# ukeSJTU/tiaozhanbei-unet

Measured on AMD Instinct MI355X. Metric: training images/sec, AnomalyUNet 256x256 bs=32 per GPU, higher is better.
Workload: dtype bf16; 1 GPU; AnomalyUNet 3x256x256, bs=32/GPU, MSE+focal loss, Adam (BASELINE.json configs[2], synthetic randn images, bernoulli masks); global_batch=32, parallelism=dp1, accumulate=fp32, master_params=fp32, dist_world=1, reserved_cus=0, cu_budget=256

## Files before the change

include/unet_hip.h:

```cpp
#ifndef UNET_HIP_H_
#define UNET_HIP_H_

#include <stddef.h>
#include <stdint.h>

#ifdef __cplusplus
extern "C" {
#endif

#define UNET_ABI_VERSION 1

enum unet_dtype { UNET_F32 = 0, UNET_BF16 = 1 };

enum unet_status {
  UNET_OK = 0,
  UNET_ERR_BAD_ARG = -1,
  UNET_ERR_UNSUPPORTED = -2,
  UNET_ERR_WORKSPACE = -3,
  UNET_ERR_LAUNCH = -4
};

typedef struct unet_view {
  void* ptr;
  int32_t c;
  int32_t h, w;
  int32_t off_y, off_x;
} unet_view;

int32_t unet_abi_version(void);
const char* unet_last_error(void);

int32_t unet_set_reserved_cus(int32_t n);
int32_t unet_get_cu_budget(void);
int32_t unet_debug_spin(int32_t blocks, int32_t lds_bytes, int32_t microseconds, void* stream);

enum unet_kclass {
  UNET_K_CONV_FWD = 0, UNET_K_CONV_DGRAD, UNET_K_CONV_WGRAD, UNET_K_CONVT_FWD, UNET_K_CONVT_DGRAD,
  UNET_K_CONVT_WGRAD, UNET_K_BN, UNET_K_POOL, UNET_K_HEAD, UNET_K_LOSS, UNET_K_PACK, UNET_K_OTHER,
  UNET_K_COUNT
};
int32_t unet_prof_enable(int32_t on);
int32_t unet_prof_collect(double* ms, int64_t* launches, double* flops);
int32_t unet_prof_kernel_stats(int32_t index, const char** name, double* ms, int64_t* launches, double* flops);
int32_t unet_prof_kernel_bytes(int32_t index, double* bytes);

int32_t unet_nchw_to_nhwc(const float* src, void* dst, int32_t n, int32_t c, int32_t h, int32_t w,
                          int32_t c_pad, int32_t dtype, void* stream);
int32_t unet_nhwc_to_nchw(const void* src, float* dst, int32_t n, int32_t c, int32_t h, int32_t w,
                          int32_t c_pad, int32_t dtype, void* stream);

enum unet_pack_mode {
  UNET_PACK_CONV_FWD = 0,
  UNET_PACK_CONV_DGRAD = 1,
  UNET_PACK_CONVT_FWD = 2,
  UNET_PACK_CONVT_DGRAD = 3
};
int32_t unet_pack_weight(const float* w, void* out, int32_t c_out, int32_t c_in, int32_t rows,
                         int32_t k, int32_t mode, int32_t dtype, void* stream);

typedef struct unet_pack_desc {
  const float* w;
  void* out;
  int32_t c_out, c_in, rows, k, mode, reserved;
} unet_pack_desc;
int32_t unet_pack_weights_batched(const unet_pack_desc* descs, int32_t n, int32_t dtype, void* stream);

int32_t unet_pack_weight_seg(const float* w, void* out, int32_t c_out, int32_t c_in, int32_t rows, int32_t k,
                             int32_t mode, int32_t split, int32_t dtype, void* stream);
int32_t unet_pack_conv_weight_folded_seg(const float* w, const float* scale, void* out, int32_t c_out, int32_t c_in,
                                         int32_t rows, int32_t k, int32_t split, int32_t dtype, void* stream);

enum unet_remap_op { UNET_REMAP_PAD = 0, UNET_REMAP_UNPAD = 1 };
#define UNET_REMAP_MAX 8
typedef struct unet_remap_desc {
  const float* src;
  float* dst;
  int32_t rows, cols, inner;
  int32_t prows, pcols;
  int32_t split, op, reserved;
} unet_remap_desc;
int32_t unet_remap_batched(const unet_remap_desc* descs, int32_t n, void* stream);

int32_t unet_widen_channels(const void* src, int32_t src_dtype, const int64_t* strides, int32_t n, int32_t c, int32_t h,
                            int32_t w, void* dst, int32_t c_pad, int32_t dtype, void* stream);

int32_t unet_conv3x3(int32_t dtype, int32_t n, int32_t h, int32_t w, const unet_view src[2],
                     const void* w_packed, int32_t c_out, const unet_view dst[2], int32_t dst_split,
                     int32_t accumulate, int32_t kclass, void* stream);

int32_t unet_pack_conv_weight_folded(const float* w, const float* scale, void* out, int32_t c_out, int32_t c_in,
                                     int32_t rows, int32_t k, int32_t dtype, void* stream);
int32_t unet_conv3x3_bias_relu(int32_t dtype, int32_t n, int32_t h, int32_t w, const unet_view src[2],
                               const void* w_packed, int32_t c_out, void* y, const float* bias, int32_t relu,
                               void* stream);

int32_t unet_conv3x3_first_supported(int32_t c_in, int32_t c_out, int32_t h, int32_t w);
int32_t unet_conv3x3_first_stats(int32_t n, int32_t h, int32_t w, const float* x_nchw, int32_t c_in,
                                 const float* weight_oihw, void* y, float* partial, int32_t* n_parts, void* stream);
size_t unet_conv3x3_first_wgrad_workspace(int32_t n, int32_t h, int32_t w);
int32_t unet_conv3x3_first_wgrad(int32_t n, int32_t h, int32_t w, const float* x_nchw, int32_t c_in, const void* dy,
                                 float* dw, void* workspace, size_t workspace_bytes, void* stream);
int32_t unet_conv3x3_first_wgrad_bn(int32_t n, int32_t h, int32_t w, const float* x_nchw, int32_t c_in, const void* dz,
                                    const void* y, const float* coefs, float* dw, void* workspace,
                                    size_t workspace_bytes, void* stream);

size_t unet_conv3x3_stats_max_parts(int32_t n, int32_t h, int32_t w);
int32_t unet_conv3x3_stats(int32_t dtype, int32_t n, int32_t h, int32_t w, const unet_view src[2],
                           const void* w_packed, int32_t c_out, void* y, float* partial, int32_t* n_parts,
                           void* stream);

int32_t unet_conv3x3_dgrad_bnrelu_supported(int32_t dtype, int32_t n, int32_t h, int32_t w, int32_t c_dy, int32_t c_dx);
int32_t unet_conv3x3_dgrad_bnrelu(int32_t dtype, int32_t n, int32_t h, int32_t w, const void* dy, int32_t c_dy,
                                  const void* w_packed, int32_t c_dx, const void* y_prev, const float* bn_scale,
                                  const float* bn_shift, const float* bn_mean, void* dz, float* partial,
                                  int32_t* n_parts, void* stream);

size_t unet_conv3x3_wgrad_workspace(int32_t n, int32_t h, int32_t w, int32_t c_in, int32_t c_out);
int32_t unet_conv3x3_wgrad(int32_t dtype, int32_t n, int32_t h, int32_t w, const unet_view src[2],
                           const void* dy, int32_t c_out, float* dw, int32_t c_in_param,
                           void* workspace, size_t workspace_bytes, void* stream);

int32_t unet_convt2x2_fwd(int32_t dtype, int32_t n, int32_t h, int32_t w, const void* x, int32_t c_in,
                          const void* w_packed, const float* bias, void* y, int32_t c_out, void* stream);
int32_t unet_convt2x2_dgrad(int32_t dtype, int32_t n, int32_t h, int32_t w, const void* dy,
                            int32_t c_out, const void* w_packed, void* dx, int32_t c_in, void* stream);

int32_t unet_convt2x2_dgrad_bnrelu_supported(int32_t dtype, int32_t n, int32_t h, int32_t w, int32_t c_in, int32_t c_out);
size_t unet_convt2x2_dgrad_bnrelu_max_parts(void);
int32_t unet_convt2x2_dgrad_bnrelu(int32_t dtype, int32_t n, int32_t h, int32_t w, const void* dy, int32_t c_out,
                                   const void* w_packed, const void* y_prev, const float* bn_scale, const float* bn_shift,
                                   const float* bn_mean, void* dz, int32_t c_in, float* partial, int32_t* n_parts,
                                   void* stream);
size_t unet_convt2x2_wgrad_workspace(int32_t n, int32_t h, int32_t w, int32_t c_in, int32_t c_out);
int32_t unet_convt2x2_wgrad(int32_t dtype, int32_t n, int32_t h, int32_t w, const void* x, int32_t c_in,
                            const void* dy, int32_t c_out, float* dw, float* db, void* workspace,
                            size_t workspace_bytes, void* stream);

size_t unet_bn_workspace(int64_t pixels, int32_t c);
int32_t unet_bn_train_stats(int32_t dtype, const void* y, int64_t pixels, int32_t c, const float* gamma,
                            const float* beta, float* running_mean, float* running_var, float momentum,
                            float eps, float* save_mean, float* save_istd, float* scale, float* shift,
                            void* workspace, size_t workspace_bytes, void* stream);
int32_t unet_bn_finalize_partials(const float* partial, int32_t n_parts, int64_t pixels, int32_t c,
                                  const float* gamma, const float* beta, float* running_mean,
                                  float* running_var, float momentum, float eps, float* save_mean,
                                  float* save_istd, float* scale, float* shift, void* stream);
int32_t unet_bn_eval_coeffs(int32_t c, const float* gamma, const float* beta, const float* running_mean,
                            const float* running_var, float eps, float* scale, float* shift, void* stream);
int32_t unet_bn_eval_coeffs4(int32_t c, const float* gamma, const float* beta, const float* running_mean,
                             const float* running_var, float eps, float* mean, float* istd, float* scale,
                             float* shift, void* stream);
int32_t unet_bn_relu_apply(int32_t dtype, const void* y, int64_t pixels, int32_t c, const float* scale,
                           const float* shift, void* a, void* stream);
int32_t unet_bn_relu_bwd(int32_t dtype, const void* da, const void* y, int64_t pixels, int32_t c,
                         const float* gamma, const float* save_mean, const float* save_istd,
                         const float* scale, const float* shift, float* dgamma, float* dbeta, void* dy,
                         void* workspace, size_t workspace_bytes, void* stream);

int32_t unet_bn_relu_bwd_frozen(int32_t dtype, const void* da, const void* y, int64_t pixels, int32_t c,
                                const float* gamma, const float* mean, const float* istd, const float* scale,
                                const float* shift, float* dgamma, float* dbeta, void* dy, void* workspace,
                                size_t workspace_bytes, void* stream);
int32_t unet_bn_bwd_premasked(int32_t dtype, const void* dz, const void* y, int64_t pixels, int32_t c,
                              const float* gamma, const float* save_mean, const float* save_istd,
                              const float* partial, int32_t n_parts, float* dgamma, float* dbeta, void* dy,
                              void* workspace, size_t workspace_bytes, void* stream);

int32_t unet_maxpool2_fwd(int32_t dtype, const void* x, int32_t n, int32_t h, int32_t w, int32_t c,
                          void* y, void* stream);
int32_t unet_maxpool2_bwd(int32_t dtype, const void* x, const void* dy, int32_t n, int32_t h, int32_t w,
                          int32_t c, void* dx, int32_t accumulate, void* stream);

int32_t unet_bn_relu_pool_supported(int32_t dtype, int32_t c);
int32_t unet_bn_relu_pool_fwd(int32_t dtype, const void* y, int32_t n, int32_t h, int32_t w, int32_t c,
                              const float* scale, const float* shift, void* a, void* pooled, void* stream);
size_t unet_bn_relu_pool_max_parts(void);
int32_t unet_bn_relu_pool_bwd(int32_t dtype, const void* y, const void* dpooled, const void* da_old, int32_t n, int32_t h,
                              int32_t w, int32_t c, const float* scale, const float* shift, const float* mean, void* dz,
                              float* partial, int32_t* n_parts, void* stream);

int32_t unet_upsample_bilinear2x_fwd(int32_t dtype, const void* x, int32_t n, int32_t h, int32_t w,
                                     int32_t c, void* y, void* stream);
int32_t unet_upsample_bilinear2x_bwd(int32_t dtype, const void* dy, int32_t n, int32_t h, int32_t w,
                                     int32_t c, void* dx, void* stream);

int32_t unet_head_fwd(int32_t dtype, const void* x, int32_t n, int32_t h, int32_t w, int32_t c_in,
                      const float* weight, const float* bias, int32_t c_out, int32_t sigmoid, float* out,
                      void* stream);
size_t unet_head_bwd_workspace(int32_t n, int32_t h, int32_t w, int32_t c_in, int32_t c_out);
int32_t unet_head_bwd(int32_t dtype, const void* x, const float* out, const float* dout, int32_t n,
                      int32_t h, int32_t w, int32_t c_in, const float* weight, int32_t c_out,
                      int32_t sigmoid, void* dx, float* dweight, float* dbias, void* workspace,
                      size_t workspace_bytes, void* stream);

int32_t unet_head_bnrelu_fwd(int32_t dtype, const void* y, int32_t n, int32_t h, int32_t w, int32_t c_in,
                             const float* bn_scale, const float* bn_shift, const float* weight, const float* bias,
                             int32_t c_out, int32_t sigmoid, float* out, void* stream);
size_t unet_head_bnrelu_max_parts(void);
int32_t unet_head_bnrelu_bwd(int32_t dtype, const void* y, const float* bn_scale, const float* bn_shift,
                             const float* bn_mean, const float* out, const float* dout, int32_t n, int32_t h, int32_t w,
                             int32_t c_in, const float* weight, int32_t c_out, int32_t sigmoid, void* dz,
                             float* dweight, float* dbias, float* bn_partial, int32_t* n_parts, void* workspace,
                             size_t workspace_bytes, void* stream);

size_t unet_loss_workspace(int64_t elems);
int32_t unet_loss_mse_focal(const float* recon, const float* image, int64_t n_recon, const float* amap,
                            const float* mask, int64_t n_amap, float alpha, float gamma, float* losses,
                            float* d_recon, float* d_amap, void* workspace, size_t workspace_bytes,
                            void* stream);
size_t unet_ssim_workspace(int32_t planes, int32_t h, int32_t w);
int32_t unet_ssim_loss(const float* img1, const float* img2, int32_t planes, int32_t h, int32_t w,
                       int32_t window, float* loss, float* d_img1, float* d_img2, void* workspace,
                       size_t workspace_bytes, void* stream);

int32_t unet_ssim_loss_per_image(const float* img1, const float* img2, int32_t n, int32_t c, int32_t h, int32_t w,
                                 int32_t window, float* loss, float* d_img1, float* d_img2, void* workspace,
                                 size_t workspace_bytes, void* stream);

size_t unet_seg_loss_workspace(int32_t n, int32_t c, int64_t hw);
int32_t unet_seg_loss(const float* logits, const int64_t* target, int32_t n, int32_t c, int64_t hw,
                      const float* class_weights, int64_t ignore_index, int32_t input_is_prob, float ce_weight,
                      float dice_weight, float focal_weight, float focal_alpha, float focal_gamma, float* loss,
                      float* dlogits, void* workspace, size_t workspace_bytes, void* stream);
int32_t unet_seg_confusion(const float* logits, const int64_t* target, int32_t n, int32_t c, int64_t hw,
                           int64_t ignore_index, int64_t* labels, int64_t* confusion, void* stream);
size_t unet_seg_image_stats_workspace(int32_t n, int32_t c, int64_t hw);
int32_t unet_seg_image_stats(const float* logits, const int64_t* target, int32_t n, int32_t c, int64_t hw,
                             int64_t ignore_index, uint8_t* labels, int64_t* confusion, double* conf, void* workspace,
                             size_t workspace_bytes, void* stream);

int32_t unet_threshold_confusion(const float* pred, const float* truth, const uint8_t* select, int64_t n_images,
                                 int64_t per_image, const float* thresholds, int32_t k, int64_t* counts, void* stream);

int32_t unet_rank_auc_append(const float* pred, const float* truth, const uint8_t* select, int64_t n_images,
                             int64_t per_image, uint32_t* keys, int64_t capacity, int64_t* counts, void* stream);
size_t unet_rank_auc_workspace(int64_t n_pos, int64_t n_neg);
int32_t unet_rank_auc(uint32_t* pos_keys, int64_t n_pos, uint32_t* neg_keys, int64_t n_neg, double* out,
                      void* workspace, size_t workspace_bytes, void* stream);

size_t unet_label_regions_workspace(int64_t n, int64_t h, int64_t w);
int32_t unet_label_regions(const float* truth, const uint8_t* select, int64_t n, int64_t h, int64_t w, int32_t* labels,
                           int32_t* sizes, int64_t* counts, void* workspace, size_t workspace_bytes, void* stream);

size_t unet_label_class_regions_workspace(int64_t n, int64_t h, int64_t w, int32_t num_classes);
int32_t unet_label_class_regions(const uint8_t* classes, int64_t n, int64_t h, int64_t w, int32_t num_classes,
                                 int32_t* region, int32_t* sizes, int64_t* counts, void* workspace,
                                 size_t workspace_bytes, void* stream);
size_t unet_match_class_regions_workspace(int64_t n, int64_t h, int64_t w, int32_t num_classes);
int32_t unet_match_class_regions(const uint8_t* truth, const int32_t* truth_region, const int32_t* truth_sizes,
                                 const uint8_t* pred, const int32_t* pred_region, const int32_t* pred_sizes, int64_t n,
                                 int64_t h, int64_t w, int32_t num_classes, int32_t min_pixels, int32_t image_base,
                                 int32_t* truth_records, int32_t* pred_records, int64_t capacity,
                                 int64_t* record_counts, void* workspace, size_t workspace_bytes, void* stream);

int32_t unet_region_auc_append(const float* pred, const int32_t* sizes, const uint8_t* select, int64_t n_images,
                               int64_t per_image, void* slots, int64_t capacity, int64_t* counts, void* stream);
size_t unet_region_auc_workspace(int64_t n_pos, int64_t n_neg);
int32_t unet_region_auc(uint64_t* pos_pairs, int64_t n_pos, uint32_t* neg_keys, int64_t n_neg, int64_t regions,
                        int64_t max_region, double fpr_limit, double* out, void* workspace, size_t workspace_bytes,
                        void* stream);

enum unet_panel_kind {
  UNET_PANEL_IMAGE = 0, UNET_PANEL_UNIT = 1, UNET_PANEL_GRAY = 2, UNET_PANEL_HOT = 3, UNET_PANEL_OVERLAY = 4
};
typedef struct unet_panel {
  int32_t kind;
  int32_t alpha8;
  const float* rgb;
  const float* map;
} unet_panel;
int32_t unet_render_range(const unet_panel* panels, int32_t k, int32_t n, int32_t h, int32_t w, uint32_t* keys,
                          void* stream);
int32_t unet_render_sheet(const unet_panel* panels, int32_t k, int32_t n, int32_t h, int32_t w, int32_t gutter,
                          const float* mean3, const float* std3, const uint32_t* keys, const uint8_t* luts,
                          uint8_t* sheet, void* stream);

int32_t unet_seg_confidence(const float* logits, int32_t n, int32_t c, int64_t hw, uint8_t* labels, float* conf,
                            void* stream);

enum unet_seg_panel_kind {
  UNET_SEG_PANEL_IMAGE = 0, UNET_SEG_PANEL_CLASSES = 1, UNET_SEG_PANEL_OVERLAY = 2, UNET_SEG_PANEL_LUT = 3
};
typedef struct unet_seg_panel {
  int32_t kind;
  int32_t alpha8;
  const uint8_t* labels;
  const float* map;
} unet_seg_panel;
int32_t unet_seg_render_sheet(const float* image, const unet_seg_panel* panels, int32_t k, int32_t n, int32_t h,
                              int32_t w, int32_t gutter, int32_t per_row, const float* mean3, const float* std3,
                              const uint8_t* palette, const uint8_t* lut, uint8_t* sheet, void* stream);

int32_t unet_channel_scale(int32_t dtype, const void* x, const float* scale, int32_t n, int64_t hw, int32_t c, void* y,
                           void* stream);
size_t unet_anomaly_score_workspace(int32_t n, int64_t hw);
int32_t unet_anomaly_score(const float* recon, const float* image, int32_t n, int32_t c, int64_t hw, int32_t l1,
                           float* score, float* image_score, void* workspace, size_t workspace_bytes, void* stream);

int32_t unet_preprocess_u8(const uint8_t* images_hwc, const uint8_t* flip, float* out_nchw, int32_t n, int32_t h,
                           int32_t w, const float* mean3, const float* std3, void* stream);

int32_t unet_resize_bilinear_ksize(int32_t in_size, int32_t out_size);
int32_t unet_resize_bilinear_coeffs(int32_t in_size, int32_t out_size, int32_t* bounds, int32_t* kk);
int32_t unet_resize_bilinear_u8(const uint8_t* src, int32_t n, int32_t h, int32_t w, int32_t c, int32_t out_h,
                                int32_t out_w, const int32_t* xbounds, const int32_t* xkk, int32_t xksize,
                                const int32_t* ybounds, const int32_t* ykk, int32_t yksize, uint8_t* tmp, uint8_t* dst,
                                void* stream);
int32_t unet_resize_nearest_index(int32_t in_size, int32_t out_size, int32_t* idx);
int32_t unet_resize_nearest_u8(const uint8_t* src, int32_t n, int32_t h, int32_t w, int32_t c, int32_t out_h,
                               int32_t out_w, const int32_t* yidx, const int32_t* xidx, uint8_t* dst, void* stream);
int32_t unet_polygon_mask_u8(const int32_t* verts, const int32_t* poly_offsets, const int32_t* poly_class,
                             const int32_t* poly_image, int32_t n_polys, int32_t max_poly_vertices, const int32_t* src_hw,
                             int32_t n, int32_t out_h, int32_t out_w, const int32_t* yidx, const int32_t* xidx,
                             uint8_t* dst, void* stream);
int32_t unet_polygon_class_histogram(const int32_t* verts, const int32_t* poly_offsets, const int32_t* poly_class,
                                     const int32_t* poly_image, int32_t n_polys, int32_t max_poly_vertices,
                                     const int32_t* src_hw, int32_t n, int32_t max_h, int32_t max_w, int64_t* hist,
                                     void* stream);
int32_t unet_flip_rotate_u8(const uint8_t* src, int32_t n, int32_t h, int32_t w, int32_t c, const uint8_t* flip,
                            const int32_t* matrices, uint8_t* dst, void* stream);
typedef struct unet_jitter_desc {
  int32_t order[4];
  float brightness, contrast, saturation;
  int32_t hue_shift;
} unet_jitter_desc;
size_t unet_color_jitter_workspace(int32_t n);
int32_t unet_color_jitter_normalize_u8(const uint8_t* images_hwc, int32_t n, int32_t h, int32_t w,
                                       const unet_jitter_desc* desc, const float* mean3, const float* std3,
                                       float* out_nchw, void* workspace, size_t workspace_bytes, void* stream);

int32_t unet_adam_step(float* param, const float* grad, float* exp_avg, float* exp_avg_sq, int64_t n,
                       float lr, double beta1, double beta2, float eps, float weight_decay,
                       float grad_scale, int32_t step, void* stream);

typedef struct unet_adam_desc {
  float* p;
  const float* g;
  float* m;
  float* v;
  int64_t n;
} unet_adam_desc;
typedef struct unet_adam_chunk {
  int32_t tensor;
  int32_t reserved;
  int64_t first;
} unet_adam_chunk;
int32_t unet_adam_chunk_elems(void);
int32_t unet_adam_multi(const unet_adam_desc* descs, const unet_adam_chunk* chunks, int32_t n_chunks, float lr, double beta1,
                        double beta2, float eps, float weight_decay, float grad_scale, int32_t step, int32_t decoupled,
                        void* stream);

#ifdef __cplusplus
}
#endif
#endif
```

tiaozhanbei_unet_amd/_lib.py:

```python
from __future__ import annotations

import ctypes as C
import os
import subprocess

_HERE = os.path.dirname(os.path.abspath(__file__))
LIB_PATH = os.environ.get("UNET_HIP_LIB") or os.path.join(_HERE, "libunet_hip.so")
CSRC = os.path.join(_HERE, "csrc")

UNET_F32, UNET_BF16 = 0, 1
PACK_CONV_FWD, PACK_CONV_DGRAD, PACK_CONVT_FWD, PACK_CONVT_DGRAD = 0, 1, 2, 3
(K_CONV_FWD, K_CONV_DGRAD, K_CONV_WGRAD, K_CONVT_FWD, K_CONVT_DGRAD, K_CONVT_WGRAD, K_BN, K_POOL,
 K_HEAD, K_LOSS, K_PACK, K_OTHER, K_COUNT) = range(13)
KCLASS_NAMES = ["conv3x3_fwd", "conv3x3_dgrad", "conv3x3_wgrad", "convt_fwd", "convt_dgrad",
                "convt_wgrad", "bn", "pool_upsample", "head", "loss", "pack_layout", "other"]


class View(C.Structure):
    _fields_ = [("ptr", C.c_void_p), ("c", C.c_int32), ("h", C.c_int32), ("w", C.c_int32),
                ("off_y", C.c_int32), ("off_x", C.c_int32)]


View2 = View * 2


class RemapDesc(C.Structure):
    _fields_ = [("src", C.c_void_p), ("dst", C.c_void_p), ("rows", C.c_int32), ("cols", C.c_int32),
                ("inner", C.c_int32), ("prows", C.c_int32), ("pcols", C.c_int32), ("split", C.c_int32),
                ("op", C.c_int32), ("reserved", C.c_int32)]


REMAP_PAD, REMAP_UNPAD = 0, 1


class Panel(C.Structure):
    _fields_ = [("kind", C.c_int32), ("alpha8", C.c_int32), ("rgb", C.c_void_p), ("map", C.c_void_p)]


PANEL_IMAGE, PANEL_UNIT, PANEL_GRAY, PANEL_HOT, PANEL_OVERLAY = range(5)


class SegPanel(C.Structure):
    _fields_ = [("kind", C.c_int32), ("alpha8", C.c_int32), ("labels", C.c_void_p), ("map", C.c_void_p)]


SEG_PANEL_IMAGE, SEG_PANEL_CLASSES, SEG_PANEL_OVERLAY, SEG_PANEL_LUT = range(4)
_i, _l, _f, _p, _z, _d = C.c_int32, C.c_int64, C.c_float, C.c_void_p, C.c_size_t, C.c_double

SIGNATURES = {
    "unet_abi_version": (_i, []),
    "unet_last_error": (C.c_char_p, []),
    "unet_set_reserved_cus": (_i, [_i]),
    "unet_get_cu_budget": (_i, []),
    "unet_debug_spin": (_i, [_i, _i, _i, _p]),
    "unet_prof_enable": (_i, [_i]),
    "unet_prof_collect": (_i, [_p, _p, _p]),
    "unet_prof_kernel_stats": (_i, [_i, _p, _p, _p, _p]),
    "unet_prof_kernel_bytes": (_i, [_i, _p]),
    "unet_nchw_to_nhwc": (_i, [_p, _p, _i, _i, _i, _i, _i, _i, _p]),
    "unet_nhwc_to_nchw": (_i, [_p, _p, _i, _i, _i, _i, _i, _i, _p]),
    "unet_pack_weight": (_i, [_p, _p, _i, _i, _i, _i, _i, _i, _p]),
    "unet_pack_weights_batched": (_i, [_p, _i, _i, _p]),
    "unet_pack_weight_seg": (_i, [_p, _p, _i, _i, _i, _i, _i, _i, _i, _p]),
    "unet_pack_conv_weight_folded_seg": (_i, [_p, _p, _p, _i, _i, _i, _i, _i, _i, _p]),
    "unet_remap_batched": (_i, [_p, _i, _p]),
    "unet_widen_channels": (_i, [_p, _i, _p, _i, _i, _i, _i, _p, _i, _i, _p]),
    "unet_conv3x3": (_i, [_i, _i, _i, _i, C.POINTER(View), _p, _i, C.POINTER(View), _i, _i, _i, _p]),
    "unet_pack_conv_weight_folded": (_i, [_p, _p, _p, _i, _i, _i, _i, _i, _p]),
    "unet_conv3x3_bias_relu": (_i, [_i, _i, _i, _i, C.POINTER(View), _p, _i, _p, _p, _i, _p]),
    "unet_conv3x3_stats_max_parts": (_z, [_i, _i, _i]),
    "unet_conv3x3_stats": (_i, [_i, _i, _i, _i, C.POINTER(View), _p, _i, _p, _p, _p, _p]),
    "unet_conv3x3_first_supported": (_i, [_i, _i, _i, _i]),
    "unet_conv3x3_first_stats": (_i, [_i, _i, _i, _p, _i, _p, _p, _p, _p, _p]),
    "unet_conv3x3_first_wgrad_workspace": (_z, [_i, _i, _i]),
    "unet_conv3x3_first_wgrad": (_i, [_i, _i, _i, _p, _i, _p, _p, _p, _z, _p]),
    "unet_conv3x3_first_wgrad_bn": (_i, [_i, _i, _i, _p, _i, _p, _p, _p, _p, _p, _z, _p]),
    "unet_bn_finalize_partials": (_i, [_p, _i, _l, _i, _p, _p, _p, _p, _f, _f, _p, _p, _p, _p, _p]),
    "unet_convt2x2_dgrad_bnrelu_supported": (_i, [_i, _i, _i, _i, _i, _i]),
    "unet_convt2x2_dgrad_bnrelu_max_parts": (_z, []),
    "unet_convt2x2_dgrad_bnrelu": (_i, [_i, _i, _i, _i, _p, _i, _p, _p, _p, _p, _p, _p, _i, _p, _p, _p]),
    "unet_conv3x3_dgrad_bnrelu_supported": (_i, [_i, _i, _i, _i, _i, _i]),
    "unet_conv3x3_dgrad_bnrelu": (_i, [_i, _i, _i, _i, _p, _i, _p, _i, _p, _p, _p, _p, _p, _p, _p, _p]),
    "unet_conv3x3_wgrad_workspace": (_z, [_i, _i, _i, _i, _i]),
    "unet_conv3x3_wgrad": (_i, [_i, _i, _i, _i, C.POINTER(View), _p, _i, _p, _i, _p, _z, _p]),
    "unet_convt2x2_fwd": (_i, [_i, _i, _i, _i, _p, _i, _p, _p, _p, _i, _p]),
    "unet_convt2x2_dgrad": (_i, [_i, _i, _i, _i, _p, _i, _p, _p, _i, _p]),
    "unet_convt2x2_wgrad_workspace": (_z, [_i, _i, _i, _i, _i]),
    "unet_convt2x2_wgrad": (_i, [_i, _i, _i, _i, _p, _i, _p, _i, _p, _p, _p, _z, _p]),
    "unet_bn_workspace": (_z, [_l, _i]),
    "unet_bn_train_stats": (_i, [_i, _p, _l, _i, _p, _p, _p, _p, _f, _f, _p, _p, _p, _p, _p, _z, _p]),
    "unet_bn_eval_coeffs": (_i, [_i, _p, _p, _p, _p, _f, _p, _p, _p]),
    "unet_bn_eval_coeffs4": (_i, [_i, _p, _p, _p, _p, _f, _p, _p, _p, _p, _p]),
    "unet_bn_relu_bwd_frozen": (_i, [_i, _p, _p, _l, _i, _p, _p, _p, _p, _p, _p, _p, _p, _p, _z, _p]),
    "unet_bn_relu_apply": (_i, [_i, _p, _l, _i, _p, _p, _p, _p]),
    "unet_bn_relu_bwd": (_i, [_i, _p, _p, _l, _i, _p, _p, _p, _p, _p, _p, _p, _p, _p, _z, _p]),
    "unet_bn_bwd_premasked": (_i, [_i, _p, _p, _l, _i, _p, _p, _p, _p, _i, _p, _p, _p, _p, _z, _p]),
    "unet_head_bnrelu_fwd": (_i, [_i, _p, _i, _i, _i, _i, _p, _p, _p, _p, _i, _i, _p, _p]),
    "unet_head_bnrelu_max_parts": (_z, []),
    "unet_head_bnrelu_bwd": (_i, [_i, _p, _p, _p, _p, _p, _p, _i, _i, _i, _i, _p, _i, _i, _p, _p, _p, _p, _p, _p, _z, _p]),
    "unet_maxpool2_fwd": (_i, [_i, _p, _i, _i, _i, _i, _p, _p]),
    "unet_maxpool2_bwd": (_i, [_i, _p, _p, _i, _i, _i, _i, _p, _i, _p]),
    "unet_bn_relu_pool_supported": (_i, [_i, _i]),
    "unet_bn_relu_pool_fwd": (_i, [_i, _p, _i, _i, _i, _i, _p, _p, _p, _p, _p]),
    "unet_bn_relu_pool_max_parts": (_z, []),
    "unet_bn_relu_pool_bwd": (_i, [_i, _p, _p, _p, _i, _i, _i, _i, _p, _p, _p, _p, _p, _p, _p]),
    "unet_upsample_bilinear2x_fwd": (_i, [_i, _p, _i, _i, _i, _i, _p, _p]),
    "unet_upsample_bilinear2x_bwd": (_i, [_i, _p, _i, _i, _i, _i, _p, _p]),
    "unet_head_fwd": (_i, [_i, _p, _i, _i, _i, _i, _p, _p, _i, _i, _p, _p]),
    "unet_head_bwd_workspace": (_z, [_i, _i, _i, _i, _i]),
    "unet_head_bwd": (_i, [_i, _p, _p, _p, _i, _i, _i, _i, _p, _i, _i, _p, _p, _p, _p, _z, _p]),
    "unet_loss_workspace": (_z, [_l]),
    "unet_loss_mse_focal": (_i, [_p, _p, _l, _p, _p, _l, _f, _f, _p, _p, _p, _p, _z, _p]),
    "unet_ssim_workspace": (_z, [_i, _i, _i]),
    "unet_ssim_loss": (_i, [_p, _p, _i, _i, _i, _i, _p, _p, _p, _p, _z, _p]),
    "unet_ssim_loss_per_image": (_i, [_p, _p, _i, _i, _i, _i, _i, _p, _p, _p, _p, _z, _p]),
    "unet_seg_loss_workspace": (_z, [_i, _i, _l]),
    "unet_seg_loss": (_i, [_p, _p, _i, _i, _l, _p, _l, _i, _f, _f, _f, _f, _f, _p, _p, _p, _z, _p]),
    "unet_seg_confusion": (_i, [_p, _p, _i, _i, _l, _l, _p, _p, _p]),
    "unet_seg_image_stats_workspace": (_z, [_i, _i, _l]),
    "unet_seg_image_stats": (_i, [_p, _p, _i, _i, _l, _l, _p, _p, _p, _p, _z, _p]),
    "unet_threshold_confusion": (_i, [_p, _p, _p, _l, _l, _p, _i, _p, _p]),
    "unet_rank_auc_append": (_i, [_p, _p, _p, _l, _l, _p, _l, _p, _p]),
    "unet_rank_auc_workspace": (_z, [_l, _l]),
    "unet_rank_auc": (_i, [_p, _l, _p, _l, _p, _p, _z, _p]),
    "unet_label_regions_workspace": (_z, [_l, _l, _l]),
    "unet_label_regions": (_i, [_p, _p, _l, _l, _l, _p, _p, _p, _p, _z, _p]),
    "unet_label_class_regions_workspace": (_z, [_l, _l, _l, _i]),
    "unet_label_class_regions": (_i, [_p, _l, _l, _l, _i, _p, _p, _p, _p, _z, _p]),
    "unet_match_class_regions_workspace": (_z, [_l, _l, _l, _i]),
    "unet_match_class_regions": (_i, [_p, _p, _p, _p, _p, _p, _l, _l, _l, _i, _i, _i, _p, _p, _l, _p, _p, _z, _p]),
    "unet_region_auc_append": (_i, [_p, _p, _p, _l, _l, _p, _l, _p, _p]),
    "unet_region_auc_workspace": (_z, [_l, _l]),
    "unet_region_auc": (_i, [_p, _l, _p, _l, _l, _l, _d, _p, _p, _z, _p]),
    "unet_render_range": (_i, [_p, _i, _i, _i, _i, _p, _p]),
    "unet_render_sheet": (_i, [_p, _i, _i, _i, _i, _i, _p, _p, _p, _p, _p, _p]),
    "unet_seg_confidence": (_i, [_p, _i, _i, _l, _p, _p, _p]),
    "unet_seg_render_sheet": (_i, [_p, _p, _i, _i, _i, _i, _i, _i, _p, _p, _p, _p, _p, _p]),
    "unet_channel_scale": (_i, [_i, _p, _p, _i, _l, _i, _p, _p]),
    "unet_anomaly_score_workspace": (_z, [_i, _l]),
    "unet_anomaly_score": (_i, [_p, _p, _i, _i, _l, _i, _p, _p, _p, _z, _p]),
    "unet_preprocess_u8": (_i, [_p, _p, _p, _i, _i, _i, _p, _p, _p]),
    "unet_resize_bilinear_ksize": (_i, [_i, _i]),
    "unet_resize_bilinear_coeffs": (_i, [_i, _i, _p, _p]),
    "unet_resize_bilinear_u8": (_i, [_p, _i, _i, _i, _i, _i, _i, _p, _p, _i, _p, _p, _i, _p, _p, _p]),
    "unet_resize_nearest_index": (_i, [_i, _i, _p]),
    "unet_resize_nearest_u8": (_i, [_p, _i, _i, _i, _i, _i, _i, _p, _p, _p, _p]),
    "unet_polygon_mask_u8": (_i, [_p, _p, _p, _p, _i, _i, _p, _i, _i, _i, _p, _p, _p, _p]),
    "unet_polygon_class_histogram": (_i, [_p, _p, _p, _p, _i, _i, _p, _i, _i, _i, _p, _p]),
    "unet_flip_rotate_u8": (_i, [_p, _i, _i, _i, _i, _p, _p, _p, _p]),
    "unet_color_jitter_workspace": (_z, [_i]),
    "unet_color_jitter_normalize_u8": (_i, [_p, _i, _i, _i, _p, _p, _p, _p, _p, _z, _p]),
    "unet_adam_chunk_elems": (_i, []),
    "unet_adam_multi": (_i, [_p, _p, _i, _f, _d, _d, _f, _f, _f, _i, _i, _p]),
    "unet_adam_step": (_i, [_p, _p, _p, _p, _l, _f, _d, _d, _f, _f, _f, _i, _p]),
}

_lib = None


def build(force: bool = False) -> str:
    if force or not os.path.exists(LIB_PATH) or _stale():
        subprocess.run(["make", "-C", CSRC, "-j8"], check=True, stdout=subprocess.DEVNULL)
    return LIB_PATH


def _stale() -> bool:
    if not os.path.isdir(CSRC):
        return False
    t = os.path.getmtime(LIB_PATH)
    srcs = [os.path.join(CSRC, f) for f in os.listdir(CSRC) if f.endswith((".hip", ".h"))]
    srcs.append(os.path.join(_HERE, "..", "include", "unet_hip.h"))
    return any(os.path.exists(s) and os.path.getmtime(s) > t for s in srcs)


def lib():
    global _lib
    if _lib is None:
        if not os.path.exists(LIB_PATH):
            raise RuntimeError(
                f"libunet_hip.so not found at {LIB_PATH}: the HIP extension is the only compute path of "
                "tiaozhanbei_unet_amd (no CPU/eager fallback). Build it with "
                "`python -c 'import __graft_entry__ as g; g.build()'` or `make -C tiaozhanbei_unet_amd/csrc`.")
        handle = C.CDLL(LIB_PATH)
        for name, (res, args) in SIGNATURES.items():
            fn = getattr(handle, name)
            fn.restype, fn.argtypes = res, args
        if handle.unet_abi_version() != 1:
            raise RuntimeError("libunet_hip.so: ABI version mismatch")
        _lib = handle
    return _lib


def check(rc: int, what: str) -> None:
    if rc != 0:
        msg = lib().unet_last_error().decode(errors="replace")
        raise RuntimeError(f"{what} failed (status {rc}): {msg}")
```

tiaozhanbei_unet_amd/csrc/elementwise.hip:

```cpp
#include "common.h"

namespace {

inline int ew_blocks(long long items) { return (int)std::min<long long>(cdiv64(items, 256), 256 * 16); }

template <typename T>
__global__ __launch_bounds__(256) void nchw_to_nhwc_kernel(const float* __restrict__ src, T* __restrict__ dst,
                                                           int N, int C, int H, int W, int Cp) {
  constexpr int PIECE = ET<T>::PIECE;
  const long long hw = (long long)H * W;
  const long long total = (long long)N * hw;
  for (long long i = blockIdx.x * (long long)blockDim.x + threadIdx.x; i < total;
       i += (long long)gridDim.x * blockDim.x) {
    const long long n = i / hw, p = i - n * hw;
    const float* s = src + n * C * hw + p;
    T* o = dst + i * Cp;
    for (int c0 = 0; c0 < Cp; c0 += PIECE) {
      float v[PIECE];
#pragma unroll
      for (int j = 0; j < PIECE; ++j) v[j] = (c0 + j < C) ? s[(long long)(c0 + j) * hw] : 0.f;
      Vec<T>::store(o + c0, v);
    }
  }
}

template <typename T>
__global__ void nhwc_to_nchw_kernel(const T* __restrict__ src, float* __restrict__ dst, int N, int C, int H,
                                    int W, int Cp) {
  const long long hw = (long long)H * W;
  const long long total = (long long)N * C * hw;
  for (long long i = blockIdx.x * (long long)blockDim.x + threadIdx.x; i < total;
       i += (long long)gridDim.x * blockDim.x) {
    const long long p = i % hw;
    const long long t = i / hw;
    const int c = (int)(t % C);
    const long long n = t / C;
    dst[i] = ET<T>::to_f(src[(n * hw + p) * Cp + c]);
  }
}

template <typename T>
__global__ void pack_weight_kernel(const float* __restrict__ w, T* __restrict__ out, int Co, int Ci, int rows,
                                   int K, int mode, long long total, const float* __restrict__ scale) {
  for (long long i = blockIdx.x * (long long)blockDim.x + threadIdx.x; i < total;
       i += (long long)gridDim.x * blockDim.x) {
    float v = 0.f;
    if (mode == UNET_PACK_CONV_FWD) {
      const int ci = (int)(i % K);
      long long t = i / K;
      const int co = (int)(t % rows);
      const int tap = (int)(t / rows);
      if (co < Co && ci < Ci) v = w[((long long)co * Ci + ci) * 9 + tap] * (scale ? scale[co] : 1.f);
    } else if (mode == UNET_PACK_CONV_DGRAD) {
      const int co = (int)(i % K);
      long long t = i / K;
      const int ci = (int)(t % rows);
      const int tap = (int)(t / rows);
      if (co < Co && ci < Ci) v = w[((long long)co * Ci + ci) * 9 + (8 - tap)];
    } else if (mode == UNET_PACK_CONVT_FWD) {
      const int ci = (int)(i % K);
      long long t = i / K;
      const int co = (int)(t % rows);
      const int z = (int)(t / rows);
      if (co < Co && ci < Ci) v = w[((long long)ci * Co + co) * 4 + z];
    } else {
      const int co = (int)(i % K);
      long long t = i / K;
      const int z = (int)(t % 4);
      const int ci = (int)(t / 4);
      if (co < Co && ci < Ci) v = w[((long long)ci * Co + co) * 4 + z];
    }
    out[i] = ET<T>::from_f(v);
  }
}

template <typename T>
__global__ __launch_bounds__(256) void pack_weights_batched_kernel(const unet_pack_desc* __restrict__ descs) {
  __shared__ float tile[32 * 289];
  const unet_pack_desc d = descs[blockIdx.y];
  const int mode = d.mode;
  if (d.reserved > 0 && mode <= UNET_PACK_CONV_DGRAD) {
    const long long total = 9LL * d.rows * d.k;
    T* __restrict__ out = reinterpret_cast<T*>(d.out);
    for (long long i = blockIdx.x * 256LL + threadIdx.x; i < total; i += (long long)gridDim.x * 256)
      out[i] = ET<T>::from_f(unet_pack_seg_value(d.w, d.c_out, d.c_in, d.rows, d.k, mode, d.reserved, i, nullptr));
    return;
  }
  if constexpr (sizeof(T) == 2) {
    auto pair_ok = [](const unet_pack_desc& f, const unet_pack_desc& g) {
      return f.mode == UNET_PACK_CONV_FWD && g.mode == UNET_PACK_CONV_DGRAD && f.w == g.w && f.c_out == g.c_out &&
             f.c_in == g.c_in && f.rows == f.c_out && f.k == f.c_in && g.rows == g.c_in && g.k == g.c_out &&
             (f.c_out & 31) == 0 && (f.c_in & 31) == 0;
    };
    if (mode == UNET_PACK_CONV_DGRAD && blockIdx.y > 0 && pair_ok(descs[blockIdx.y - 1], d)) return;
    if (mode == UNET_PACK_CONV_FWD && blockIdx.y + 1 < gridDim.y && pair_ok(d, descs[blockIdx.y + 1])) {
      const unet_pack_desc g = descs[blockIdx.y + 1];
      const int Co = d.c_out, Ci = d.c_in;
      const int nB = Ci / 32, ntile = (Co / 32) * nB;
      const float* __restrict__ w = d.w;
      bf16_t* __restrict__ of = reinterpret_cast<bf16_t*>(d.out);
      bf16_t* __restrict__ og = reinterpret_cast<bf16_t*>(g.out);
      for (int t = blockIdx.x; t < ntile; t += gridDim.x) {
        const int a0 = (t / nB) * 32, b0 = (t % nB) * 32;
        __syncthreads();
        for (int i = threadIdx.x; i < 32 * 288; i += 256) {
          const int al = i / 288, r = i - al * 288;
          tile[al * 289 + r] = w[((size_t)(a0 + al) * Ci + b0) * 9 + r];
        }
        __syncthreads();
        for (int gi = threadIdx.x; gi < 2 * 32 * 9 * 4; gi += 256) {
          const int lay = gi / (32 * 9 * 4), rem = gi % (32 * 9 * 4);
          const int q = rem & 3, rest = rem >> 2;
          const int tap = rest % 9, outer = rest / 9;
          bf16x8 r8;
          if (lay == 0) {
#pragma unroll
            for (int e = 0; e < 8; ++e) r8[e] = (bf16_t)tile[outer * 289 + (q * 8 + e) * 9 + tap];
            *reinterpret_cast<bf16x8*>(of + ((size_t)tap * Co + a0 + outer) * Ci + b0 + q * 8) = r8;
          } else {
#pragma unroll
            for (int e = 0; e < 8; ++e) r8[e] = (bf16_t)tile[(q * 8 + e) * 289 + outer * 9 + tap];
            *reinterpret_cast<bf16x8*>(og + ((size_t)(8 - tap) * Ci + b0 + outer) * Co + a0 + q * 8) = r8;
          }
        }
      }
      return;
    }
  }
  const bool conv = mode <= UNET_PACK_CONV_DGRAD;
  const int taps = conv ? 9 : 4;
  const int As = conv ? d.c_out : d.c_in, Bs = conv ? d.c_in : d.c_out;
  const bool along_b = (mode == UNET_PACK_CONV_FWD || mode == UNET_PACK_CONVT_DGRAD);
  const int Ap = (mode == UNET_PACK_CONV_FWD || mode == UNET_PACK_CONVT_DGRAD) ? d.rows : d.k;
  const int Bp = (mode == UNET_PACK_CONV_FWD || mode == UNET_PACK_CONVT_DGRAD) ? d.k : d.rows;
  const int TA = along_b ? 8 : 64, TB = along_b ? 64 : 8;
  const int nA = (Ap + TA - 1) / TA, nB = (Bp + TB - 1) / TB;
  const float* __restrict__ w = d.w;
  T* __restrict__ out = reinterpret_cast<T*>(d.out);
  const int run = TB * taps;
  for (int t = blockIdx.x; t < nA * nB; t += gridDim.x) {
    const int a0 = (t / nB) * TA, b0 = (t % nB) * TB;
    __syncthreads();
    for (int i = threadIdx.x; i < TA * run; i += 256) {
      const int al = i / run, r = i - al * run;
      const int a = a0 + al, bb = b0 + r / taps;
      tile[i] = (a < As && bb < Bs) ? w[((size_t)a * Bs + b0) * taps + r] : 0.f;
    }
    __syncthreads();
    if ((((along_b ? Bp : Ap) & 7) == 0) && ((d.k & 7) == 0)) {
      for (int gi = threadIdx.x; gi < TA * TB * taps / 8; gi += 256) {
        const int inner0 = (gi & 7) * 8, rest = gi >> 3;
        const int tap = rest % taps, outer = rest / taps;
        const int al0 = along_b ? outer : inner0, bl0 = along_b ? inner0 : outer;
        const int a = a0 + al0, bb = b0 + bl0;
        if (a >= Ap || bb >= Bp) continue;
        float v[8];
#pragma unroll
        for (int e = 0; e < 8; ++e) v[e] = tile[(al0 + (along_b ? 0 : e)) * run + (bl0 + (along_b ? e : 0)) * taps + tap];
        size_t o;
        if (mode == UNET_PACK_CONV_FWD) o = ((size_t)tap * d.rows + a) * d.k + bb;
        else if (mode == UNET_PACK_CONV_DGRAD) o = ((size_t)(8 - tap) * d.rows + bb) * d.k + a;
        else if (mode == UNET_PACK_CONVT_FWD) o = ((size_t)tap * d.rows + bb) * d.k + a;
        else o = ((size_t)a * 4 + tap) * d.k + bb;
        if constexpr (sizeof(T) == 2) {
          bf16x8 r;
#pragma unroll
          for (int e = 0; e < 8; ++e) r[e] = (bf16_t)v[e];
          *reinterpret_cast<bf16x8*>(out + o) = r;
        } else {
          *reinterpret_cast<f32x4*>(out + o) = f32x4{v[0], v[1], v[2], v[3]};
          *reinterpret_cast<f32x4*>(out + o + 4) = f32x4{v[4], v[5], v[6], v[7]};
        }
      }
      continue;
    }
    for (int i = threadIdx.x; i < TA * TB * taps; i += 256) {
      const int inner = i & 63, rest = i >> 6;
      const int tap = rest % taps, outer = rest / taps;
      const int al = along_b ? outer : inner, bl = along_b ? inner : outer;
      const int a = a0 + al, bb = b0 + bl;
      if (a >= Ap || bb >= Bp) continue;
      const float v = tile[al * run + bl * taps + tap];
      size_t o;
      if (mode == UNET_PACK_CONV_FWD) o = ((size_t)tap * d.rows + a) * d.k + bb;
      else if (mode == UNET_PACK_CONV_DGRAD) o = ((size_t)(8 - tap) * d.rows + bb) * d.k + a;
      else if (mode == UNET_PACK_CONVT_FWD) o = ((size_t)tap * d.rows + bb) * d.k + a;
      else o = ((size_t)a * 4 + tap) * d.k + bb;
      out[o] = ET<T>::from_f(v);
    }
  }
}

template <typename T>
__global__ void maxpool2_fwd_kernel(const T* __restrict__ x, T* __restrict__ y, int N, int H, int W, int C) {
  constexpr int PIECE = ET<T>::PIECE;
  const int OH = H / 2, OW = W / 2, G = C / PIECE;
  const long long total = (long long)N * OH * OW * G;
  for (long long i = blockIdx.x * (long long)blockDim.x + threadIdx.x; i < total;
       i += (long long)gridDim.x * blockDim.x) {
    const int g = (int)(i % G);
    long long t = i / G;
    const int ox = (int)(t % OW);  t /= OW;
    const int oy = (int)(t % OH);
    const long long n = t / OH;
    const T* p = x + ((n * H + 2 * oy) * W + 2 * ox) * (long long)C + g * PIECE;
    float a[PIECE], b[PIECE], c[PIECE], d[PIECE];
    Vec<T>::load(p, a);
    Vec<T>::load(p + C, b);
    Vec<T>::load(p + (long long)W * C, c);
    Vec<T>::load(p + (long long)W * C + C, d);
#pragma unroll
    for (int j = 0; j < PIECE; ++j) a[j] = fmaxf(fmaxf(a[j], b[j]), fmaxf(c[j], d[j]));
    Vec<T>::store(y + i * PIECE, a);
  }
}

template <typename T>
__global__ void maxpool2_bwd_kernel(const T* __restrict__ x, const T* __restrict__ dy, T* __restrict__ dx,
                                    int N, int H, int W, int C, int accumulate) {
  constexpr int PIECE = ET<T>::PIECE;
  const int OH = H / 2, OW = W / 2, G = C / PIECE;
  const int WH = (H + 1) / 2, WW = (W + 1) / 2;
  const long long total = (long long)N * WH * WW * G;
  for (long long i = blockIdx.x * (long long)blockDim.x + threadIdx.x; i < total;
       i += (long long)gridDim.x * blockDim.x) {
    const int g = (int)(i % G);
    long long t = i / G;
    const int ox = (int)(t % WW);  t /= WW;
    const int oy = (int)(t % WH);
    const long long n = t / WH;
    const long long base = ((n * H + 2 * oy) * W + 2 * ox) * (long long)C + g * PIECE;
    float z[PIECE];
#pragma unroll
    for (int j = 0; j < PIECE; ++j) z[j] = 0.f;
    if (oy < OH && ox < OW) {
      float a[PIECE], b[PIECE], c[PIECE], d[PIECE], gr[PIECE];
      Vec<T>::load(x + base, a);
      Vec<T>::load(x + base + C, b);
      Vec<T>::load(x + base + (long long)W * C, c);
      Vec<T>::load(x + base + (long long)W * C + C, d);
      Vec<T>::load(dy + (((n * OH + oy) * OW + ox) * (long long)C + g * PIECE), gr);
      float ga[PIECE], gb[PIECE], gc[PIECE], gd[PIECE];
#pragma unroll
      for (int j = 0; j < PIECE; ++j) {
        const float m = fmaxf(fmaxf(a[j], b[j]), fmaxf(c[j], d[j]));
        const bool fa = a[j] == m, fb = !fa && b[j] == m, fc = !fa && !fb && c[j] == m;
        const bool fd = !fa && !fb && !fc;
        ga[j] = fa ? gr[j] : 0.f; gb[j] = fb ? gr[j] : 0.f; gc[j] = fc ? gr[j] : 0.f; gd[j] = fd ? gr[j] : 0.f;
      }
      if (accumulate) {
        Vec<T>::load(dx + base, a);
        Vec<T>::load(dx + base + C, b);
        Vec<T>::load(dx + base + (long long)W * C, c);
        Vec<T>::load(dx + base + (long long)W * C + C, d);
#pragma unroll
        for (int j = 0; j < PIECE; ++j) { ga[j] += a[j]; gb[j] += b[j]; gc[j] += c[j]; gd[j] += d[j]; }
      }
      Vec<T>::store(dx + base, ga);
      Vec<T>::store(dx + base + C, gb);
      Vec<T>::store(dx + base + (long long)W * C, gc);
      Vec<T>::store(dx + base + (long long)W * C + C, gd);
    } else if (!accumulate) {
      const int y0 = 2 * oy, x0 = 2 * ox;
      for (int dyy = 0; dyy < 2; ++dyy)
        for (int dxx = 0; dxx < 2; ++dxx)
          if (y0 + dyy < H && x0 + dxx < W)
            Vec<T>::store(dx + base + ((long long)dyy * W + dxx) * C, z);
    }
  }
}

template <typename T, typename IDX>
__global__ __launch_bounds__(256) void bn_relu_pool_fwd_kernel(const T* __restrict__ y, const float* __restrict__ scale,
                                                               const float* __restrict__ shift, T* __restrict__ a,
                                                               T* __restrict__ pooled, int N, int H, int W, int C) {
  constexpr int PIECE = ET<T>::PIECE;
  typedef IDX idx_t;
  const int OH = H / 2, OW = W / 2, G = C / PIECE;
  const int WH = (H + 1) / 2, WW = (W + 1) / 2;
  const idx_t total = (idx_t)N * WH * WW * G;
  const int g = threadIdx.x % G;
  float sc[PIECE], sh[PIECE];
#pragma unroll
  for (int j = 0; j < PIECE; ++j) { sc[j] = scale[g * PIECE + j]; sh[j] = shift[g * PIECE + j]; }
  for (idx_t i = (idx_t)blockIdx.x * 256 + threadIdx.x; i < total; i += (idx_t)gridDim.x * 256) {
    idx_t t = i / G;
    const int ox = (int)(t % WW);  t /= WW;
    const int oy = (int)(t % WH);
    const idx_t n = t / WH;
    const idx_t base = ((n * H + 2 * oy) * W + 2 * ox) * (idx_t)C + g * PIECE;
    const bool ex = 2 * ox + 1 < W, ey = 2 * oy + 1 < H;
    float v[4][PIECE];
#pragma unroll
    for (int k = 0; k < 4; ++k) {
      const bool ok = ((k & 1) == 0 || ex) && ((k >> 1) == 0 || ey);
      const idx_t o = base + ((idx_t)(k >> 1) * W + (k & 1)) * C;
#pragma unroll
      for (int j = 0; j < PIECE; ++j) v[k][j] = 0.f;
      if (ok) {
        Vec<T>::load(y + o, v[k]);
#pragma unroll
        for (int j = 0; j < PIECE; ++j) v[k][j] = ET<T>::to_f(ET<T>::from_f(fmaxf(fmaf(v[k][j], sc[j], sh[j]), 0.f)));
        Vec<T>::store(a + o, v[k]);
      }
    }
    if (oy < OH && ox < OW) {
#pragma unroll
      for (int j = 0; j < PIECE; ++j) v[0][j] = fmaxf(fmaxf(v[0][j], v[1][j]), fmaxf(v[2][j], v[3][j]));
      Vec<T>::store(pooled + (((n * OH + oy) * OW + ox) * (idx_t)C + g * PIECE), v[0]);
    }
  }
}

template <typename T, typename IDX>
__global__ __launch_bounds__(256) void bn_relu_pool_bwd_kernel(const T* __restrict__ y, const T* __restrict__ dpooled,
                                                               const T* da_old, const float* __restrict__ scale,
                                                               const float* __restrict__ shift,
                                                               const float* __restrict__ mean, T* dz,
                                                               float* __restrict__ part, int N, int H, int W, int C) {
  constexpr int PIECE = ET<T>::PIECE;
  typedef IDX idx_t;
  __shared__ float red[2][256][PIECE + 1];
  const int OH = H / 2, OW = W / 2, G = C / PIECE;
  const int WH = (H + 1) / 2, WW = (W + 1) / 2;
  const idx_t total = (idx_t)N * WH * WW * G;
  const int g = threadIdx.x % G;
  float sc[PIECE], sh[PIECE], mu[PIECE], s0[PIECE], s1[PIECE];
#pragma unroll
  for (int j = 0; j < PIECE; ++j) {
    sc[j] = scale[g * PIECE + j]; sh[j] = shift[g * PIECE + j]; mu[j] = mean[g * PIECE + j];
    s0[j] = 0.f; s1[j] = 0.f;
  }
  const idx_t i0 = (idx_t)blockIdx.x * 256 + threadIdx.x;
  idx_t t0 = i0 / G;
  int ox = (int)(t0 % WW);  t0 /= WW;
  int oy = (int)(t0 % WH);
  idx_t n = t0 / WH;
  idx_t ts = ((idx_t)gridDim.x * 256) / G;
  const int sx = (int)(ts % WW);  ts /= WW;
  const int sy = (int)(ts % WH);
  const idx_t sn = ts / WH;
  for (idx_t i = i0; i < total; i += (idx_t)gridDim.x * 256) {
    const idx_t base = ((n * H + 2 * oy) * W + 2 * ox) * (idx_t)C + g * PIECE;
    const bool ex = 2 * ox + 1 < W, ey = 2 * oy + 1 < H, full = oy < OH && ox < OW;
    if (ex && ey) {
      const idx_t o1 = base + C, o2 = base + (idx_t)W * C, o3 = o2 + C;
      float gr[PIECE], yv[4][PIECE], od[4][PIECE];
      Vec<T>::load(dpooled + (((n * OH + oy) * OW + ox) * (idx_t)C + g * PIECE), gr);
      Vec<T>::load(y + base, yv[0]);
      Vec<T>::load(y + o1, yv[1]);
      Vec<T>::load(y + o2, yv[2]);
      Vec<T>::load(y + o3, yv[3]);
      if (da_old) {
        Vec<T>::load(da_old + base, od[0]);
        Vec<T>::load(da_old + o1, od[1]);
        Vec<T>::load(da_old + o2, od[2]);
        Vec<T>::load(da_old + o3, od[3]);
      } else {
#pragma unroll
        for (int k = 0; k < 4; ++k)
#pragma unroll
          for (int j = 0; j < PIECE; ++j) od[k][j] = 0.f;
      }
#pragma unroll
      for (int j = 0; j < PIECE; ++j) {
        float z[4], a[4];
#pragma unroll
        for (int k = 0; k < 4; ++k) {
          z[k] = fmaf(yv[k][j], sc[j], sh[j]);
          a[k] = ET<T>::to_f(ET<T>::from_f(fmaxf(z[k], 0.f)));
        }
        const float m = fmaxf(fmaxf(a[0], a[1]), fmaxf(a[2], a[3]));
        const bool e0 = a[0] == m, e1 = a[1] == m, e2 = a[2] == m;
        const bool f[4] = {e0, !e0 && e1, !(e0 || e1) && e2, !(e0 || e1 || e2)};
#pragma unroll
        for (int k = 0; k < 4; ++k) {
          const float d = f[k] ? od[k][j] + gr[j] : od[k][j];
          const float da = ET<T>::to_f(ET<T>::from_f(d));
          const float v = z[k] > 0.f ? da : 0.f;
          od[k][j] = v;
          s0[j] += v;
          s1[j] = fmaf(v, yv[k][j] - mu[j], s1[j]);
        }
      }
      Vec<T>::store(dz + base, od[0]);
      Vec<T>::store(dz + o1, od[1]);
      Vec<T>::store(dz + o2, od[2]);
      Vec<T>::store(dz + o3, od[3]);
    } else {
    float yv[4][PIECE], av[4][PIECE], gr[PIECE];
    bool on[4][PIECE];
#pragma unroll
    for (int j = 0; j < PIECE; ++j) gr[j] = 0.f;
    if (full) Vec<T>::load(dpooled + (((n * OH + oy) * OW + ox) * (idx_t)C + g * PIECE), gr);
#pragma unroll
    for (int k = 0; k < 4; ++k) {
      const bool ok = ((k & 1) == 0 || ex) && ((k >> 1) == 0 || ey);
#pragma unroll
      for (int j = 0; j < PIECE; ++j) { yv[k][j] = 0.f; av[k][j] = -1.f; on[k][j] = false; }
      if (ok) {
        Vec<T>::load(y + base + ((idx_t)(k >> 1) * W + (k & 1)) * C, yv[k]);
#pragma unroll
        for (int j = 0; j < PIECE; ++j) {
          const float z = fmaf(yv[k][j], sc[j], sh[j]);
          on[k][j] = z > 0.f;
          av[k][j] = ET<T>::to_f(ET<T>::from_f(fmaxf(z, 0.f)));
        }
      }
    }
#pragma unroll
    for (int k = 0; k < 4; ++k) {
      const bool ok = ((k & 1) == 0 || ex) && ((k >> 1) == 0 || ey);
      if (!ok) continue;
      const idx_t o = base + ((idx_t)(k >> 1) * W + (k & 1)) * C;
      float d[PIECE];
#pragma unroll
      for (int j = 0; j < PIECE; ++j) d[j] = 0.f;
      if (da_old) Vec<T>::load(da_old + o, d);
#pragma unroll
      for (int j = 0; j < PIECE; ++j) {
        if (full) {
          const float m = fmaxf(fmaxf(av[0][j], av[1][j]), fmaxf(av[2][j], av[3][j]));
          bool first = av[k][j] == m;
#pragma unroll
          for (int q = 0; q < 4; ++q) first = first && !(q < k && av[q][j] == m);
          if (first) d[j] += gr[j];
        }
        const float da = ET<T>::to_f(ET<T>::from_f(d[j]));
        const float v = ET<T>::to_f(ET<T>::from_f(on[k][j] ? da : 0.f));
        d[j] = v;
        s0[j] += v;
        s1[j] = fmaf(v, yv[k][j] - mu[j], s1[j]);
      }
      Vec<T>::store(dz + o, d);
    }
    }
    ox += sx;
    if (ox >= WW) { ox -= WW; ++oy; }
    oy += sy;
    if (oy >= WH) { oy -= WH; ++n; }
    n += sn;
  }
#pragma unroll
  for (int j = 0; j < PIECE; ++j) { red[0][threadIdx.x][j] = s0[j]; red[1][threadIdx.x][j] = s1[j]; }
  __syncthreads();
  for (int c = threadIdx.x; c < 2 * C; c += 256) {
    const int q = c / C, ch = c - q * C, gg = ch / PIECE, j = ch - gg * PIECE;
    float tsum = 0.f;
    for (int k = gg; k < 256; k += G) tsum += red[q][k][j];
    part[((size_t)blockIdx.x * 2 + q) * C + ch] = tsum;
  }
}

__device__ inline void bil_axis(int o, int n_in, int n_out, int& i0, int& i1, float& f, float& g) {
  const unsigned den = n_out > 1 ? n_out - 1 : 1;
  const unsigned num = (unsigned)o * (unsigned)(n_in - 1);
  i0 = (int)(num / den);
  if (i0 > n_in - 1) i0 = n_in - 1;
  i1 = i0 + 1 < n_in ? i0 + 1 : n_in - 1;
  const unsigned rem = num - (unsigned)i0 * den;
  f = (float)rem / (float)den;
  g = (float)(den - rem) / (float)den;
}

template <typename T>
__global__ void bilinear2x_fwd_kernel(const T* __restrict__ x, T* __restrict__ y, int N, int H, int W, int C) {
  constexpr int PIECE = ET<T>::PIECE;
  const int OH = 2 * H, OW = 2 * W, G = C / PIECE;
  const long long total = (long long)N * OH * OW * G;
  for (long long i = blockIdx.x * (long long)blockDim.x + threadIdx.x; i < total;
       i += (long long)gridDim.x * blockDim.x) {
    const int g = (int)(i % G);
    long long t = i / G;
    const int ox = (int)(t % OW);  t /= OW;
    const int oy = (int)(t % OH);
    const long long n = t / OH;
    int y0, y1, x0, x1; float fy, fx, gy, gx;
    bil_axis(oy, H, OH, y0, y1, fy, gy);
    bil_axis(ox, W, OW, x0, x1, fx, gx);
    float a[PIECE], b[PIECE], c[PIECE], d[PIECE];
    const T* p = x + n * H * (long long)W * C + g * PIECE;
    Vec<T>::load(p + ((long long)y0 * W + x0) * C, a);
    Vec<T>::load(p + ((long long)y0 * W + x1) * C, b);
    Vec<T>::load(p + ((long long)y1 * W + x0) * C, c);
    Vec<T>::load(p + ((long long)y1 * W + x1) * C, d);
#pragma unroll
    for (int j = 0; j < PIECE; ++j) {
      const float top = a[j] * gx + b[j] * fx, bot = c[j] * gx + d[j] * fx;
      a[j] = top * gy + bot * fy;
    }
    Vec<T>::store(y + i * PIECE, a);
  }
}

template <typename T>
__global__ void bilinear2x_bwd_kernel(const T* __restrict__ dy, T* __restrict__ dx, int N, int H, int W, int C) {
  constexpr int PIECE = ET<T>::PIECE;
  const int OH = 2 * H, OW = 2 * W, G = C / PIECE;
  const long long total = (long long)N * H * W * G;
  for (long long i = blockIdx.x * (long long)blockDim.x + threadIdx.x; i < total;
       i += (long long)gridDim.x * blockDim.x) {
    const int g = (int)(i % G);
    long long t = i / G;
    const int ix = (int)(t % W);  t /= W;
    const int iy = (int)(t % H);
    const long long n = t / H;
    float acc[PIECE];
#pragma unroll
    for (int j = 0; j < PIECE; ++j) acc[j] = 0.f;
    const int oy_lo = max(0, 2 * iy - 2), oy_hi = min(OH - 1, 2 * iy + 3);
    const int ox_lo = max(0, 2 * ix - 2), ox_hi = min(OW - 1, 2 * ix + 3);
    for (int oy = oy_lo; oy <= oy_hi; ++oy) {
      int y0, y1; float fy, gy;
      bil_axis(oy, H, OH, y0, y1, fy, gy);
      float wy = 0.f;
      if (y0 == iy) wy += gy;
      if (y1 == iy) wy += fy;
      if (wy == 0.f) continue;
      for (int ox = ox_lo; ox <= ox_hi; ++ox) {
        int x0, x1; float fx, gx;
        bil_axis(ox, W, OW, x0, x1, fx, gx);
        float wx = 0.f;
        if (x0 == ix) wx += gx;
        if (x1 == ix) wx += fx;
        if (wx == 0.f) continue;
        float v[PIECE];
        Vec<T>::load(dy + (((n * OH + oy) * OW + ox) * (long long)C + g * PIECE), v);
#pragma unroll
        for (int j = 0; j < PIECE; ++j) acc[j] = fmaf(v[j], wy * wx, acc[j]);
      }
    }
    Vec<T>::store(dx + i * PIECE, acc);
  }
}

__global__ void adam_kernel(float* __restrict__ p, const float* __restrict__ g, float* __restrict__ m,
                            float* __restrict__ v, long long n4, float lr, float b1, float b2, float omb1,
                            float omb2, float eps, float wd, float gscale, float bc1, float bc2_sqrt) {
  for (long long i = blockIdx.x * (long long)blockDim.x + threadIdx.x; i < n4;
       i += (long long)gridDim.x * blockDim.x) {
    f32x4 pp = reinterpret_cast<f32x4*>(p)[i], gg = reinterpret_cast<const f32x4*>(g)[i];
    f32x4 mm = reinterpret_cast<f32x4*>(m)[i], vv = reinterpret_cast<f32x4*>(v)[i];
#pragma unroll
    for (int j = 0; j < 4; ++j) {
      const float gr = fmaf(wd, pp[j], gg[j] * gscale);
      mm[j] = b1 * mm[j] + omb1 * gr;
      vv[j] = b2 * vv[j] + omb2 * gr * gr;
      const float denom = sqrtf(vv[j]) / bc2_sqrt + eps;
      pp[j] -= (lr / bc1) * (mm[j] / denom);
    }
    reinterpret_cast<f32x4*>(p)[i] = pp;
    reinterpret_cast<f32x4*>(m)[i] = mm;
    reinterpret_cast<f32x4*>(v)[i] = vv;
  }
}

}

extern "C" int32_t unet_nchw_to_nhwc(const float* src, void* dst, int32_t n, int32_t c, int32_t h, int32_t w,
                                     int32_t c_pad, int32_t dtype, void* stream) {
  UNET_REQUIRE(src && dst, UNET_ERR_BAD_ARG, "unet_nchw_to_nhwc: null pointer");
  UNET_REQUIRE(n > 0 && c > 0 && h > 0 && w > 0 && c_pad >= c && c_pad % 8 == 0, UNET_ERR_BAD_ARG,
               "unet_nchw_to_nhwc: bad dims (c=%d c_pad=%d, c_pad must be a multiple of 8)", c, c_pad);
  hipStream_t s = (hipStream_t)stream;
  const long long total = (long long)n * h * w;
  ProfScope prof(UNET_K_PACK, 0.0, s);
  if (dtype == UNET_BF16)
    hipLaunchKernelGGL(nchw_to_nhwc_kernel<bf16_t>, dim3(ew_blocks(total)), dim3(256), 0, s, src, (bf16_t*)dst, n, c, h, w, c_pad);
  else
    hipLaunchKernelGGL(nchw_to_nhwc_kernel<float>, dim3(ew_blocks(total)), dim3(256), 0, s, src, (float*)dst, n, c, h, w, c_pad);
  return unet_check_launch("nchw_to_nhwc_kernel");
}

extern "C" int32_t unet_nhwc_to_nchw(const void* src, float* dst, int32_t n, int32_t c, int32_t h, int32_t w,
                                     int32_t c_pad, int32_t dtype, void* stream) {
  UNET_REQUIRE(src && dst, UNET_ERR_BAD_ARG, "unet_nhwc_to_nchw: null pointer");
  UNET_REQUIRE(n > 0 && c > 0 && h > 0 && w > 0 && c_pad >= c, UNET_ERR_BAD_ARG, "unet_nhwc_to_nchw: bad dims");
  hipStream_t s = (hipStream_t)stream;
  const long long total = (long long)n * h * w * c;
  ProfScope prof(UNET_K_PACK, 0.0, s);
  if (dtype == UNET_BF16)
    hipLaunchKernelGGL(nhwc_to_nchw_kernel<bf16_t>, dim3(ew_blocks(total)), dim3(256), 0, s, (const bf16_t*)src, dst, n, c, h, w, c_pad);
  else
    hipLaunchKernelGGL(nhwc_to_nchw_kernel<float>, dim3(ew_blocks(total)), dim3(256), 0, s, (const float*)src, dst, n, c, h, w, c_pad);
  return unet_check_launch("nhwc_to_nchw_kernel");
}

extern "C" int32_t unet_pack_weight(const float* w, void* out, int32_t c_out, int32_t c_in, int32_t rows,
                                    int32_t k, int32_t mode, int32_t dtype, void* stream) {
  UNET_REQUIRE(w && out, UNET_ERR_BAD_ARG, "unet_pack_weight: null pointer");
  UNET_REQUIRE(c_out > 0 && c_in > 0 && rows > 0 && k > 0 && mode >= 0 && mode <= 3, UNET_ERR_BAD_ARG,
               "unet_pack_weight: bad dims/mode");
  const int gemm_rows = (mode == UNET_PACK_CONV_FWD || mode == UNET_PACK_CONVT_FWD) ? c_out : c_in;
  const int gemm_k = (mode == UNET_PACK_CONV_FWD || mode == UNET_PACK_CONVT_FWD) ? c_in : c_out;
  UNET_REQUIRE(rows >= gemm_rows && k >= gemm_k, UNET_ERR_BAD_ARG, "unet_pack_weight: padded dims too small");
  const int taps = (mode <= UNET_PACK_CONV_DGRAD) ? 9 : 4;
  const long long total = (long long)taps * rows * k;
  hipStream_t s = (hipStream_t)stream;
  ProfScope prof(UNET_K_PACK, 0.0, s);
  if (dtype == UNET_BF16)
    hipLaunchKernelGGL(pack_weight_kernel<bf16_t>, dim3(ew_blocks(total)), dim3(256), 0, s, w, (bf16_t*)out, c_out, c_in, rows, k, mode, total, (const float*)nullptr);
  else
    hipLaunchKernelGGL(pack_weight_kernel<float>, dim3(ew_blocks(total)), dim3(256), 0, s, w, (float*)out, c_out, c_in, rows, k, mode, total, (const float*)nullptr);
  return unet_check_launch("pack_weight_kernel");
}

extern "C" int32_t unet_pack_conv_weight_folded(const float* w, const float* scale, void* out, int32_t c_out, int32_t c_in,
                                                int32_t rows, int32_t k, int32_t dtype, void* stream) {
  UNET_REQUIRE(w && scale && out, UNET_ERR_BAD_ARG, "unet_pack_conv_weight_folded: null pointer");
  UNET_REQUIRE(c_out > 0 && c_in > 0 && rows >= c_out && k >= c_in, UNET_ERR_BAD_ARG, "unet_pack_conv_weight_folded: bad dims");
  const long long total = 9LL * rows * k;
  hipStream_t s = (hipStream_t)stream;
  ProfScope prof(UNET_K_PACK, 0.0, s);
  if (dtype == UNET_BF16)
    hipLaunchKernelGGL(pack_weight_kernel<bf16_t>, dim3(ew_blocks(total)), dim3(256), 0, s, w, (bf16_t*)out, c_out, c_in, rows, k,
                       (int)UNET_PACK_CONV_FWD, total, scale);
  else
    hipLaunchKernelGGL(pack_weight_kernel<float>, dim3(ew_blocks(total)), dim3(256), 0, s, w, (float*)out, c_out, c_in, rows, k,
                       (int)UNET_PACK_CONV_FWD, total, scale);
  return unet_check_launch("pack_weight_kernel");
}

extern "C" int32_t unet_pack_weights_batched(const unet_pack_desc* descs, int32_t n, int32_t dtype, void* stream) {
  UNET_REQUIRE(descs && n > 0 && n <= 65535, UNET_ERR_BAD_ARG, "unet_pack_weights_batched: bad argument");
  hipStream_t s = (hipStream_t)stream;
  ProfScope prof(UNET_K_PACK, 0.0, s);
  if (dtype == UNET_BF16)
    hipLaunchKernelGGL(pack_weights_batched_kernel<bf16_t>, dim3(224, n), dim3(256), 0, s, descs);
  else
    hipLaunchKernelGGL(pack_weights_batched_kernel<float>, dim3(224, n), dim3(256), 0, s, descs);
  return unet_check_launch("pack_weights_batched_kernel");
}

#define EW_DISPATCH(NAME, KERN, TOTAL, ...)                                                                 \
  do {                                                                                                        \
    hipStream_t s = (hipStream_t)stream;                                                                      \
    ProfScope prof(UNET_K_POOL, 0.0, s);                                                                      \
    if (dtype == UNET_BF16) {                                                                                 \
      typedef bf16_t T;                                                                                       \
      const long long total = (TOTAL) / 8;                                                                    \
      hipLaunchKernelGGL(KERN<bf16_t>, dim3(ew_blocks(total)), dim3(256), 0, s, __VA_ARGS__);                 \
    } else {                                                                                                  \
      typedef float T;                                                                                        \
      const long long total = (TOTAL) / 4;                                                                    \
      hipLaunchKernelGGL(KERN<float>, dim3(ew_blocks(total)), dim3(256), 0, s, __VA_ARGS__);                  \
    }                                                                                                         \
    return unet_check_launch(NAME);                                                                           \
  } while (0)

extern "C" int32_t unet_maxpool2_fwd(int32_t dtype, const void* x, int32_t n, int32_t h, int32_t w, int32_t c,
                                     void* y, void* stream) {
  UNET_REQUIRE(x && y, UNET_ERR_BAD_ARG, "unet_maxpool2_fwd: null pointer");
  UNET_REQUIRE(n > 0 && h >= 2 && w >= 2 && c > 0 && c % 8 == 0, UNET_ERR_UNSUPPORTED, "unet_maxpool2_fwd: dims");
  EW_DISPATCH("maxpool2_fwd_kernel", maxpool2_fwd_kernel, (long long)n * (h / 2) * (w / 2) * c, (const T*)x, (T*)y, n, h, w, c);
}

extern "C" int32_t unet_maxpool2_bwd(int32_t dtype, const void* x, const void* dy, int32_t n, int32_t h,
                                     int32_t w, int32_t c, void* dx, int32_t accumulate, void* stream) {
  UNET_REQUIRE(x && dy && dx, UNET_ERR_BAD_ARG, "unet_maxpool2_bwd: null pointer");
  UNET_REQUIRE(n > 0 && h >= 2 && w >= 2 && c > 0 && c % 8 == 0, UNET_ERR_UNSUPPORTED, "unet_maxpool2_bwd: dims");
  EW_DISPATCH("maxpool2_bwd_kernel", maxpool2_bwd_kernel, (long long)n * ((h + 1) / 2) * ((w + 1) / 2) * c,
              (const T*)x, (const T*)dy, (T*)dx, n, h, w, c, accumulate);
}


extern "C" int32_t unet_bn_relu_pool_supported(int32_t dtype, int32_t c) {
  const int piece = dtype == UNET_BF16 ? 8 : 4;
  return (c > 0 && c % piece == 0 && 256 % (c / piece) == 0) ? 1 : 0;
}

extern "C" int32_t unet_bn_relu_pool_fwd(int32_t dtype, const void* y, int32_t n, int32_t h, int32_t w, int32_t c,
                                         const float* scale, const float* shift, void* a, void* pooled, void* stream) {
  UNET_REQUIRE(y && scale && shift && a && pooled, UNET_ERR_BAD_ARG, "unet_bn_relu_pool_fwd: null pointer");
  UNET_REQUIRE(n > 0 && h >= 2 && w >= 2 && unet_bn_relu_pool_supported(dtype, c), UNET_ERR_UNSUPPORTED,
               "unet_bn_relu_pool_fwd: c=%d h=%d w=%d", c, h, w);
  hipStream_t s = (hipStream_t)stream;
  ProfScope prof(UNET_K_BN, 0.0, s, "bn_relu_pool_fwd_kernel");
  const long long total = (long long)n * ((h + 1) / 2) * ((w + 1) / 2) * (c / (dtype == UNET_BF16 ? 8 : 4));
  const bool small = (long long)n * h * w * c < 0x7FFFFFFFLL;
  if (dtype == UNET_BF16) {
    if (small)
      hipLaunchKernelGGL((bn_relu_pool_fwd_kernel<bf16_t, int>), dim3(ew_blocks(total)), dim3(256), 0, s, (const bf16_t*)y, scale,
                         shift, (bf16_t*)a, (bf16_t*)pooled, n, h, w, c);
    else
      hipLaunchKernelGGL((bn_relu_pool_fwd_kernel<bf16_t, long long>), dim3(ew_blocks(total)), dim3(256), 0, s, (const bf16_t*)y,
                         scale, shift, (bf16_t*)a, (bf16_t*)pooled, n, h, w, c);
  } else {
    hipLaunchKernelGGL((bn_relu_pool_fwd_kernel<float, long long>), dim3(ew_blocks(total)), dim3(256), 0, s, (const float*)y, scale,
                       shift, (float*)a, (float*)pooled, n, h, w, c);
  }
  return unet_check_launch("bn_relu_pool_fwd_kernel");
}

namespace { constexpr int POOL_BWD_MAX_BLOCKS = 256 * 8; }
extern "C" size_t unet_bn_relu_pool_max_parts(void) { return POOL_BWD_MAX_BLOCKS; }

extern "C" int32_t unet_bn_relu_pool_bwd(int32_t dtype, const void* y, const void* dpooled, const void* da_old, int32_t n,
                                         int32_t h, int32_t w, int32_t c, const float* scale, const float* shift,
                                         const float* mean, void* dz, float* partial, int32_t* n_parts, void* stream) {
  UNET_REQUIRE(y && dpooled && scale && shift && mean && dz && partial && n_parts, UNET_ERR_BAD_ARG,
               "unet_bn_relu_pool_bwd: null pointer");
  UNET_REQUIRE(n > 0 && h >= 2 && w >= 2 && unet_bn_relu_pool_supported(dtype, c), UNET_ERR_UNSUPPORTED,
               "unet_bn_relu_pool_bwd: c=%d h=%d w=%d", c, h, w);
  hipStream_t s = (hipStream_t)stream;
  ProfScope prof(UNET_K_POOL, 0.0, s, "bn_relu_pool_bwd_kernel");
  const long long total = (long long)n * ((h + 1) / 2) * ((w + 1) / 2) * (c / (dtype == UNET_BF16 ? 8 : 4));
  const int blocks = (int)std::min<long long>(cdiv64(total, 256), POOL_BWD_MAX_BLOCKS);
  const bool small = (long long)n * h * w * c < 0x7FFFFFFFLL;
  if (dtype == UNET_BF16) {
    if (small)
      hipLaunchKernelGGL((bn_relu_pool_bwd_kernel<bf16_t, int>), dim3(blocks), dim3(256), 0, s, (const bf16_t*)y,
                         (const bf16_t*)dpooled, (const bf16_t*)da_old, scale, shift, mean, (bf16_t*)dz, partial, n, h, w, c);
    else
      hipLaunchKernelGGL((bn_relu_pool_bwd_kernel<bf16_t, long long>), dim3(blocks), dim3(256), 0, s, (const bf16_t*)y,
                         (const bf16_t*)dpooled, (const bf16_t*)da_old, scale, shift, mean, (bf16_t*)dz, partial, n, h, w, c);
  } else {
    hipLaunchKernelGGL((bn_relu_pool_bwd_kernel<float, long long>), dim3(blocks), dim3(256), 0, s, (const float*)y,
                       (const float*)dpooled, (const float*)da_old, scale, shift, mean, (float*)dz, partial, n, h, w, c);
  }
  *n_parts = blocks;
  return unet_check_launch("bn_relu_pool_bwd_kernel");
}

extern "C" int32_t unet_upsample_bilinear2x_fwd(int32_t dtype, const void* x, int32_t n, int32_t h, int32_t w,
                                                int32_t c, void* y, void* stream) {
  UNET_REQUIRE(x && y, UNET_ERR_BAD_ARG, "unet_upsample_bilinear2x_fwd: null pointer");
  UNET_REQUIRE(n > 0 && h > 0 && w > 0 && h <= 32768 && w <= 32768 && c > 0 && c % 8 == 0, UNET_ERR_UNSUPPORTED,
               "unet_upsample_bilinear2x_fwd: dims");
  EW_DISPATCH("bilinear2x_fwd_kernel", bilinear2x_fwd_kernel, (long long)n * 4 * h * w * c, (const T*)x, (T*)y, n, h, w, c);
}

extern "C" int32_t unet_upsample_bilinear2x_bwd(int32_t dtype, const void* dy, int32_t n, int32_t h, int32_t w,
                                                int32_t c, void* dx, void* stream) {
  UNET_REQUIRE(dy && dx, UNET_ERR_BAD_ARG, "unet_upsample_bilinear2x_bwd: null pointer");
  UNET_REQUIRE(n > 0 && h > 0 && w > 0 && h <= 32768 && w <= 32768 && c > 0 && c % 8 == 0, UNET_ERR_UNSUPPORTED,
               "unet_upsample_bilinear2x_bwd: dims");
  EW_DISPATCH("bilinear2x_bwd_kernel", bilinear2x_bwd_kernel, (long long)n * h * w * c, (const T*)dy, (T*)dx, n, h, w, c);
}

namespace {

template <typename T>
__global__ void channel_scale_kernel(const T* __restrict__ x, const float* __restrict__ scale, T* __restrict__ y,
                                     long long hw, int C, long long total) {
  constexpr int PIECE = ET<T>::PIECE;
  const int G = C / PIECE;
  for (long long i = blockIdx.x * (long long)blockDim.x + threadIdx.x; i < total; i += (long long)gridDim.x * blockDim.x) {
    const int g = (int)(i % G);
    const long long n = i / G / hw;
    float v[PIECE];
    Vec<T>::load(x + i * PIECE, v);
#pragma unroll
    for (int j = 0; j < PIECE; ++j) v[j] *= scale[n * C + g * PIECE + j];
    Vec<T>::store(y + i * PIECE, v);
  }
}

__global__ __launch_bounds__(256) void anomaly_score_kernel(const float* __restrict__ recon, const float* __restrict__ image,
                                                           int C, long long hw, int l1, float* __restrict__ score,
                                                           float* __restrict__ part) {
  __shared__ float red[4];
  const int n = blockIdx.y;
  float acc = 0.f;
  for (long long q = blockIdx.x * 256LL + threadIdx.x; q < hw; q += (long long)gridDim.x * 256) {
    float s = 0.f;
    for (int c = 0; c < C; ++c) {
      const float d = recon[((long long)n * C + c) * hw + q] - image[((long long)n * C + c) * hw + q];
      s += l1 ? fabsf(d) : d * d;
    }
    s /= (float)C;
    score[(long long)n * hw + q] = s;
    acc += s;
  }
#pragma unroll
  for (int m = 32; m >= 1; m >>= 1) acc += __shfl_xor(acc, m);
  if ((threadIdx.x & 63) == 0) red[threadIdx.x >> 6] = acc;
  __syncthreads();
  if (threadIdx.x == 0) part[(size_t)n * gridDim.x + blockIdx.x] = (red[0] + red[1]) + (red[2] + red[3]);
}

__global__ void anomaly_score_finalize_kernel(const float* __restrict__ part, int N, int nb, long long hw,
                                              float* __restrict__ out) {
  const int n = blockIdx.x * blockDim.x + threadIdx.x;
  if (n >= N) return;
  double s = 0.0;
  for (int b = 0; b < nb; ++b) s += (double)part[(size_t)n * nb + b];
  out[n] = (float)(s / (double)hw);
}

}

extern "C" int32_t unet_channel_scale(int32_t dtype, const void* x, const float* scale, int32_t n, int64_t hw, int32_t c,
                                      void* y, void* stream) {
  UNET_REQUIRE(x && scale && y, UNET_ERR_BAD_ARG, "unet_channel_scale: null pointer");
  UNET_REQUIRE(n > 0 && hw > 0 && c > 0 && c % 8 == 0, UNET_ERR_UNSUPPORTED, "unet_channel_scale: c=%d", c);
  hipStream_t s = (hipStream_t)stream;
  ProfScope prof(UNET_K_POOL, 0.0, s);
  if (dtype == UNET_BF16) {
    const long long total = (long long)n * hw * c / 8;
    hipLaunchKernelGGL(channel_scale_kernel<bf16_t>, dim3(ew_blocks(total)), dim3(256), 0, s, (const bf16_t*)x, scale,
                       (bf16_t*)y, (long long)hw, c, total);
  } else {
    const long long total = (long long)n * hw * c / 4;
    hipLaunchKernelGGL(channel_scale_kernel<float>, dim3(ew_blocks(total)), dim3(256), 0, s, (const float*)x, scale,
                       (float*)y, (long long)hw, c, total);
  }
  return unet_check_launch("channel_scale_kernel");
}

extern "C" size_t unet_anomaly_score_workspace(int32_t n, int64_t hw) {
  (void)hw;
  return (size_t)n * 64 * sizeof(float);
}

extern "C" int32_t unet_anomaly_score(const float* recon, const float* image, int32_t n, int32_t c, int64_t hw,
                                      int32_t l1, float* score, float* image_score, void* workspace,
                                      size_t workspace_bytes, void* stream) {
  UNET_REQUIRE(recon && image && score && image_score && workspace, UNET_ERR_BAD_ARG, "unet_anomaly_score: null pointer");
  UNET_REQUIRE(n > 0 && c > 0 && hw > 0, UNET_ERR_BAD_ARG, "unet_anomaly_score: bad dims");
  UNET_REQUIRE(workspace_bytes >= unet_anomaly_score_workspace(n, hw), UNET_ERR_WORKSPACE, "unet_anomaly_score: workspace too small");
  hipStream_t s = (hipStream_t)stream;
  long long nb = cdiv64(hw, 256 * 4);
  if (nb > 64) nb = 64;
  ProfScope prof(UNET_K_LOSS, 0.0, s);
  hipLaunchKernelGGL(anomaly_score_kernel, dim3((unsigned)nb, n), dim3(256), 0, s, recon, image, c, (long long)hw, l1, score,
                     (float*)workspace);
  int32_t rc = unet_check_launch("anomaly_score_kernel");
  if (rc) return rc;
  hipLaunchKernelGGL(anomaly_score_finalize_kernel, dim3(cdiv(n, 256)), dim3(256), 0, s, (const float*)workspace, n, (int)nb,
                     (long long)hw, image_score);
  return unet_check_launch("anomaly_score_finalize_kernel");
}

namespace {
constexpr int ADAM_CHUNK = 4096;
__device__ __forceinline__ void adam_one(float& p, float g, float& m, float& v, float lr_bc1, float b1, float b2, float omb1,
                                         float omb2, float eps, float wd, float gscale, float bc2_sqrt, int decoupled) {
  float gr = g * gscale;
  if (!decoupled) gr = fmaf(wd, p, gr);
  m = b1 * m + omb1 * gr;
  v = b2 * v + omb2 * gr * gr;
  const float denom = sqrtf(v) / bc2_sqrt + eps;
  p -= lr_bc1 * (m / denom);
}
__global__ __launch_bounds__(256) void adam_multi_kernel(const unet_adam_desc* __restrict__ descs,
                                                         const unet_adam_chunk* __restrict__ chunks, float lr, float b1,
                                                         float b2, float omb1, float omb2, float eps, float wd,
                                                         float gscale, float bc1, float bc2_sqrt, int decoupled) {
  const unet_adam_chunk ck = chunks[blockIdx.x];
  const unet_adam_desc d = descs[ck.tensor];
  const long long begin = ck.first, end = begin + ADAM_CHUNK < d.n ? begin + ADAM_CHUNK : d.n;
  const float lr_bc1 = lr / bc1;
  const float decay = decoupled ? 1.f - lr * wd : 1.f;
  const long long vend = begin + ((end - begin) / 4) * 4;
  for (long long i = begin + threadIdx.x * 4LL; i < vend; i += 1024) {
    f32x4 pp = *reinterpret_cast<f32x4*>(d.p + i), gg = *reinterpret_cast<const f32x4*>(d.g + i);
    f32x4 mm = *reinterpret_cast<f32x4*>(d.m + i), vv = *reinterpret_cast<f32x4*>(d.v + i);
#pragma unroll
    for (int j = 0; j < 4; ++j) {
      float pj = pp[j] * decay, mj = mm[j], vj = vv[j];
      adam_one(pj, gg[j], mj, vj, lr_bc1, b1, b2, omb1, omb2, eps, wd, gscale, bc2_sqrt, decoupled);
      pp[j] = pj; mm[j] = mj; vv[j] = vj;
    }
    *reinterpret_cast<f32x4*>(d.p + i) = pp;
    *reinterpret_cast<f32x4*>(d.m + i) = mm;
    *reinterpret_cast<f32x4*>(d.v + i) = vv;
  }
  for (long long i = vend + threadIdx.x; i < end; i += 256) {
    float pp = d.p[i] * decay, mm = d.m[i], vv = d.v[i];
    adam_one(pp, d.g[i], mm, vv, lr_bc1, b1, b2, omb1, omb2, eps, wd, gscale, bc2_sqrt, decoupled);
    d.p[i] = pp; d.m[i] = mm; d.v[i] = vv;
  }
}
}

extern "C" int32_t unet_adam_chunk_elems(void) { return ADAM_CHUNK; }

extern "C" int32_t unet_adam_multi(const unet_adam_desc* descs, const unet_adam_chunk* chunks, int32_t n_chunks, float lr,
                                   double beta1, double beta2, float eps, float weight_decay, float grad_scale, int32_t step,
                                   int32_t decoupled, void* stream) {
  UNET_REQUIRE(descs && chunks && n_chunks > 0 && step >= 1, UNET_ERR_BAD_ARG, "unet_adam_multi: bad argument");
  const double bc1 = 1.0 - pow(beta1, (double)step);
  const double bc2 = 1.0 - pow(beta2, (double)step);
  hipStream_t s = (hipStream_t)stream;
  ProfScope prof(UNET_K_OTHER, 0.0, s, "adam_multi_kernel");
  hipLaunchKernelGGL(adam_multi_kernel, dim3((unsigned)n_chunks), dim3(256), 0, s, descs, chunks, lr, (float)beta1, (float)beta2,
                     (float)(1.0 - beta1), (float)(1.0 - beta2), eps, weight_decay, grad_scale, (float)bc1, (float)sqrt(bc2), decoupled);
  return unet_check_launch("adam_multi_kernel");
}

extern "C" int32_t unet_adam_step(float* param, const float* grad, float* exp_avg, float* exp_avg_sq, int64_t n,
                                  float lr, double beta1, double beta2, float eps, float weight_decay,
                                  float grad_scale, int32_t step, void* stream) {
  UNET_REQUIRE(param && grad && exp_avg && exp_avg_sq, UNET_ERR_BAD_ARG, "unet_adam_step: null pointer");
  UNET_REQUIRE(n > 0 && n % 4 == 0 && step >= 1, UNET_ERR_BAD_ARG, "unet_adam_step: n=%lld (must be a multiple of 4), step=%d",
               (long long)n, step);
  const double bc1 = 1.0 - pow(beta1, (double)step);
  const double bc2 = 1.0 - pow(beta2, (double)step);
  hipStream_t s = (hipStream_t)stream;
  ProfScope prof(UNET_K_OTHER, 0.0, s);
  hipLaunchKernelGGL(adam_kernel, dim3(ew_blocks(n / 4)), dim3(256), 0, s, param, grad, exp_avg, exp_avg_sq,
                     (long long)(n / 4), lr, (float)beta1, (float)beta2, (float)(1.0 - beta1), (float)(1.0 - beta2), eps, weight_decay, grad_scale, (float)bc1,
                     (float)sqrt(bc2));
  return unet_check_launch("adam_kernel");
}

namespace {
__global__ __launch_bounds__(256) void preprocess_u8_kernel(const unsigned char* __restrict__ src,
                                                            const unsigned char* __restrict__ flip,
                                                            float* __restrict__ dst, int N, int H, int W,
                                                            float m0, float m1, float m2, float s0, float s1, float s2) {
  const long long total = (long long)N * H * W;
  for (long long i = blockIdx.x * 256LL + threadIdx.x; i < total; i += (long long)gridDim.x * 256) {
    const int x = (int)(i % W);
    const long long r = i / W;
    const int y = (int)(r % H), n = (int)(r / H);
    const int xs = (flip && flip[n]) ? W - 1 - x : x;
    const unsigned char* p = src + (((long long)n * H + y) * W + xs) * 3;
    const long long plane = (long long)H * W;
    float* o = dst + (long long)n * 3 * plane + (long long)y * W + x;
    o[0] = ((float)p[0] / 255.f - m0) / s0;
    o[plane] = ((float)p[1] / 255.f - m1) / s1;
    o[2 * plane] = ((float)p[2] / 255.f - m2) / s2;
  }
}
}

extern "C" int32_t unet_preprocess_u8(const uint8_t* images_hwc, const uint8_t* flip, float* out_nchw, int32_t n, int32_t h,
                                      int32_t w, const float* mean3, const float* std3, void* stream) {
  UNET_REQUIRE(images_hwc && out_nchw && mean3 && std3, UNET_ERR_BAD_ARG, "unet_preprocess_u8: null pointer");
  UNET_REQUIRE(n > 0 && h > 0 && w > 0, UNET_ERR_BAD_ARG, "unet_preprocess_u8: bad dims");
  const long long total = (long long)n * h * w;
  const int blocks = (int)std::min<long long>(cdiv64(total, 256), 256 * 16);
  hipLaunchKernelGGL(preprocess_u8_kernel, dim3(blocks), dim3(256), 0, (hipStream_t)stream, images_hwc, flip, out_nchw, n, h, w,
                     mean3[0], mean3[1], mean3[2], std3[0], std3[1], std3[2]);
  return unet_check_launch("preprocess_u8_kernel");
}
```

tiaozhanbei_unet_amd/csrc/head.hip:

```cpp
#include "common.h"

namespace {

constexpr int MAXCO = 8;

__device__ __forceinline__ void split_pixel(long long p, long long hw, long long& n, long long& q) {
  if (p < (1LL << 31) && hw < (1LL << 31)) {
    const unsigned nn = (unsigned)p / (unsigned)hw;
    n = nn;
    q = (unsigned)p - nn * (unsigned)hw;
  } else {
    n = p / hw;
    q = p - n * hw;
  }
}

template <typename T, int TPP, int CO, bool BN = false>
__global__ __launch_bounds__(256) void head_fwd_kernel(const T* __restrict__ x, long long pixels, long long hw,
                                                       int Cin, const float* __restrict__ w,
                                                       const float* __restrict__ b, int sigm,
                                                       float* __restrict__ out,
                                                       const float* __restrict__ bn_scale = nullptr,
                                                       const float* __restrict__ bn_shift = nullptr) {
  constexpr int PIECE = ET<T>::PIECE;
  constexpr int PPW = 64 / TPP, S = TPP;
  constexpr int SB = S < 8 ? S : 8;
  const int lane = threadIdx.x & 63, wave = threadIdx.x >> 6;
  const int g = lane % TPP, sub = lane / TPP;
  float wr[CO][PIECE];
#pragma unroll
  for (int co = 0; co < CO; ++co)
#pragma unroll
    for (int j = 0; j < PIECE; ++j) wr[co][j] = w[co * Cin + g * PIECE + j];
  float sc[BN ? PIECE : 1], sh[BN ? PIECE : 1];
  if constexpr (BN) {
#pragma unroll
    for (int j = 0; j < PIECE; ++j) { sc[j] = bn_scale[g * PIECE + j]; sh[j] = bn_shift[g * PIECE + j]; }
  }
  const long long nw = (long long)gridDim.x * 4;
  for (long long c = blockIdx.x * 4LL + wave; c * 64 < pixels; c += nw) {
    const long long base = c * 64;
    float res[CO];
#pragma unroll
    for (int co = 0; co < CO; ++co) res[co] = 0.f;
#pragma unroll 1
    for (int s0 = 0; s0 < S; s0 += SB) {
      float v[SB][PIECE];
#pragma unroll
      for (int i = 0; i < SB; ++i) {
        const long long p = base + (s0 + i) * PPW + sub;
#pragma unroll
        for (int j = 0; j < PIECE; ++j) v[i][j] = 0.f;
        if (p < pixels) Vec<T>::load(x + p * Cin + g * PIECE, v[i]);
      }
      if constexpr (BN) {
#pragma unroll
        for (int i = 0; i < SB; ++i)
#pragma unroll
          for (int j = 0; j < PIECE; ++j)
            v[i][j] = ET<T>::to_f(ET<T>::from_f(fmaxf(fmaf(v[i][j], sc[j], sh[j]), 0.f)));
      }
      if constexpr (TPP == 8) {
        static_assert(SB == 8 && S == 8, "one batch");
        const bool b0 = g & 1, b1 = g & 2, b2 = g & 4;
#pragma unroll
        for (int co = 0; co < CO; ++co) {
          float a[8];
#pragma unroll
          for (int i = 0; i < 8; ++i) {
            a[i] = 0.f;
#pragma unroll
            for (int j = 0; j < PIECE; ++j) a[i] = fmaf(v[i][j], wr[co][j], a[i]);
          }
          float h4[4], h2[2];
#pragma unroll
          for (int k = 0; k < 4; ++k) {
            const float keep = b0 ? a[2 * k + 1] : a[2 * k], send = b0 ? a[2 * k] : a[2 * k + 1];
            h4[k] = keep + __shfl_xor(send, 1);
          }
#pragma unroll
          for (int k = 0; k < 2; ++k) {
            const float keep = b1 ? h4[2 * k + 1] : h4[2 * k], send = b1 ? h4[2 * k] : h4[2 * k + 1];
            h2[k] = keep + __shfl_xor(send, 2);
          }
          const float keep = b2 ? h2[1] : h2[0], send = b2 ? h2[0] : h2[1];
          res[co] = keep + __shfl_xor(send, 4);
        }
      } else {
#pragma unroll
      for (int i = 0; i < SB; ++i) {
        const int s = s0 + i;
        float acc[CO];
#pragma unroll
        for (int co = 0; co < CO; ++co) {
          acc[co] = 0.f;
#pragma unroll
          for (int j = 0; j < PIECE; ++j) acc[co] = fmaf(v[i][j], wr[co][j], acc[co]);
        }
#pragma unroll
        for (int m = 1; m < TPP; m <<= 1)
#pragma unroll
          for (int co = 0; co < CO; ++co) acc[co] += __shfl_xor(acc[co], m);
#pragma unroll
        for (int co = 0; co < CO; ++co) {
          const float t = __shfl(acc[co], (lane % PPW) * TPP);
          if (lane / PPW == s) res[co] = t;
        }
      }
      }
    }
    const long long p = base + (TPP == 8 ? g * PPW + sub : lane);
    if (p < pixels) {
      long long n, q;
      split_pixel(p, hw, n, q);
#pragma unroll
      for (int co = 0; co < CO; ++co) {
        float r = res[co] + b[co];
        if (sigm) r = 1.f / (1.f + expf(-r));
        out[(n * CO + co) * hw + q] = r;
      }
    }
  }
}

template <typename T, int TPP, int CO, bool BN = false>
__global__ __launch_bounds__(256) void head_bwd_kernel(const T* __restrict__ x, const float* __restrict__ out,
                                                       const float* __restrict__ dout, long long pixels,
                                                       long long hw, int Cin, const float* __restrict__ w,
                                                       int sigm, T* __restrict__ dx, float* __restrict__ part,
                                                       const float* __restrict__ bn_scale = nullptr,
                                                       const float* __restrict__ bn_shift = nullptr,
                                                       const float* __restrict__ bn_mean = nullptr,
                                                       float* __restrict__ bn_part = nullptr) {
  constexpr int PIECE = ET<T>::PIECE;
  constexpr int PPW = 64 / TPP, S = TPP;
  __shared__ float red[4][MAXCO * 129];
  const int lane = threadIdx.x & 63, wave = threadIdx.x >> 6;
  const int g = lane % TPP, sub = lane / TPP;
  float wr[CO][PIECE];
#pragma unroll
  for (int co = 0; co < CO; ++co)
#pragma unroll
    for (int j = 0; j < PIECE; ++j) wr[co][j] = w[co * Cin + g * PIECE + j];
  float dwacc[CO][PIECE], dbacc[CO];
#pragma unroll
  for (int co = 0; co < CO; ++co) {
    dbacc[co] = 0.f;
#pragma unroll
    for (int j = 0; j < PIECE; ++j) dwacc[co][j] = 0.f;
  }
  float sc[BN ? PIECE : 1], sh[BN ? PIECE : 1], mu[BN ? PIECE : 1], bs0[BN ? PIECE : 1], bs1[BN ? PIECE : 1];
  if constexpr (BN) {
#pragma unroll
    for (int j = 0; j < PIECE; ++j) {
      sc[j] = bn_scale[g * PIECE + j]; sh[j] = bn_shift[g * PIECE + j]; mu[j] = bn_mean[g * PIECE + j];
      bs0[j] = 0.f; bs1[j] = 0.f;
    }
  }
  constexpr int SB = S < 8 ? S : 8;
  const long long nw = (long long)gridDim.x * 4;
  for (long long c = blockIdx.x * 4LL + wave; c * 64 < pixels; c += nw) {
    const long long base = c * 64;
    float dl[CO];
#pragma unroll
    for (int co = 0; co < CO; ++co) dl[co] = 0.f;
    {
      const long long p = base + lane;
      if (p < pixels) {
        long long n, q;
        split_pixel(p, hw, n, q);
#pragma unroll
        for (int co = 0; co < CO; ++co) {
          float d = dout[(n * CO + co) * hw + q];
          if (sigm) { const float o = out[(n * CO + co) * hw + q]; d *= o * (1.f - o); }
          dl[co] = d;
          dbacc[co] += d;
        }
      }
    }
#pragma unroll 1
    for (int s0 = 0; s0 < S; s0 += SB) {
      float v[SB][PIECE];
#pragma unroll
      for (int i = 0; i < SB; ++i) {
        const long long p = base + (s0 + i) * PPW + sub;
#pragma unroll
        for (int j = 0; j < PIECE; ++j) v[i][j] = 0.f;
        if (p < pixels) Vec<T>::load(x + p * Cin + g * PIECE, v[i]);
      }
#pragma unroll
      for (int i = 0; i < SB; ++i) {
        const int s = s0 + i;
        const long long p = base + s * PPW + sub;
        float ds[CO], d[PIECE];
#pragma unroll
        for (int co = 0; co < CO; ++co) ds[co] = __shfl(dl[co], s * PPW + sub);
#pragma unroll
        for (int j = 0; j < PIECE; ++j) d[j] = 0.f;
        float av[PIECE];
        bool on[PIECE];
#pragma unroll
        for (int j = 0; j < PIECE; ++j) {
          if constexpr (BN) {
            const float z = fmaf(v[i][j], sc[j], sh[j]);
            on[j] = z > 0.f;
            av[j] = ET<T>::to_f(ET<T>::from_f(fmaxf(z, 0.f)));
          } else {
            on[j] = true;
            av[j] = v[i][j];
          }
        }
#pragma unroll
        for (int co = 0; co < CO; ++co)
#pragma unroll
          for (int j = 0; j < PIECE; ++j) {
            d[j] = fmaf(ds[co], wr[co][j], d[j]);
            dwacc[co][j] = fmaf(ds[co], av[j], dwacc[co][j]);
          }
        if constexpr (BN) {
#pragma unroll
          for (int j = 0; j < PIECE; ++j) {
            d[j] = ET<T>::to_f(ET<T>::from_f(on[j] ? d[j] : 0.f));
            bs0[j] += d[j];
            bs1[j] = fmaf(d[j], v[i][j] - mu[j], bs1[j]);
          }
        }
        if (p < pixels) Vec<T>::store(dx + p * Cin + g * PIECE, d);
      }
    }
  }
#pragma unroll
  for (int m = TPP; m < 64; m <<= 1)
#pragma unroll
    for (int co = 0; co < CO; ++co)
#pragma unroll
      for (int j = 0; j < PIECE; ++j) dwacc[co][j] += __shfl_xor(dwacc[co][j], m);
#pragma unroll
  for (int m = 1; m < 64; m <<= 1)
#pragma unroll
    for (int co = 0; co < CO; ++co) dbacc[co] += __shfl_xor(dbacc[co], m);
  const int stride = Cin + 1;
  if (lane < TPP) {
#pragma unroll
    for (int co = 0; co < CO; ++co) {
#pragma unroll
      for (int j = 0; j < PIECE; ++j) red[wave][co * stride + lane * PIECE + j] = dwacc[co][j];
      if (lane == 0) red[wave][co * stride + Cin] = dbacc[co];
    }
  }
  __syncthreads();
  for (int i = threadIdx.x; i < CO * stride; i += 256)
    part[(size_t)blockIdx.x * CO * stride + i] = (red[0][i] + red[1][i]) + (red[2][i] + red[3][i]);
  if constexpr (BN) {
#pragma unroll
    for (int m = TPP; m < 64; m <<= 1)
#pragma unroll
      for (int j = 0; j < PIECE; ++j) {
        bs0[j] += __shfl_xor(bs0[j], m);
        bs1[j] += __shfl_xor(bs1[j], m);
      }
    __syncthreads();
    if (lane < TPP) {
#pragma unroll
      for (int j = 0; j < PIECE; ++j) {
        red[wave][lane * PIECE + j] = bs0[j];
        red[wave][Cin + lane * PIECE + j] = bs1[j];
      }
    }
    __syncthreads();
    for (int i = threadIdx.x; i < 2 * Cin; i += 256)
      bn_part[(size_t)blockIdx.x * 2 * Cin + i] = (red[0][i] + red[1][i]) + (red[2][i] + red[3][i]);
  }
}

__global__ __launch_bounds__(256) void head_bwd_finalize_kernel(const float* __restrict__ part, int nblocks, int CO,
                                                                int Cin, float* __restrict__ dw,
                                                                float* __restrict__ db) {
  const int stride = Cin + 1;
  const int lane = threadIdx.x & 63, i = blockIdx.x * 4 + (threadIdx.x >> 6);
  if (i >= CO * stride) return;
  double s = 0.0;
  for (int k = lane; k < nblocks; k += 64) s += (double)part[(size_t)k * CO * stride + i];
#pragma unroll
  for (int m = 32; m >= 1; m >>= 1) s += __shfl_xor(s, m);
  if (lane == 0) {
    const int co = i / stride, c = i % stride;
    if (c < Cin) dw[co * Cin + c] = (float)s;
    else db[co] = (float)s;
  }
}

template <typename T, int CO, bool BN>
__global__ __launch_bounds__(256) void head_bwd_tile_kernel(const T* __restrict__ x, const float* __restrict__ out,
                                                            const float* __restrict__ dout, long long pixels,
                                                            long long hw, const float* __restrict__ w, int sigm,
                                                            T* __restrict__ dx, float* __restrict__ part,
                                                            const float* __restrict__ bn_scale,
                                                            const float* __restrict__ bn_shift,
                                                            const float* __restrict__ bn_mean,
                                                            float* __restrict__ bn_part) {
  constexpr int CIN = 64, ES = ET<T>::ES;
  constexpr int ROW = CIN * ES;
  constexpr int TILE = 64 * ROW;
  constexpr int NLD = TILE / 1024;
  extern __shared__ __attribute__((aligned(16))) char smem[];
  const int lane = threadIdx.x & 63, wave = threadIdx.x >> 6;
  char* const tile = smem + wave * (TILE + CO * 256);
  float* const dlt = reinterpret_cast<float*>(tile + TILE);
  const int c2 = lane & 31, ph = lane >> 5;
  const int ch0 = sizeof(T) == 2 ? 2 * c2 : c2, ch1 = sizeof(T) == 2 ? 2 * c2 + 1 : c2 + 32;
  float wr[CO][2], dwacc[CO][2], dbacc[CO];
#pragma unroll
  for (int co = 0; co < CO; ++co) {
    wr[co][0] = w[co * CIN + ch0]; wr[co][1] = w[co * CIN + ch1];
    dwacc[co][0] = dwacc[co][1] = 0.f; dbacc[co] = 0.f;
  }
  float sc[2] = {1.f, 1.f}, sh[2] = {0.f, 0.f}, mu[2] = {0.f, 0.f}, bs0[2] = {0.f, 0.f}, bs1[2] = {0.f, 0.f};
  if constexpr (BN) {
#pragma unroll
    for (int j = 0; j < 2; ++j) {
      const int ch = j ? ch1 : ch0;
      sc[j] = bn_scale[ch]; sh[j] = bn_shift[ch]; mu[j] = bn_mean[ch];
    }
  }
  const long long nw = (long long)gridDim.x * 4;
  for (long long c = blockIdx.x * 4LL + wave; c * 64 < pixels; c += nw) {
    const long long base = c * 64;
    u32x4 ld[NLD];
#pragma unroll
    for (int i = 0; i < NLD; ++i) {
      const int q = i * 64 + lane;
      const long long p = base + q / (ROW / 16);
      ld[i] = u32x4{0u, 0u, 0u, 0u};
      if (p < pixels) ld[i] = *reinterpret_cast<const u32x4*>(reinterpret_cast<const char*>(x) + base * ROW + (size_t)q * 16);
    }
    {
      const long long p = base + lane;
      float dl[CO];
#pragma unroll
      for (int co = 0; co < CO; ++co) dl[co] = 0.f;
      if (p < pixels) {
        long long n, q;
        split_pixel(p, hw, n, q);
#pragma unroll
        for (int co = 0; co < CO; ++co) {
          float d = dout[(n * CO + co) * hw + q];
          if (sigm) { const float o = out[(n * CO + co) * hw + q]; d *= o * (1.f - o); }
          dl[co] = d;
          dbacc[co] += d;
        }
      }
#pragma unroll
      for (int co = 0; co < CO; ++co) dlt[co * 64 + lane] = dl[co];
    }
#pragma unroll
    for (int i = 0; i < NLD; ++i) *reinterpret_cast<u32x4*>(tile + (i * 64 + lane) * 16) = ld[i];
    __builtin_amdgcn_wave_barrier();
    asm volatile("s_waitcnt lgkmcnt(0)" ::: "memory");
#pragma unroll 4
    for (int k = 0; k < 32; ++k) {
      const int p = 2 * k + ph;
      float v[2];
      if constexpr (sizeof(T) == 2) {
        const unsigned u = *reinterpret_cast<const unsigned*>(tile + p * ROW + c2 * 4);
        v[0] = __builtin_bit_cast(float, u << 16);
        v[1] = __builtin_bit_cast(float, u & 0xFFFF0000u);
      } else {
        v[0] = *reinterpret_cast<const float*>(tile + p * ROW + ch0 * 4);
        v[1] = *reinterpret_cast<const float*>(tile + p * ROW + ch1 * 4);
      }
      float ds[CO];
#pragma unroll
      for (int co = 0; co < CO; ++co) ds[co] = dlt[co * 64 + p];
      float d[2];
#pragma unroll
      for (int j = 0; j < 2; ++j) {
        float av = v[j];
        bool on = true;
        if constexpr (BN) {
          const float z = fmaf(v[j], sc[j], sh[j]);
          on = z > 0.f;
          av = ET<T>::to_f(ET<T>::from_f(fmaxf(z, 0.f)));
        }
        float t = 0.f;
#pragma unroll
        for (int co = 0; co < CO; ++co) {
          t = fmaf(ds[co], wr[co][j], t);
          dwacc[co][j] = fmaf(ds[co], av, dwacc[co][j]);
        }
        if constexpr (BN) {
          t = ET<T>::to_f(ET<T>::from_f(on ? t : 0.f));
          bs0[j] += t;
          bs1[j] = fmaf(t, v[j] - mu[j], bs1[j]);
        }
        d[j] = t;
      }
      if constexpr (sizeof(T) == 2) {
        const bf16_t d0 = (bf16_t)d[0], d1 = (bf16_t)d[1];
        const unsigned u = (unsigned)__builtin_bit_cast(unsigned short, d0) | ((unsigned)__builtin_bit_cast(unsigned short, d1) << 16);
        *reinterpret_cast<unsigned*>(tile + p * ROW + c2 * 4) = u;
      } else {
        *reinterpret_cast<float*>(tile + p * ROW + ch0 * 4) = d[0];
        *reinterpret_cast<float*>(tile + p * ROW + ch1 * 4) = d[1];
      }
    }
    __builtin_amdgcn_wave_barrier();
    asm volatile("s_waitcnt lgkmcnt(0)" ::: "memory");
#pragma unroll
    for (int i = 0; i < NLD; ++i) {
      const int q = i * 64 + lane;
      const long long p = base + q / (ROW / 16);
      const u32x4 r = *reinterpret_cast<const u32x4*>(tile + q * 16);
      if (p < pixels) *reinterpret_cast<u32x4*>(reinterpret_cast<char*>(dx) + base * ROW + (size_t)q * 16) = r;
    }
    __builtin_amdgcn_wave_barrier();
    asm volatile("s_waitcnt lgkmcnt(0)" ::: "memory");
  }
#pragma unroll
  for (int co = 0; co < CO; ++co) {
#pragma unroll
    for (int j = 0; j < 2; ++j) dwacc[co][j] += __shfl_xor(dwacc[co][j], 32);
#pragma unroll
    for (int m = 1; m < 64; m <<= 1) dbacc[co] += __shfl_xor(dbacc[co], m);
  }
#pragma unroll
  for (int j = 0; j < 2; ++j) { bs0[j] += __shfl_xor(bs0[j], 32); bs1[j] += __shfl_xor(bs1[j], 32); }
  __syncthreads();
  float* red = reinterpret_cast<float*>(smem);
  constexpr int stride = CIN + 1, RW = CO * stride + 2 * CIN;
  if (ph == 0) {
#pragma unroll
    for (int co = 0; co < CO; ++co) {
      red[wave * RW + co * stride + ch0] = dwacc[co][0];
      red[wave * RW + co * stride + ch1] = dwacc[co][1];
      if (lane == 0) red[wave * RW + co * stride + CIN] = dbacc[co];
    }
#pragma unroll
    for (int j = 0; j < 2; ++j) {
      red[wave * RW + CO * stride + (j ? ch1 : ch0)] = bs0[j];
      red[wave * RW + CO * stride + CIN + (j ? ch1 : ch0)] = bs1[j];
    }
  }
  __syncthreads();
  for (int i = threadIdx.x; i < CO * stride; i += 256)
    part[(size_t)blockIdx.x * CO * stride + i] = (red[i] + red[RW + i]) + (red[2 * RW + i] + red[3 * RW + i]);
  if constexpr (BN) {
    for (int i = threadIdx.x; i < 2 * CIN; i += 256) {
      const int o = CO * stride + i;
      bn_part[(size_t)blockIdx.x * 2 * CIN + i] = (red[o] + red[RW + o]) + (red[2 * RW + o] + red[3 * RW + o]);
    }
  }
}

template <typename T, int CO, bool BN>
int32_t launch_head_bwd_tile(const void* x, const float* out, const float* dout, long long pixels, long long hw,
                             const float* w, int sigm, void* dx, float* part, const float* bn_scale,
                             const float* bn_shift, const float* bn_mean, float* bn_part, int nb, hipStream_t s) {
  constexpr int TILE = 64 * 64 * ET<T>::ES;
  constexpr int LDS = 4 * (TILE + CO * 256);
  static_assert(LDS >= 4 * (CO * 65 + 128) * 4, "reduction scratch fits the tile area");
  auto kern = head_bwd_tile_kernel<T, CO, BN>;
  unet_set_max_lds(reinterpret_cast<const void*>(kern), LDS);
  hipLaunchKernelGGL(kern, dim3(nb), dim3(256), LDS, s, (const T*)x, out, dout, pixels, hw, w, sigm, (T*)dx, part,
                     bn_scale, bn_shift, bn_mean, bn_part);
  return unet_check_launch("head_bwd_tile_kernel");
}

inline int head_blocks(long long pixels, int tpp) {
  (void)tpp;
  long long b = cdiv64(pixels, 256 * 4);
  if (b > 1024) b = 1024;
  if (b < 1) b = 1;
  return (int)b;
}

template <typename T>
int tpp_of(int c_in) { return c_in / ET<T>::PIECE; }

}

#define HEAD_CO_SWITCH(...)                                  \
  switch (c_out) {                                          \
    case 1: { constexpr int CO = 1; __VA_ARGS__; } break;          \
    case 2: { constexpr int CO = 2; __VA_ARGS__; } break;          \
    case 3: { constexpr int CO = 3; __VA_ARGS__; } break;          \
    case 4: { constexpr int CO = 4; __VA_ARGS__; } break;          \
    default: { constexpr int CO = 8; __VA_ARGS__; } break;         \
  }
#define HEAD_TPP_SWITCH(T, tpp, ...)                        \
  switch (tpp) {                                            \
    case 4: { constexpr int TPP = 4; HEAD_CO_SWITCH(__VA_ARGS__); } break;   \
    case 8: { constexpr int TPP = 8; HEAD_CO_SWITCH(__VA_ARGS__); } break;   \
    case 16: { constexpr int TPP = 16; HEAD_CO_SWITCH(__VA_ARGS__); } break; \
    case 32: { constexpr int TPP = 32; HEAD_CO_SWITCH(__VA_ARGS__); } break; \
    default:                                                \
      unet_set_error("head: c_in %d unsupported", c_in);    \
      return UNET_ERR_UNSUPPORTED;                          \
  }

extern "C" int32_t unet_head_fwd(int32_t dtype, const void* x, int32_t n, int32_t h, int32_t w, int32_t c_in,
                                 const float* weight, const float* bias, int32_t c_out, int32_t sigmoid,
                                 float* out, void* stream) {
  UNET_REQUIRE(x && weight && bias && out, UNET_ERR_BAD_ARG, "unet_head_fwd: null pointer");
  UNET_REQUIRE(n > 0 && h > 0 && w > 0, UNET_ERR_BAD_ARG, "unet_head_fwd: bad dims");
  UNET_REQUIRE(c_out >= 1 && c_out <= MAXCO && c_in <= 128 && (c_in == 32 || c_in == 64 || c_in == 128), UNET_ERR_UNSUPPORTED,
               "unet_head_fwd: %d -> %d channels unsupported (c_out <= 8, c_in in {32,64,128})", c_in, c_out);
  UNET_REQUIRE(c_out <= c_in / (dtype == UNET_BF16 ? 8 : 4), UNET_ERR_UNSUPPORTED, "unet_head_fwd: c_out %d too wide for c_in %d", c_out, c_in);
  hipStream_t s = (hipStream_t)stream;
  const long long pixels = (long long)n * h * w, hw = (long long)h * w;
  ProfScope prof(UNET_K_HEAD, 2.0 * pixels * c_in * c_out, s);
  if (dtype == UNET_BF16) {
    const int tpp = tpp_of<bf16_t>(c_in);
    HEAD_TPP_SWITCH(bf16_t, tpp, hipLaunchKernelGGL((head_fwd_kernel<bf16_t, TPP, CO>), dim3(head_blocks(pixels, TPP)), dim3(256), 0, s,
                    (const bf16_t*)x, pixels, hw, c_in, weight, bias, sigmoid, out));
  } else {
    const int tpp = tpp_of<float>(c_in);
    HEAD_TPP_SWITCH(float, tpp, hipLaunchKernelGGL((head_fwd_kernel<float, TPP, CO>), dim3(head_blocks(pixels, TPP)), dim3(256), 0, s,
                    (const float*)x, pixels, hw, c_in, weight, bias, sigmoid, out));
  }
  return unet_check_launch("head_fwd_kernel");
}

extern "C" size_t unet_head_bwd_workspace(int32_t n, int32_t h, int32_t w, int32_t c_in, int32_t c_out) {
  (void)n; (void)h; (void)w;
  return (size_t)2048 * c_out * (c_in + 1) * sizeof(float);
}

extern "C" int32_t unet_head_bwd(int32_t dtype, const void* x, const float* out, const float* dout, int32_t n,
                                 int32_t h, int32_t w, int32_t c_in, const float* weight, int32_t c_out,
                                 int32_t sigmoid, void* dx, float* dweight, float* dbias, void* workspace,
                                 size_t workspace_bytes, void* stream) {
  UNET_REQUIRE(x && dout && weight && dx && dweight && dbias && workspace && (out || !sigmoid), UNET_ERR_BAD_ARG,
               "unet_head_bwd: null pointer");
  UNET_REQUIRE(n > 0 && h > 0 && w > 0, UNET_ERR_BAD_ARG, "unet_head_bwd: bad dims");
  UNET_REQUIRE(c_out >= 1 && c_out <= MAXCO && c_in <= 128 && (c_in == 32 || c_in == 64 || c_in == 128), UNET_ERR_UNSUPPORTED,
               "unet_head_bwd: %d -> %d channels unsupported", c_in, c_out);
  UNET_REQUIRE(workspace_bytes >= unet_head_bwd_workspace(n, h, w, c_in, c_out), UNET_ERR_WORKSPACE,
               "unet_head_bwd: workspace too small");
  hipStream_t s = (hipStream_t)stream;
  const long long pixels = (long long)n * h * w, hw = (long long)h * w;
  ProfScope prof(UNET_K_HEAD, 4.0 * pixels * c_in * c_out, s);
  int nb = 0;
  if (c_in == 64 && (dtype == UNET_BF16 || dtype == UNET_F32)) {
    nb = head_blocks(pixels, 8);
    int32_t rc = UNET_OK;
    if (dtype == UNET_BF16) {
      HEAD_CO_SWITCH(rc = (launch_head_bwd_tile<bf16_t, CO, false>(x, out, dout, pixels, hw, weight, sigmoid, dx, (float*)workspace,
                                                                 nullptr, nullptr, nullptr, nullptr, nb, s)));
    } else {
      HEAD_CO_SWITCH(rc = (launch_head_bwd_tile<float, CO, false>(x, out, dout, pixels, hw, weight, sigmoid, dx, (float*)workspace,
                                                                nullptr, nullptr, nullptr, nullptr, nb, s)));
    }
    if (rc) return rc;
  } else if (dtype == UNET_BF16) {
    const int tpp = tpp_of<bf16_t>(c_in);
    nb = head_blocks(pixels, tpp);
    HEAD_TPP_SWITCH(bf16_t, tpp, hipLaunchKernelGGL((head_bwd_kernel<bf16_t, TPP, CO>), dim3(nb), dim3(256), 0, s,
                    (const bf16_t*)x, out, dout, pixels, hw, c_in, weight, sigmoid, (bf16_t*)dx, (float*)workspace));
  } else {
    const int tpp = tpp_of<float>(c_in);
    nb = head_blocks(pixels, tpp);
    HEAD_TPP_SWITCH(float, tpp, hipLaunchKernelGGL((head_bwd_kernel<float, TPP, CO>), dim3(nb), dim3(256), 0, s,
                    (const float*)x, out, dout, pixels, hw, c_in, weight, sigmoid, (float*)dx, (float*)workspace));
  }
  int32_t rc = unet_check_launch("head_bwd_kernel");
  if (rc) return rc;
  hipLaunchKernelGGL(head_bwd_finalize_kernel, dim3(cdiv(c_out * (c_in + 1), 4)), dim3(256), 0, s,
                     (const float*)workspace, nb, c_out, c_in, dweight, dbias);
  return unet_check_launch("head_bwd_finalize_kernel");
}

extern "C" int32_t unet_head_bnrelu_fwd(int32_t dtype, const void* y, int32_t n, int32_t h, int32_t w, int32_t c_in,
                                        const float* bn_scale, const float* bn_shift, const float* weight,
                                        const float* bias, int32_t c_out, int32_t sigmoid, float* out, void* stream) {
  UNET_REQUIRE(y && bn_scale && bn_shift && weight && bias && out, UNET_ERR_BAD_ARG, "unet_head_bnrelu_fwd: null pointer");
  UNET_REQUIRE(n > 0 && h > 0 && w > 0, UNET_ERR_BAD_ARG, "unet_head_bnrelu_fwd: bad dims");
  UNET_REQUIRE(c_out >= 1 && c_out <= MAXCO && (c_in == 32 || c_in == 64 || c_in == 128), UNET_ERR_UNSUPPORTED,
               "unet_head_bnrelu_fwd: %d -> %d channels unsupported (c_out <= 8, c_in in {32,64,128})", c_in, c_out);
  UNET_REQUIRE(c_out <= c_in / (dtype == UNET_BF16 ? 8 : 4), UNET_ERR_UNSUPPORTED,
               "unet_head_bnrelu_fwd: c_out %d too wide for c_in %d", c_out, c_in);
  hipStream_t s = (hipStream_t)stream;
  const long long pixels = (long long)n * h * w, hw = (long long)h * w;
  ProfScope prof(UNET_K_HEAD, 2.0 * pixels * c_in * c_out, s);
  if (dtype == UNET_BF16) {
    const int tpp = tpp_of<bf16_t>(c_in);
    HEAD_TPP_SWITCH(bf16_t, tpp, hipLaunchKernelGGL((head_fwd_kernel<bf16_t, TPP, CO, true>), dim3(head_blocks(pixels, TPP)),
                    dim3(256), 0, s, (const bf16_t*)y, pixels, hw, c_in, weight, bias, sigmoid, out, bn_scale, bn_shift));
  } else if (dtype == UNET_F32) {
    const int tpp = tpp_of<float>(c_in);
    HEAD_TPP_SWITCH(float, tpp, hipLaunchKernelGGL((head_fwd_kernel<float, TPP, CO, true>), dim3(head_blocks(pixels, TPP)),
                    dim3(256), 0, s, (const float*)y, pixels, hw, c_in, weight, bias, sigmoid, out, bn_scale, bn_shift));
  } else {
    unet_set_error("unet_head_bnrelu_fwd: dtype %d", dtype);
    return UNET_ERR_BAD_ARG;
  }
  return unet_check_launch("head_fwd_kernel<BN>");
}

extern "C" size_t unet_head_bnrelu_max_parts(void) { return 1024; }

extern "C" int32_t unet_head_bnrelu_bwd(int32_t dtype, const void* y, const float* bn_scale, const float* bn_shift,
                                        const float* bn_mean, const float* out, const float* dout, int32_t n, int32_t h,
                                        int32_t w, int32_t c_in, const float* weight, int32_t c_out, int32_t sigmoid,
                                        void* dz, float* dweight, float* dbias, float* bn_partial, int32_t* n_parts,
                                        void* workspace, size_t workspace_bytes, void* stream) {
  UNET_REQUIRE(y && bn_scale && bn_shift && bn_mean && dout && weight && dz && dweight && dbias && bn_partial && n_parts &&
               workspace && (out || !sigmoid), UNET_ERR_BAD_ARG, "unet_head_bnrelu_bwd: null pointer");
  UNET_REQUIRE(n > 0 && h > 0 && w > 0, UNET_ERR_BAD_ARG, "unet_head_bnrelu_bwd: bad dims");
  UNET_REQUIRE(c_out >= 1 && c_out <= MAXCO && (c_in == 32 || c_in == 64 || c_in == 128), UNET_ERR_UNSUPPORTED,
               "unet_head_bnrelu_bwd: %d -> %d channels unsupported", c_in, c_out);
  UNET_REQUIRE(workspace_bytes >= unet_head_bwd_workspace(n, h, w, c_in, c_out), UNET_ERR_WORKSPACE,
               "unet_head_bnrelu_bwd: workspace too small");
  hipStream_t s = (hipStream_t)stream;
  const long long pixels = (long long)n * h * w, hw = (long long)h * w;
  ProfScope prof(UNET_K_HEAD, 4.0 * pixels * c_in * c_out, s);
  int nb = 0;
  if (c_in == 64 && (dtype == UNET_BF16 || dtype == UNET_F32)) {
    nb = head_blocks(pixels, 8);
    int32_t rc = UNET_OK;
    if (dtype == UNET_BF16) {
      HEAD_CO_SWITCH(rc = (launch_head_bwd_tile<bf16_t, CO, true>(y, out, dout, pixels, hw, weight, sigmoid, dz, (float*)workspace,
                                                                bn_scale, bn_shift, bn_mean, bn_partial, nb, s)));
    } else {
      HEAD_CO_SWITCH(rc = (launch_head_bwd_tile<float, CO, true>(y, out, dout, pixels, hw, weight, sigmoid, dz, (float*)workspace,
                                                               bn_scale, bn_shift, bn_mean, bn_partial, nb, s)));
    }
    if (rc) return rc;
  } else if (dtype == UNET_BF16) {
    const int tpp = tpp_of<bf16_t>(c_in);
    nb = head_blocks(pixels, tpp);
    HEAD_TPP_SWITCH(bf16_t, tpp, hipLaunchKernelGGL((head_bwd_kernel<bf16_t, TPP, CO, true>), dim3(nb), dim3(256), 0, s,
                    (const bf16_t*)y, out, dout, pixels, hw, c_in, weight, sigmoid, (bf16_t*)dz, (float*)workspace,
                    bn_scale, bn_shift, bn_mean, bn_partial));
  } else if (dtype == UNET_F32) {
    const int tpp = tpp_of<float>(c_in);
    nb = head_blocks(pixels, tpp);
    HEAD_TPP_SWITCH(float, tpp, hipLaunchKernelGGL((head_bwd_kernel<float, TPP, CO, true>), dim3(nb), dim3(256), 0, s,
                    (const float*)y, out, dout, pixels, hw, c_in, weight, sigmoid, (float*)dz, (float*)workspace,
                    bn_scale, bn_shift, bn_mean, bn_partial));
  } else {
    unet_set_error("unet_head_bnrelu_bwd: dtype %d", dtype);
    return UNET_ERR_BAD_ARG;
  }
  int32_t rc = unet_check_launch("head_bwd_kernel<BN>");
  if (rc) return rc;
  *n_parts = nb;
  hipLaunchKernelGGL(head_bwd_finalize_kernel, dim3(cdiv(c_out * (c_in + 1), 4)), dim3(256), 0, s,
                     (const float*)workspace, nb, c_out, c_in, dweight, dbias);
  return unet_check_launch("head_bwd_finalize_kernel");
}
```

tiaozhanbei_unet_amd/ops.py:

```python
from __future__ import annotations

import ctypes as C
from typing import Optional, Tuple

import torch

from . import _lib as L

_DT = {torch.float32: L.UNET_F32, torch.bfloat16: L.UNET_BF16}
BN_EPS = 1e-5


def _stream():
    return C.c_void_p(torch.cuda.current_stream().cuda_stream)


def _ptr(t: Optional[torch.Tensor]):
    return C.c_void_p(0 if t is None else t.data_ptr())


def _require_cuda(*ts):
    for t in ts:
        if t is not None and not t.is_cuda:
            raise RuntimeError(
# ... 273 lines not shown

    def get(self, weight, mode, rows, k, split=0):
        s_ = self.slots.get((id(weight), mode))
        if s_ is not None and s_[0] is not None and s_[1] == rows and s_[2] == k and s_[3] == weight._version \
                and s_[4] == split:
            return s_[0]
        return None


_active_packs = None


def set_active_packs(cache):
    global _active_packs
    _active_packs = cache


def packed(weight, mode, rows, k, dtype, split=0):
    if _active_packs is not None and _active_packs.dtype == dtype:
        hit = _active_packs.get(weight, mode, rows, k, split)
        if hit is not None:
            return hit
    return pack_weight(weight, mode, rows, k, dtype, split)


class GradSink:

    __slots__ = ("buf", "event")

    def __init__(self):
        self.buf = None
        self.event = None

    def begin(self, dev):
        if self.buf is None:
            return False
        cur = torch.cuda.current_stream(dev)
        if self.event is not None:
            cur.wait_event(self.event)
        self.buf.record_stream(cur)
        return True

    def done(self, buf, dev):
        self.buf = buf
        self.event = torch.cuda.Event()
        self.event.record(torch.cuda.current_stream(dev))

    def collect(self, grad, dev):
        if self.buf is not None:
            if grad.data_ptr() != self.buf.data_ptr():
                raise RuntimeError("GradSink: autograd delivered a different tensor than the shared gradient buffer")
            cur = torch.cuda.current_stream(dev)
            if self.event is not None:
                cur.wait_event(self.event)
            self.buf.record_stream(cur)
        self.buf = None
        self.event = None


SHARE_SKIP_GRADS = __import__("os").environ.get("UNET_GRAD_SINK", "1") != "0"


def share_grad(t: torch.Tensor) -> torch.Tensor:
    if SHARE_SKIP_GRADS and t.grad_fn is not None and hasattr(t.grad_fn, "out_sink"):
        sink = GradSink()
        t.grad_fn.out_sink = sink
        t._unet_sink = sink
    return t


FOLD_EVAL_BN = __import__("os").environ.get("UNET_FOLD_BN", "1") != "0"
_folded = {}
_train_generation = 0


def _folded_pack(weight, gamma, beta, running_mean, running_var, co, ctot, dtype, rows=None, split=0):
    stamp = (_train_generation, weight._version, gamma._version, beta._version, running_mean._version,
             running_var._version, running_mean.data_ptr(), running_var.data_ptr(), weight.data_ptr())
    import weakref
    slot = _folded.get(id(weight))
    if slot is None or slot[0]() is not weight:
        key = id(weight)
        slot = (weakref.ref(weight, lambda _r, k=key: _folded.pop(k, None)), {})
        _folded[key] = slot
    per_weight = slot[1]
    rows = co if rows is None else rows
    key = (dtype, ctot) if (rows == co and not split) else (dtype, ctot, rows, split)
    hit = per_weight.get(key)
    if hit is not None and hit[0] == stamp:
        return hit[1]
    lib, st, dev = L.lib(), _stream(), weight.device
    if key != (dtype, ctot):
        g, b, rm, rv = _NarrowBn(gamma, beta, running_mean, running_var, rows).params
        ss = torch.empty((2, rows), dtype=torch.float32, device=dev)
        L.check(lib.unet_bn_eval_coeffs(rows, _ptr(g), _ptr(b), _ptr(rm), _ptr(rv), BN_EPS, _ptr(ss[0]), _ptr(ss[1]), st),
                "unet_bn_eval_coeffs")
        wq = torch.empty(9 * rows * ctot, dtype=dtype, device=dev)
        L.check(lib.unet_pack_conv_weight_folded_seg(_ptr(weight.detach()), _ptr(ss[0]), _ptr(wq), co, weight.shape[1],
                                                     rows, ctot, split, _DT[dtype], st), "unet_pack_conv_weight_folded_seg")
        per_weight[key] = (stamp, (wq, ss[1]))
        return wq, ss[1]
    ss = torch.empty((2, co), dtype=torch.float32, device=dev)
    L.check(lib.unet_bn_eval_coeffs(co, _ptr(gamma), _ptr(beta), _ptr(running_mean), _ptr(running_var), BN_EPS,
                                    _ptr(ss[0]), _ptr(ss[1]), st), "unet_bn_eval_coeffs")
    wq = torch.empty(9 * co * ctot, dtype=dtype, device=dev)
    L.check(lib.unet_pack_conv_weight_folded(_ptr(weight.detach()), _ptr(ss[0]), _ptr(wq), co, weight.shape[1], co, ctot,
                                             _DT[dtype], st), "unet_pack_conv_weight_folded")
    per_weight[(dtype, ctot)] = (stamp, (wq, ss[1]))
    return wq, ss[1]


FUSE_BN_BWD = __import__("os").environ.get("UNET_FUSE_BN_BWD", "1") != "0"
FUSE_BN_HEAD = __import__("os").environ.get("UNET_FUSE_BN_HEAD", "1") != "0"
FUSE_BN_POOL = __import__("os").environ.get("UNET_FUSE_BN_POOL", "1") != "0"
FUSE_BN_CONVT = __import__("os").environ.get("UNET_FUSE_BN_CONVT", "1") != "0"


class BnLink:

    __slots__ = ("y", "coef", "partial", "n_parts", "dz_ptr")

    def __init__(self):
        self.y = None
        self.coef = None
        self.partial = None
        self.n_parts = 0
        self.dz_ptr = 0


def _bn_stats_conv(lib, dt, n, h, w, src, wp, co, y, gamma, beta, running_mean, running_var, momentum, coef, dev, st):
    cap = lib.unet_conv3x3_stats_max_parts(n, h, w)
    part = _workspace(cap * 2 * co * 4, dev)
    nparts = C.c_int32(0)
    L.check(lib.unet_conv3x3_stats(dt, n, h, w, src, _ptr(wp), co, _ptr(y), _ptr(part), C.byref(nparts), st),
            "unet_conv3x3_stats")
    L.check(lib.unet_bn_finalize_partials(_ptr(part), nparts.value, n * h * w, co, _ptr(gamma), _ptr(beta),
                                          _ptr(running_mean), _ptr(running_var), momentum, BN_EPS,
                                          _ptr(coef[0]), _ptr(coef[1]), _ptr(coef[2]), _ptr(coef[3]), st),
            "unet_bn_finalize_partials")


def _bn_relu_backward(lib, dt, dtype, da, y, gamma, coef, link, out_sink, dev, st, frozen=False, beta_key=None,
                      gamma_key=None):
    n, co, h, w = y.shape
    pixels = n * h * w
    dgb = (grad_out(gamma.shape, dev, gamma.data_ptr() if gamma_key is None else gamma_key),
           grad_out(gamma.shape, dev, beta_key))
    if link is not None and link.dz_ptr and link.dz_ptr == da.data_ptr() and da.dtype == dtype and _is_nhwc(da):
        dy = da
        ws = _workspace(3 * co * 4, dev)
        L.check(lib.unet_bn_bwd_premasked(dt, _ptr(da), _ptr(y), pixels, co, _ptr(gamma), _ptr(coef[0]),
                                          _ptr(coef[1]), _ptr(link.partial), link.n_parts, _ptr(dgb[0]),
                                          _ptr(dgb[1]), _ptr(dy), _ptr(ws), ws.numel(), st), "unet_bn_bwd_premasked")
    else:
        if link is not None and link.dz_ptr:
            raise RuntimeError("conv-BN-ReLU: the premasked gradient of a linked activation did not arrive unchanged "
                               "(the activation has a second consumer?)")
        if out_sink is not None:
            out_sink.collect(da, dev)
        da = _as_nhwc(da, dtype)
        dy = _nhwc_empty(n, co, h, w, dtype, dev)
        ws = _workspace(lib.unet_bn_workspace(pixels, co), dev)
        fn = lib.unet_bn_relu_bwd_frozen if frozen else lib.unet_bn_relu_bwd
        L.check(fn(dt, _ptr(da), _ptr(y), pixels, co, _ptr(gamma), _ptr(coef[0]), _ptr(coef[1]),
                   _ptr(coef[2]), _ptr(coef[3]), _ptr(dgb[0]), _ptr(dgb[1]), _ptr(dy),
                   _ptr(ws), ws.numel(), st), "unet_bn_relu_bwd")
    if link is not None:
        link.y = link.coef = link.partial = None
        link.dz_ptr = 0
    return dy, dgb


class ConvBnRelu(torch.autograd.Function):

    @staticmethod
    def forward(ctx, x0, x1, weight, gamma, beta, running_mean, running_var, training, momentum, fold=False,
                in_link=None, out_link=None, head_w=None, head_b=None, head_sigmoid=False, pool=False, split=0):
        _require_cuda(x0, weight)
        dtype = x0.dtype
        dt = _DT[dtype]
        n, c0, h, w = x0.shape
        c1 = 0 if x1 is None else x1.shape[1]
        oy = ox = 0
        if x1 is not None:
            dy_, dx_ = h - x1.shape[2], w - x1.shape[3]
            if dy_ < 0 or dx_ < 0:
                raise ValueError("Up: the skip tensor must be at least as large as the up-sampled one")
            oy, ox = dy_ // 2, dx_ // 2
        co_p, ci = weight.shape[0], weight.shape[1]
        co = _pad64(co_p)
        ctot = c0 + c1
        split = int(split or 0)
        if split:
            if x1 is None or c0 != _pad64(split) or ctot != seg_cols(ci, split):
                raise ValueError(f"conv weight expects {split} + {ci - split} input channels, activations carry "
                                 f"{c0} + {c1} (padded)")
        elif not (ci <= ctot < ci + 64):
            raise ValueError(f"conv weight expects {ci} input channels, activations carry {ctot}")
        if (head_w is not None or pool) and not training:
            raise RuntimeError("ConvBnRelu: the fused head / pool are training-path fusions")
        lib, st, dev = L.lib(), _stream(), x0.device
        bn_param = (gamma, beta, running_mean, running_var)
        narrow = co != co_p
        y = _nhwc_empty(n, co, h, w, dtype, dev)
        src = _views([(x0, 0, 0), None if x1 is None else (x1, oy, ox)])
        pixels = n * h * w
        coef = torch.empty((4, co), dtype=torch.float32, device=dev)
        fold = bool(fold) and FOLD_EVAL_BN and not training
        nb = None
        if not fold:
            wp = packed(weight, L.PACK_CONV_FWD, co, ctot, dtype, split)
            if narrow:
                nb = _NarrowBn(gamma, beta, running_mean, running_var, co)
                gamma, beta, running_mean, running_var = nb.params
        if training:
            global _train_generation
            _train_generation += 1
            _bn_stats_conv(lib, dt, n, h, w, src, wp, co, y, gamma, beta, running_mean, running_var, momentum, coef,
                           dev, st)
            if nb is not None:
                nb.write_back()
        elif fold:
            if narrow or split:
                wf = _folded_pack(weight, *bn_param, co_p, ctot, dtype, rows=co, split=split)
            else:
                wf = _folded_pack(weight, gamma, beta, running_mean, running_var, co, ctot, dtype)
            L.check(lib.unet_conv3x3_bias_relu(dt, n, h, w, src, _ptr(wf[0]), co, _ptr(y), _ptr(wf[1]), 1, st),
                    "unet_conv3x3_bias_relu")
            return y
        else:
            dst = _views([(y, 0, 0), None])
            L.check(lib.unet_conv3x3(dt, n, h, w, src, _ptr(wp), co, dst, co, 0, L.K_CONV_FWD, st), "unet_conv3x3")
            L.check(lib.unet_bn_eval_coeffs4(co, _ptr(gamma), _ptr(beta), _ptr(running_mean), _ptr(running_var),
                                             BN_EPS, _ptr(coef[0]), _ptr(coef[1]), _ptr(coef[2]), _ptr(coef[3]), st),
                    "unet_bn_eval_coeffs4")
        ctx.geom = (oy, ox, training)
        ctx.keys = (weight.data_ptr(), bn_param[1].data_ptr(), 0 if head_w is None else head_w.data_ptr(),
                    0 if head_b is None else head_b.data_ptr())
        ctx.widths = (co_p, split, bn_param[0].data_ptr())
        ctx.sink0 = getattr(x0, "_unet_sink", None)
        ctx.out_sink = None
        ctx.in_link = in_link if (in_link is not None and in_link.y is not None and x1 is None) else None
        ctx.out_link = None
        ctx.head = None
        ctx.pool = False
        if pool:
            a = _nhwc_empty(n, co, h, w, dtype, dev)
            pooled = _nhwc_empty(n, co, h // 2, w // 2, dtype, dev)
            L.check(lib.unet_bn_relu_pool_fwd(dt, _ptr(y), n, h, w, co, _ptr(coef[2]), _ptr(coef[3]), _ptr(a),
                                              _ptr(pooled), st), "unet_bn_relu_pool_fwd")
            ctx.save_for_backward(x0, x1, y, weight, gamma, coef)
            ctx.pool = True
            ctx.set_materialize_grads(False)
            return a, pooled
        if head_w is not None:
            hc = head_w.shape[0]
            if narrow:
                hw_p = torch.empty((hc, co, 1, 1), dtype=torch.float32, device=dev)
                _remap([(L.REMAP_PAD, head_w.detach(), hw_p, hc, co_p, 1, hc, co, 0)])
                head_w = hw_p
            out = torch.empty((n, hc, h, w), dtype=torch.float32, device=dev)
            L.check(lib.unet_head_bnrelu_fwd(dt, _ptr(y), n, h, w, co, _ptr(coef[2]), _ptr(coef[3]), _ptr(head_w),
                                             _ptr(head_b), hc, int(head_sigmoid), _ptr(out), st), "unet_head_bnrelu_fwd")
            ctx.save_for_backward(x0, x1, y, weight, gamma, coef, head_w, out)
            ctx.head = bool(head_sigmoid)
            return out
        a = _nhwc_empty(n, co, h, w, dtype, dev)
        L.check(lib.unet_bn_relu_apply(dt, _ptr(y), pixels, co, _ptr(coef[2]), _ptr(coef[3]), _ptr(a), st),
                "unet_bn_relu_apply")
        ctx.save_for_backward(x0, x1, y, weight, gamma, coef)
        if out_link is not None and training:
            out_link.y, out_link.coef, out_link.dz_ptr = y, coef, 0
            ctx.out_link = out_link
        return a

    @staticmethod
    def backward(ctx, da, dpooled=None):
        saved = ctx.saved_tensors
        x0, x1, y, weight, gamma, coef = saved[:6]
        oy, ox, training = ctx.geom
        dtype = x0.dtype
        dt = _DT[dtype]
        n, c0, h, w = x0.shape
        co, ci = y.shape[1], weight.shape[1]
        co_p, split, gamma_key = ctx.widths
        narrow = co != co_p
        gkey, bkey, hkey = (0, 0, 0) if narrow else (gamma_key, ctx.keys[1], ctx.keys[2])
        ctot = c0 + (0 if x1 is None else x1.shape[1])
        lib, st, dev = L.lib(), _stream(), x0.device
        pixels = n * h * w
        dhw = dhb = None
        link = ctx.out_link
        if ctx.head is not None:
            head_w, out = saved[6], saved[7]
            hc = head_w.shape[0]
            dout = da.contiguous().float()
            dy = _nhwc_empty(n, co, h, w, dtype, dev)
            dgb = (grad_out(gamma.shape, dev, gkey), grad_out(gamma.shape, dev, bkey))
            dhw = grad_out(head_w.shape, dev, hkey)
            dhb = grad_out((hc,), dev, ctx.keys[3])
            part = torch.empty((lib.unet_head_bnrelu_max_parts(), 2, co), dtype=torch.float32, device=dev)
            nparts = C.c_int32(0)
            ws = _workspace(lib.unet_head_bwd_workspace(n, h, w, co, hc), dev)
            L.check(lib.unet_head_bnrelu_bwd(dt, _ptr(y), _ptr(coef[2]), _ptr(coef[3]), _ptr(coef[0]), _ptr(out),
                                             _ptr(dout), n, h, w, co, _ptr(head_w), hc, int(ctx.head), _ptr(dy),
                                             _ptr(dhw), _ptr(dhb), _ptr(part), C.byref(nparts), _ptr(ws), ws.numel(),
                                             st), "unet_head_bnrelu_bwd")
            ws = _workspace(3 * co * 4, dev)
            L.check(lib.unet_bn_bwd_premasked(dt, _ptr(dy), _ptr(y), pixels, co, _ptr(gamma), _ptr(coef[0]),
                                              _ptr(coef[1]), _ptr(part), nparts.value, _ptr(dgb[0]), _ptr(dgb[1]),
                                              _ptr(dy), _ptr(ws), ws.numel(), st), "unet_bn_bwd_premasked")
        elif ctx.pool and dpooled is not None:
            own = False
            if da is not None:
                if ctx.out_sink is not None and ctx.out_sink.buf is not None and \
                        da.data_ptr() == ctx.out_sink.buf.data_ptr():
                    own = True
                if ctx.out_sink is not None:
                    ctx.out_sink.collect(da, dev)
                da = _as_nhwc(da, dtype)
            dpooled = _as_nhwc(dpooled, dtype)
            dy = da if own else _nhwc_empty(n, co, h, w, dtype, dev)
            part = torch.empty((lib.unet_bn_relu_pool_max_parts(), 2, co), dtype=torch.float32, device=dev)
            nparts = C.c_int32(0)
            L.check(lib.unet_bn_relu_pool_bwd(dt, _ptr(y), _ptr(dpooled), _ptr(da), n, h, w, co, _ptr(coef[2]),
                                              _ptr(coef[3]), _ptr(coef[0]), _ptr(dy), _ptr(part), C.byref(nparts), st),
                    "unet_bn_relu_pool_bwd")
            dgb = (grad_out(gamma.shape, dev, gkey), grad_out(gamma.shape, dev, bkey))
            ws = _workspace(3 * co * 4, dev)
            L.check(lib.unet_bn_bwd_premasked(dt, _ptr(dy), _ptr(y), pixels, co, _ptr(gamma), _ptr(coef[0]),
                                              _ptr(coef[1]), _ptr(part), nparts.value, _ptr(dgb[0]), _ptr(dgb[1]),
                                              _ptr(dy), _ptr(ws), ws.numel(), st), "unet_bn_bwd_premasked")
        else:
            if da is None:
                da = torch.zeros_like(y)
            dy, dgb = _bn_relu_backward(lib, dt, dtype, da, y, gamma, coef, link, ctx.out_sink, dev, st,
                                        frozen=not training, beta_key=bkey, gamma_key=gkey)
        src = _views([(x0, 0, 0), None if x1 is None else (x1, oy, ox)])
        dw = None
        if ctx.needs_input_grad[2]:
            ci_k = ctot if split else ci
            dw = torch.empty((co, ci_k, 3, 3), dtype=torch.float32, device=dev) if (narrow or split) else \
                grad_out(weight.shape, dev, ctx.keys[0])
            need = lib.unet_conv3x3_wgrad_workspace(n, h, w, ctot, co)
            ws2 = _workspace(need, dev)
            L.check(lib.unet_conv3x3_wgrad(dt, n, h, w, src, _ptr(dy), co, _ptr(dw), ci_k, _ptr(ws2), ws2.numel(), st),
                    "unet_conv3x3_wgrad")
        dx0 = dx1 = None
        if ctx.needs_input_grad[0] or (x1 is not None and ctx.needs_input_grad[1]):
            wp = packed(weight, L.PACK_CONV_DGRAD, ctot, co, dtype, split)
            sink = ctx.sink0
            ilink = ctx.in_link if (FUSE_BN_BWD and sink is None and x1 is None) else None
            if ilink is not None and ilink.y is not None and \
                    lib.unet_conv3x3_dgrad_bnrelu_supported(dt, n, h, w, co, c0):
                dx0 = _nhwc_empty(n, c0, h, w, dtype, dev)
                cap = lib.unet_conv3x3_stats_max_parts(n, h, w)
                part = torch.empty((cap, 2, c0), dtype=torch.float32, device=dev)
                nparts = C.c_int32(0)
                pc = ilink.coef
                L.check(lib.unet_conv3x3_dgrad_bnrelu(dt, n, h, w, _ptr(dy), co, _ptr(wp), c0, _ptr(ilink.y),
                                                      _ptr(pc[2]), _ptr(pc[3]), _ptr(pc[0]), _ptr(dx0), _ptr(part),
                                                      C.byref(nparts), st), "unet_conv3x3_dgrad_bnrelu")
                ilink.partial, ilink.n_parts, ilink.dz_ptr = part, nparts.value, dx0.data_ptr()
            else:
                fan_in = sink is not None and sink.begin(dev)
                dx0 = sink.buf if fan_in else _nhwc_empty(n, c0, h, w, dtype, dev)
                if x1 is not None:
                    dx1 = _nhwc_empty(*x1.shape, dtype, dev)
                dsrc = _views([(dy, 0, 0), None])
                ddst = _views([(dx0, 0, 0), None if x1 is None else (dx1, oy, ox)])
                L.check(lib.unet_conv3x3(dt, n, h, w, dsrc, _ptr(wp), ctot, ddst, c0, 1 if fan_in else 0,
                                         L.K_CONV_DGRAD, st), "unet_conv3x3(dgrad)")
                if sink is not None:
                    sink.done(dx0, dev)
                    if fan_in:
                        dx0 = None
        if narrow or split:
            items = []
            if dw is not None:
                dw, dw_pad = grad_out(weight.shape, dev, ctx.keys[0]), dw
                items.append((L.REMAP_UNPAD, dw_pad, dw, co_p, ci, 9, co, dw_pad.shape[1], split))
            if narrow:
                dgb_pad, dgb = dgb, (grad_out((co_p,), dev, gamma_key), grad_out((co_p,), dev, ctx.keys[1]))
                items += [_vec_item(L.REMAP_UNPAD, dgb_pad[0], dgb[0], co_p, co),
                          _vec_item(L.REMAP_UNPAD, dgb_pad[1], dgb[1], co_p, co)]
                if dhw is not None:
                    hc = dhw.shape[0]
                    dhw, dhw_pad = grad_out((hc, co_p, 1, 1), dev, ctx.keys[2]), dhw
                    items.append((L.REMAP_UNPAD, dhw_pad, dhw, hc, co_p, 1, hc, co, 0))
            if items:
                _remap(items)
        return dx0, dx1, dw, dgb[0], dgb[1], None, None, None, None, None, None, None, dhw, dhb, None, None, None


class FirstConvBnRelu(torch.autograd.Function):

    @staticmethod
    def forward(ctx, x, weight, gamma, beta, running_mean, running_var, training, momentum, out_link=None):
        _require_cuda(x, weight)
        x = x.contiguous().float()
        n, ci, h, w = x.shape
        co_p = weight.shape[0]
        co = _pad64(co_p)
        dtype = torch.bfloat16
        lib, st, dev = L.lib(), _stream(), x.device
        y = _nhwc_empty(n, co, h, w, dtype, dev)
        pixels = n * h * w
        coef = torch.empty((4, co), dtype=torch.float32, device=dev)
        wq = weight.detach().contiguous()
        ctx.keys = (weight.data_ptr(), beta.data_ptr(), gamma.data_ptr())
        nb = None
        if co != co_p:
            wq_p = torch.empty((co, ci, 3, 3), dtype=torch.float32, device=dev)
            nb = _NarrowBn(gamma, beta, running_mean, running_var, co,
                           extra=[(L.REMAP_PAD, wq, wq_p, co_p, ci, 9, co, ci, 0)])
            wq = wq_p
            gamma, beta, running_mean, running_var = nb.params
        if training:
            cap = lib.unet_conv3x3_stats_max_parts(n, h, w)
            part = _workspace(cap * 2 * co * 4, dev)
            nparts = C.c_int32(0)
            L.check(lib.unet_conv3x3_first_stats(n, h, w, _ptr(x), ci, _ptr(wq), _ptr(y), _ptr(part), C.byref(nparts), st),
                    "unet_conv3x3_first_stats")
            L.check(lib.unet_bn_finalize_partials(_ptr(part), nparts.value, pixels, co, _ptr(gamma), _ptr(beta),
                                                  _ptr(running_mean), _ptr(running_var), momentum, BN_EPS,
                                                  _ptr(coef[0]), _ptr(coef[1]), _ptr(coef[2]), _ptr(coef[3]), st),
                    "unet_bn_finalize_partials")
            if nb is not None:
                nb.write_back()
        else:
            L.check(lib.unet_conv3x3_first_stats(n, h, w, _ptr(x), ci, _ptr(wq), _ptr(y), None, None, st),
                    "unet_conv3x3_first_stats")
            L.check(lib.unet_bn_eval_coeffs4(co, _ptr(gamma), _ptr(beta), _ptr(running_mean), _ptr(running_var),
                                             BN_EPS, _ptr(coef[0]), _ptr(coef[1]), _ptr(coef[2]), _ptr(coef[3]), st),
                    "unet_bn_eval_coeffs4")
        a = _nhwc_empty(n, co, h, w, dtype, dev)
        L.check(lib.unet_bn_relu_apply(_DT[dtype], _ptr(y), pixels, co, _ptr(coef[2]), _ptr(coef[3]), _ptr(a), st),
                "unet_bn_relu_apply")
        ctx.save_for_backward(x, y, weight, gamma, coef)
        ctx.training = training
        ctx.out_sink = None
        ctx.out_link = None
        if out_link is not None and training:
            out_link.y, out_link.coef, out_link.dz_ptr = y, coef, 0
            ctx.out_link = out_link
        return a

    @staticmethod
    def backward(ctx, da):
        x, y, weight, gamma, coef = ctx.saved_tensors
        dtype = torch.bfloat16
        dt = _DT[dtype]
        n, ci, h, w = x.shape
        co, co_p = y.shape[1], weight.shape[0]
        narrow = co != co_p
        gkey, bkey = (0, 0) if narrow else (ctx.keys[2], ctx.keys[1])
        lib, st, dev = L.lib(), _stream(), x.device
        link = ctx.out_link
        dw, dgb = None, None
        if FUSE_FIRST_BN_BWD and link is not None and link.dz_ptr and link.dz_ptr == da.data_ptr() and da.dtype == dtype \
                and _is_nhwc(da) and ctx.training and ctx.needs_input_grad[1]:
            dgb = (grad_out(gamma.shape, dev, gkey), grad_out(gamma.shape, dev, bkey))
            cf = torch.empty(3 * co, dtype=torch.float32, device=dev)
            L.check(lib.unet_bn_bwd_premasked(dt, None, None, n * h * w, co, _ptr(gamma), _ptr(coef[0]), _ptr(coef[1]),
                                              _ptr(link.partial), link.n_parts, _ptr(dgb[0]), _ptr(dgb[1]), None, _ptr(cf),
                                              cf.numel() * 4, st), "unet_bn_bwd_premasked(coefficients)")
            link.y = link.coef = link.partial = None
            link.dz_ptr = 0
            dw = torch.empty((co, ci, 3, 3), dtype=torch.float32, device=dev) if narrow else \
                grad_out(weight.shape, dev, ctx.keys[0])
            ws2 = _workspace(lib.unet_conv3x3_first_wgrad_workspace(n, h, w), dev)
            L.check(lib.unet_conv3x3_first_wgrad_bn(n, h, w, _ptr(x), ci, _ptr(da), _ptr(y), _ptr(cf), _ptr(dw), _ptr(ws2),
                                                    ws2.numel(), st), "unet_conv3x3_first_wgrad_bn")
        else:
            dy, dgb = _bn_relu_backward(lib, dt, dtype, da, y, gamma, coef, ctx.out_link, ctx.out_sink, dev, st,
                                        frozen=not ctx.training, beta_key=bkey, gamma_key=gkey)
            if ctx.needs_input_grad[1]:
                dw = torch.empty((co, ci, 3, 3), dtype=torch.float32, device=dev) if narrow else \
                    grad_out(weight.shape, dev, ctx.keys[0])
                need = lib.unet_conv3x3_first_wgrad_workspace(n, h, w)
                ws2 = _workspace(need, dev)
                L.check(lib.unet_conv3x3_first_wgrad(n, h, w, _ptr(x), ci, _ptr(dy), _ptr(dw), _ptr(ws2), ws2.numel(), st),
                        "unet_conv3x3_first_wgrad")
        if narrow:
            dgb_pad, dgb = dgb, (grad_out((co_p,), dev, ctx.keys[2]), grad_out((co_p,), dev, ctx.keys[1]))
            items = [_vec_item(L.REMAP_UNPAD, dgb_pad[0], dgb[0], co_p, co),
                     _vec_item(L.REMAP_UNPAD, dgb_pad[1], dgb[1], co_p, co)]
            if dw is not None:
                dw, dw_pad = grad_out(weight.shape, dev, ctx.keys[0]), dw
                items.append((L.REMAP_UNPAD, dw_pad, dw, co_p, ci, 9, co, ci, 0))
            _remap(items)
        return None, dw, dgb[0], dgb[1], None, None, None, None, None


FIRST_LAYER_KERNELS = __import__("os").environ.get("UNET_FIRST_LAYER", "1") != "0"
FUSE_FIRST_BN_BWD = __import__("os").environ.get("UNET_FUSE_FIRST_BN", "1") != "0"


def first_layer_ok(x: torch.Tensor, conv, dtype) -> bool:
    return (FIRST_LAYER_KERNELS and dtype == torch.bfloat16 and x.dim() == 4 and x.dtype == torch.float32
            and not x.requires_grad and x.shape[1] == conv.in_channels
            and bool(L.lib().unet_conv3x3_first_supported(conv.in_channels, _pad64(conv.out_channels), x.shape[2],
                                                          x.shape[3])))


class ChannelDropout(torch.autograd.Function):

    @staticmethod
    def forward(ctx, x, noise):
        _require_cuda(x, noise)
        n, c, h, w = x.shape
        y = _nhwc_empty(n, c, h, w, x.dtype, x.device)
        L.check(L.lib().unet_channel_scale(_DT[x.dtype], _ptr(x), _ptr(noise), n, h * w, c, _ptr(y), _stream()),
                "unet_channel_scale")
        ctx.save_for_backward(noise)
        return y

    @staticmethod
    def backward(ctx, dy):
        (noise,) = ctx.saved_tensors
        n, c, h, w = dy.shape
        dy = _as_nhwc(dy, dy.dtype)
        dx = _nhwc_empty(n, c, h, w, dy.dtype, dy.device)
        L.check(L.lib().unet_channel_scale(_DT[dy.dtype], _ptr(dy), _ptr(noise), n, h * w, c, _ptr(dx), _stream()),
                "unet_channel_scale")
        return dx, None


def anomaly_score(reconstruction, original, l1=False):
    _require_cuda(reconstruction, original)
    r = reconstruction.detach().contiguous().float()
    o = original.detach().contiguous().float()
    n, c = r.shape[0], r.shape[1]
    hw = int(r.numel() // (n * c))
    score = torch.empty((n,) + tuple(r.shape[2:]), dtype=torch.float32, device=r.device)
    img = torch.empty(n, dtype=torch.float32, device=r.device)
    lib = L.lib()
    ws = _workspace(lib.unet_anomaly_score_workspace(n, hw), r.device)
    L.check(lib.unet_anomaly_score(_ptr(r), _ptr(o), n, c, hw, 1 if l1 else 0, _ptr(score), _ptr(img), _ptr(ws), ws.numel(),
                                   _stream()), "unet_anomaly_score")
    return score, img


class MaxPool2(torch.autograd.Function):

    @staticmethod
    def forward(ctx, x):
        _require_cuda(x)
        n, c, h, w = x.shape
        if h < 2 or w < 2:
            raise ValueError("MaxPool2d(2) needs at least 2x2 pixels")
        y = _nhwc_empty(n, c, h // 2, w // 2, x.dtype, x.device)
        L.check(L.lib().unet_maxpool2_fwd(_DT[x.dtype], _ptr(x), n, h, w, c, _ptr(y), _stream()), "unet_maxpool2_fwd")
        ctx.save_for_backward(x)
        ctx.sink = getattr(x, "_unet_sink", None)
        return y

    @staticmethod
    def backward(ctx, dy):
        (x,) = ctx.saved_tensors
        n, c, h, w = x.shape
        dy = _as_nhwc(dy, x.dtype)
        sink = ctx.sink
        fan_in = sink is not None and sink.begin(x.device)
        dx = sink.buf if fan_in else _nhwc_empty(n, c, h, w, x.dtype, x.device)
        L.check(L.lib().unet_maxpool2_bwd(_DT[x.dtype], _ptr(x), _ptr(dy), n, h, w, c, _ptr(dx), 1 if fan_in else 0,
                                          _stream()), "unet_maxpool2_bwd")
        if sink is not None:
            sink.done(dx, x.device)
            if fan_in:
                return None
        return dx


class ConvT2x2(torch.autograd.Function):

    @staticmethod
    def forward(ctx, x, weight, bias, in_link=None):
        _require_cuda(x, weight)
        n, ci, h, w = x.shape
        co = _pad64(weight.shape[1])
        dtype = x.dtype
        wp = packed(weight, L.PACK_CONVT_FWD, co, ci, dtype)
        if co != weight.shape[1]:
            bias_p = torch.empty(co, dtype=torch.float32, device=x.device)
            _remap([_vec_item(L.REMAP_PAD, bias.detach(), bias_p, weight.shape[1], co)])
            bias = bias_p
        y = _nhwc_empty(n, co, 2 * h, 2 * w, dtype, x.device)
        L.check(L.lib().unet_convt2x2_fwd(_DT[dtype], n, h, w, _ptr(x), ci, _ptr(wp), _ptr(bias), _ptr(y), co,
                                          _stream()), "unet_convt2x2_fwd")
        ctx.save_for_backward(x, weight)
        ctx.keys = (weight.data_ptr(), bias.data_ptr() if co == weight.shape[1] else 0)
        ctx.in_link = in_link if (in_link is not None and in_link.y is not None and
                                  in_link.y.data_ptr() != 0 and tuple(in_link.y.shape) == tuple(x.shape)) else None
        return y

    @staticmethod
    def backward(ctx, dy):
        x, weight = ctx.saved_tensors
        n, ci, h, w = x.shape
        ci_p, co_p = weight.shape[0], weight.shape[1]
        co = _pad64(co_p)
        padded = (ci, co) != (ci_p, co_p)
        dtype = x.dtype
        lib, st, dev = L.lib(), _stream(), x.device
        dy = _as_nhwc(dy, dtype)
        dx = None
        if ctx.needs_input_grad[0]:
            wp = packed(weight, L.PACK_CONVT_DGRAD, ci, co, dtype)
            dx = _nhwc_empty(n, ci, h, w, dtype, dev)
            ilink = ctx.in_link if (FUSE_BN_BWD and FUSE_BN_CONVT) else None
            if ilink is not None and ilink.y is not None and \
                    lib.unet_convt2x2_dgrad_bnrelu_supported(_DT[dtype], n, h, w, ci, co):
                part = torch.empty((lib.unet_convt2x2_dgrad_bnrelu_max_parts(), 2, ci), dtype=torch.float32, device=dev)
                nparts = C.c_int32(0)
                pc = ilink.coef
                L.check(lib.unet_convt2x2_dgrad_bnrelu(_DT[dtype], n, h, w, _ptr(dy), co, _ptr(wp), _ptr(ilink.y),
                                                       _ptr(pc[2]), _ptr(pc[3]), _ptr(pc[0]), _ptr(dx), ci, _ptr(part),
                                                       C.byref(nparts), st), "unet_convt2x2_dgrad_bnrelu")
                ilink.partial, ilink.n_parts, ilink.dz_ptr = part, nparts.value, dx.data_ptr()
            else:
                L.check(lib.unet_convt2x2_dgrad(_DT[dtype], n, h, w, _ptr(dy), co, _ptr(wp), _ptr(dx), ci, st),
                        "unet_convt2x2_dgrad")
        if padded:
            dw = torch.empty((ci, co, 2, 2), dtype=torch.float32, device=dev)
            db = torch.empty(co, dtype=torch.float32, device=dev)
        else:
            dw = grad_out(weight.shape, dev, ctx.keys[0])
            db = grad_out((co,), dev, ctx.keys[1])
        ws = _workspace(lib.unet_convt2x2_wgrad_workspace(n, h, w, ci, co), dev)
        L.check(lib.unet_convt2x2_wgrad(_DT[dtype], n, h, w, _ptr(x), ci, _ptr(dy), co, _ptr(dw), _ptr(db),
                                        _ptr(ws), ws.numel(), st), "unet_convt2x2_wgrad")
        if padded:
            (dw, dw_pad), (db, db_pad) = (grad_out(weight.shape, dev, ctx.keys[0]), dw), (grad_out((co_p,), dev, 0), db)
            _remap([(L.REMAP_UNPAD, dw_pad, dw, ci_p, co_p, 4, ci, co, 0),
# ... 722 lines not shown
```

Baseline: 1837 images/sec.

## Split fused BN backward into sums pass and recompute-apply pass, skipping dz round-trip

The fused pool and head BN-ReLU backward kernels no longer write an intermediate masked gradient that a separate premasked BN pass then reads and rewrites. A sums-only pass now produces the per-channel partial reductions, a small call turns them into coefficients, and an apply pass recomputes the masked gradient from y, dpooled and da_old and writes dy directly. This trades one full-tensor write-plus-read of dz for recomputing the ReLU, pool-scatter and head matvec in the second pass, and rereads the inputs twice. It depends on unet_bn_bwd_premasked accepting null dz, y and dy and emitting coefficients into the workspace, which the visible code does not show.

```diff
diff --git a/include/unet_hip.h b/include/unet_hip.h
--- a/include/unet_hip.h
+++ b/include/unet_hip.h
@@ -178,6 +178,12 @@
 int32_t unet_bn_relu_pool_bwd(int32_t dtype, const void* y, const void* dpooled, const void* da_old, int32_t n, int32_t h,
                               int32_t w, int32_t c, const float* scale, const float* shift, const float* mean, void* dz,
                               float* partial, int32_t* n_parts, void* stream);
+int32_t unet_bn_relu_pool_bwd_sums(int32_t dtype, const void* y, const void* dpooled, const void* da_old, int32_t n,
+                                   int32_t h, int32_t w, int32_t c, const float* scale, const float* shift,
+                                   const float* mean, float* partial, int32_t* n_parts, void* stream);
+int32_t unet_bn_relu_pool_bwd_apply(int32_t dtype, const void* y, const void* dpooled, const void* da_old, int32_t n,
+                                    int32_t h, int32_t w, int32_t c, const float* scale, const float* shift,
+                                    const float* coefs, void* dy, void* stream);
 
 int32_t unet_upsample_bilinear2x_fwd(int32_t dtype, const void* x, int32_t n, int32_t h, int32_t w,
                                      int32_t c, void* y, void* stream);
@@ -202,6 +208,15 @@
                              int32_t c_in, const float* weight, int32_t c_out, int32_t sigmoid, void* dz,
                              float* dweight, float* dbias, float* bn_partial, int32_t* n_parts, void* workspace,
                              size_t workspace_bytes, void* stream);
+int32_t unet_head_bnrelu_bwd_sums(int32_t dtype, const void* y, const float* bn_scale, const float* bn_shift,
+                                  const float* bn_mean, const float* out, const float* dout, int32_t n, int32_t h,
+                                  int32_t w, int32_t c_in, const float* weight, int32_t c_out, int32_t sigmoid,
+                                  float* dweight, float* dbias, float* bn_partial, int32_t* n_parts, void* workspace,
+                                  size_t workspace_bytes, void* stream);
+int32_t unet_head_bnrelu_bwd_apply(int32_t dtype, const void* y, const float* bn_scale, const float* bn_shift,
+                                   const float* out, const float* dout, int32_t n, int32_t h, int32_t w, int32_t c_in,
+                                   const float* weight, int32_t c_out, int32_t sigmoid, const float* coefs, void* dy,
+                                   void* stream);
 
 size_t unet_loss_workspace(int64_t elems);
 int32_t unet_loss_mse_focal(const float* recon, const float* image, int64_t n_recon, const float* amap,
diff --git a/tiaozhanbei_unet_amd/_lib.py b/tiaozhanbei_unet_amd/_lib.py
--- a/tiaozhanbei_unet_amd/_lib.py
+++ b/tiaozhanbei_unet_amd/_lib.py
@@ -98,12 +98,16 @@
     "unet_head_bnrelu_fwd": (_i, [_i, _p, _i, _i, _i, _i, _p, _p, _p, _p, _i, _i, _p, _p]),
     "unet_head_bnrelu_max_parts": (_z, []),
     "unet_head_bnrelu_bwd": (_i, [_i, _p, _p, _p, _p, _p, _p, _i, _i, _i, _i, _p, _i, _i, _p, _p, _p, _p, _p, _p, _z, _p]),
+    "unet_head_bnrelu_bwd_sums": (_i, [_i, _p, _p, _p, _p, _p, _p, _i, _i, _i, _i, _p, _i, _i, _p, _p, _p, _p, _p, _z, _p]),
+    "unet_head_bnrelu_bwd_apply": (_i, [_i, _p, _p, _p, _p, _p, _i, _i, _i, _i, _p, _i, _i, _p, _p, _p]),
     "unet_maxpool2_fwd": (_i, [_i, _p, _i, _i, _i, _i, _p, _p]),
     "unet_maxpool2_bwd": (_i, [_i, _p, _p, _i, _i, _i, _i, _p, _i, _p]),
     "unet_bn_relu_pool_supported": (_i, [_i, _i]),
     "unet_bn_relu_pool_fwd": (_i, [_i, _p, _i, _i, _i, _i, _p, _p, _p, _p, _p]),
     "unet_bn_relu_pool_max_parts": (_z, []),
     "unet_bn_relu_pool_bwd": (_i, [_i, _p, _p, _p, _i, _i, _i, _i, _p, _p, _p, _p, _p, _p, _p]),
+    "unet_bn_relu_pool_bwd_sums": (_i, [_i, _p, _p, _p, _i, _i, _i, _i, _p, _p, _p, _p, _p, _p]),
+    "unet_bn_relu_pool_bwd_apply": (_i, [_i, _p, _p, _p, _i, _i, _i, _i, _p, _p, _p, _p, _p]),
     "unet_upsample_bilinear2x_fwd": (_i, [_i, _p, _i, _i, _i, _i, _p, _p]),
     "unet_upsample_bilinear2x_bwd": (_i, [_i, _p, _i, _i, _i, _i, _p, _p]),
     "unet_head_fwd": (_i, [_i, _p, _i, _i, _i, _i, _p, _p, _i, _i, _p, _p]),
diff --git a/tiaozhanbei_unet_amd/csrc/elementwise.hip b/tiaozhanbei_unet_amd/csrc/elementwise.hip
--- a/tiaozhanbei_unet_amd/csrc/elementwise.hip
+++ b/tiaozhanbei_unet_amd/csrc/elementwise.hip
@@ -312,12 +312,14 @@
   }
 }
 
-template <typename T, typename IDX>
+enum { POOL_BWD_FULL = 0, POOL_BWD_SUMS = 1, POOL_BWD_APPLY = 2 };
+template <typename T, typename IDX, int MODE = POOL_BWD_FULL>
 __global__ __launch_bounds__(256) void bn_relu_pool_bwd_kernel(const T* __restrict__ y, const T* __restrict__ dpooled,
                                                                const T* da_old, const float* __restrict__ scale,
                                                                const float* __restrict__ shift,
                                                                const float* __restrict__ mean, T* dz,
-                                                               float* __restrict__ part, int N, int H, int W, int C) {
+                                                               float* __restrict__ part, int N, int H, int W, int C,
+                                                               const float* __restrict__ coefs = nullptr) {
   constexpr int PIECE = ET<T>::PIECE;
   typedef IDX idx_t;
   __shared__ float red[2][256][PIECE + 1];
@@ -325,11 +327,15 @@
   const int WH = (H + 1) / 2, WW = (W + 1) / 2;
   const idx_t total = (idx_t)N * WH * WW * G;
   const int g = threadIdx.x % G;
+  constexpr bool SUM = MODE != POOL_BWD_APPLY, APPLY = MODE == POOL_BWD_APPLY;
   float sc[PIECE], sh[PIECE], mu[PIECE], s0[PIECE], s1[PIECE];
+  float cA[APPLY ? PIECE : 1], cB[APPLY ? PIECE : 1], cK[APPLY ? PIECE : 1];
 #pragma unroll
   for (int j = 0; j < PIECE; ++j) {
-    sc[j] = scale[g * PIECE + j]; sh[j] = shift[g * PIECE + j]; mu[j] = mean[g * PIECE + j];
+    sc[j] = scale[g * PIECE + j]; sh[j] = shift[g * PIECE + j];
+    mu[j] = SUM ? mean[g * PIECE + j] : 0.f;
     s0[j] = 0.f; s1[j] = 0.f;
+    if constexpr (APPLY) { cA[j] = coefs[g * PIECE + j]; cB[j] = coefs[C + g * PIECE + j]; cK[j] = coefs[2 * C + g * PIECE + j]; }
   }
   const idx_t i0 = (idx_t)blockIdx.x * 256 + threadIdx.x;
   idx_t t0 = i0 / G;
@@ -378,15 +384,21 @@
           const float d = f[k] ? od[k][j] + gr[j] : od[k][j];
           const float da = ET<T>::to_f(ET<T>::from_f(d));
           const float v = z[k] > 0.f ? da : 0.f;
-          od[k][j] = v;
-          s0[j] += v;
-          s1[j] = fmaf(v, yv[k][j] - mu[j], s1[j]);
+          if constexpr (SUM) {
+            od[k][j] = v;
+            s0[j] += v;
+            s1[j] = fmaf(v, yv[k][j] - mu[j], s1[j]);
+          } else {
+            od[k][j] = fmaf(cA[j], v, fmaf(cB[j], yv[k][j], cK[j]));
+          }
         }
       }
-      Vec<T>::store(dz + base, od[0]);
-      Vec<T>::store(dz + o1, od[1]);
-      Vec<T>::store(dz + o2, od[2]);
-      Vec<T>::store(dz + o3, od[3]);
+      if constexpr (MODE != POOL_BWD_SUMS) {
+        Vec<T>::store(dz + base, od[0]);
+        Vec<T>::store(dz + o1, od[1]);
+        Vec<T>::store(dz + o2, od[2]);
+        Vec<T>::store(dz + o3, od[3]);
+      }
     } else {
     float yv[4][PIECE], av[4][PIECE], gr[PIECE];
     bool on[4][PIECE];
@@ -428,11 +440,15 @@
         }
         const float da = ET<T>::to_f(ET<T>::from_f(d[j]));
         const float v = ET<T>::to_f(ET<T>::from_f(on[k][j] ? da : 0.f));
-        d[j] = v;
-        s0[j] += v;
-        s1[j] = fmaf(v, yv[k][j] - mu[j], s1[j]);
-      }
-      Vec<T>::store(dz + o, d);
+        if constexpr (SUM) {
+          d[j] = v;
+          s0[j] += v;
+          s1[j] = fmaf(v, yv[k][j] - mu[j], s1[j]);
+        } else {
+          d[j] = fmaf(cA[j], v, fmaf(cB[j], yv[k][j], cK[j]));
+        }
+      }
+      if constexpr (MODE != POOL_BWD_SUMS) Vec<T>::store(dz + o, d);
     }
     }
     ox += sx;
@@ -441,6 +457,7 @@
     if (oy >= WH) { oy -= WH; ++n; }
     n += sn;
   }
+  if constexpr (APPLY) return;
 #pragma unroll
   for (int j = 0; j < PIECE; ++j) { red[0][threadIdx.x][j] = s0[j]; red[1][threadIdx.x][j] = s1[j]; }
   __syncthreads();
@@ -695,13 +712,16 @@
 namespace { constexpr int POOL_BWD_MAX_BLOCKS = 256 * 8; }
 extern "C" size_t unet_bn_relu_pool_max_parts(void) { return POOL_BWD_MAX_BLOCKS; }
 
-extern "C" int32_t unet_bn_relu_pool_bwd(int32_t dtype, const void* y, const void* dpooled, const void* da_old, int32_t n,
-                                         int32_t h, int32_t w, int32_t c, const float* scale, const float* shift,
-                                         const float* mean, void* dz, float* partial, int32_t* n_parts, void* stream) {
-  UNET_REQUIRE(y && dpooled && scale && shift && mean && dz && partial && n_parts, UNET_ERR_BAD_ARG,
-               "unet_bn_relu_pool_bwd: null pointer");
+template <int MODE>
+static int32_t bn_relu_pool_bwd_impl(const char* what, int32_t dtype, const void* y, const void* dpooled, const void* da_old,
+                                     int32_t n, int32_t h, int32_t w, int32_t c, const float* scale, const float* shift,
+                                     const float* mean, void* dst, float* partial, int32_t* n_parts, const float* coefs,
+                                     void* stream) {
+  constexpr bool SUM = MODE != POOL_BWD_APPLY;
+  UNET_REQUIRE(y && dpooled && scale && shift && (dst || MODE == POOL_BWD_SUMS) &&
+               (SUM ? (mean && partial && n_parts) : coefs != nullptr), UNET_ERR_BAD_ARG, "%s: null pointer", what);
   UNET_REQUIRE(n > 0 && h >= 2 && w >= 2 && unet_bn_relu_pool_supported(dtype, c), UNET_ERR_UNSUPPORTED,
-               "unet_bn_relu_pool_bwd: c=%d h=%d w=%d", c, h, w);
+               "%s: c=%d h=%d w=%d", what, c, h, w);
   hipStream_t s = (hipStream_t)stream;
   ProfScope prof(UNET_K_POOL, 0.0, s, "bn_relu_pool_bwd_kernel");
   const long long total = (long long)n * ((h + 1) / 2) * ((w + 1) / 2) * (c / (dtype == UNET_BF16 ? 8 : 4));
@@ -709,17 +729,42 @@
   const bool small = (long long)n * h * w * c < 0x7FFFFFFFLL;
   if (dtype == UNET_BF16) {
     if (small)
-      hipLaunchKernelGGL((bn_relu_pool_bwd_kernel<bf16_t, int>), dim3(blocks), dim3(256), 0, s, (const bf16_t*)y,
-                         (const bf16_t*)dpooled, (const bf16_t*)da_old, scale, shift, mean, (bf16_t*)dz, partial, n, h, w, c);
+      hipLaunchKernelGGL((bn_relu_pool_bwd_kernel<bf16_t, int, MODE>), dim3(blocks), dim3(256), 0, s, (const bf16_t*)y,
+                         (const bf16_t*)dpooled, (const bf16_t*)da_old, scale, shift, mean, (bf16_t*)dst, partial, n, h, w, c,
+                         coefs);
     else
-      hipLaunchKernelGGL((bn_relu_pool_bwd_kernel<bf16_t, long long>), dim3(blocks), dim3(256), 0, s, (const bf16_t*)y,
-                         (const bf16_t*)dpooled, (const bf16_t*)da_old, scale, shift, mean, (bf16_t*)dz, partial, n, h, w, c);
+      hipLaunchKernelGGL((bn_relu_pool_bwd_kernel<bf16_t, long long, MODE>), dim3(blocks), dim3(256), 0, s, (const bf16_t*)y,
+                         (const bf16_t*)dpooled, (const bf16_t*)da_old, scale, shift, mean, (bf16_t*)dst, partial, n, h, w, c,
+                         coefs);
   } else {
-    hipLaunchKernelGGL((bn_relu_pool_bwd_kernel<float, long long>), dim3(blocks), dim3(256), 0, s, (const float*)y,
-                       (const float*)dpooled, (const float*)da_old, scale, shift, mean, (float*)dz, partial, n, h, w, c);
-  }
-  *n_parts = blocks;
+    hipLaunchKernelGGL((bn_relu_pool_bwd_kernel<float, long long, MODE>), dim3(blocks), dim3(256), 0, s, (const float*)y,
+                       (const float*)dpooled, (const float*)da_old, scale, shift, mean, (float*)dst, partial, n, h, w, c,
+                       coefs);
+  }
+  if (SUM) *n_parts = blocks;
   return unet_check_launch("bn_relu_pool_bwd_kernel");
+}
+
+extern "C" int32_t unet_bn_relu_pool_bwd(int32_t dtype, const void* y, const void* dpooled, const void* da_old, int32_t n,
+                                         int32_t h, int32_t w, int32_t c, const float* scale, const float* shift,
+                                         const float* mean, void* dz, float* partial, int32_t* n_parts, void* stream) {
+  return bn_relu_pool_bwd_impl<POOL_BWD_FULL>("unet_bn_relu_pool_bwd", dtype, y, dpooled, da_old, n, h, w, c, scale, shift,
+                                              mean, dz, partial, n_parts, nullptr, stream);
+}
+
+extern "C" int32_t unet_bn_relu_pool_bwd_sums(int32_t dtype, const void* y, const void* dpooled, const void* da_old,
+                                              int32_t n, int32_t h, int32_t w, int32_t c, const float* scale,
+                                              const float* shift, const float* mean, float* partial, int32_t* n_parts,
+                                              void* stream) {
+  return bn_relu_pool_bwd_impl<POOL_BWD_SUMS>("unet_bn_relu_pool_bwd_sums", dtype, y, dpooled, da_old, n, h, w, c, scale,
+                                              shift, mean, nullptr, partial, n_parts, nullptr, stream);
+}
+
+extern "C" int32_t unet_bn_relu_pool_bwd_apply(int32_t dtype, const void* y, const void* dpooled, const void* da_old,
+                                               int32_t n, int32_t h, int32_t w, int32_t c, const float* scale,
+                                               const float* shift, const float* coefs, void* dy, void* stream) {
+  return bn_relu_pool_bwd_impl<POOL_BWD_APPLY>("unet_bn_relu_pool_bwd_apply", dtype, y, dpooled, da_old, n, h, w, c, scale,
+                                               shift, nullptr, dy, nullptr, nullptr, coefs, stream);
 }
 
 extern "C" int32_t unet_upsample_bilinear2x_fwd(int32_t dtype, const void* x, int32_t n, int32_t h, int32_t w,
diff --git a/tiaozhanbei_unet_amd/csrc/head.hip b/tiaozhanbei_unet_amd/csrc/head.hip
--- a/tiaozhanbei_unet_amd/csrc/head.hip
+++ b/tiaozhanbei_unet_amd/csrc/head.hip
@@ -13,6 +13,27 @@
     n = p / hw;
     q = p - n * hw;
   }
+}
+
+__device__ __forceinline__ float head_dlogit(const float* __restrict__ dout, const float* __restrict__ out,
+                                             long long idx, int sigm) {
+  float d = dout[idx];
+  if (sigm) { const float o = out[idx]; d *= o * (1.f - o); }
+  return d;
+}
+
+template <int CO, int WS>
+__device__ __forceinline__ float head_dx(const float (&ds)[CO], const float* wr) {
+  float t = 0.f;
+#pragma unroll
+  for (int co = 0; co < CO; ++co) t = fmaf(ds[co], wr[co * WS], t);
+  return t;
+}
+
+template <typename T, int CO, int WS>
+__device__ __forceinline__ float head_dz(const float (&ds)[CO], const float* wr, float yv, float scale, float shift) {
+  const float t = head_dx<CO, WS>(ds, wr);
+  return ET<T>::to_f(ET<T>::from_f(fmaf(yv, scale, shift) > 0.f ? t : 0.f));
 }
 
 template <typename T, int TPP, int CO, bool BN = false>
@@ -123,7 +144,7 @@
   }
 }
 
-template <typename T, int TPP, int CO, bool BN = false>
+template <typename T, int TPP, int CO, bool BN = false, bool STORE = true>
 __global__ __launch_bounds__(256) void head_bwd_kernel(const T* __restrict__ x, const float* __restrict__ out,
                                                        const float* __restrict__ dout, long long pixels,
                                                        long long hw, int Cin, const float* __restrict__ w,
@@ -171,8 +192,7 @@
         split_pixel(p, hw, n, q);
 #pragma unroll
         for (int co = 0; co < CO; ++co) {
-          float d = dout[(n * CO + co) * hw + q];
-          if (sigm) { const float o = out[(n * CO + co) * hw + q]; d *= o * (1.f - o); }
+          const float d = head_dlogit(dout, out, (n * CO + co) * hw + q, sigm);
           dl[co] = d;
           dbacc[co] += d;
         }
@@ -195,37 +215,28 @@
         float ds[CO], d[PIECE];
 #pragma unroll
         for (int co = 0; co < CO; ++co) ds[co] = __shfl(dl[co], s * PPW + sub);
-#pragma unroll
-        for (int j = 0; j < PIECE; ++j) d[j] = 0.f;
         float av[PIECE];
-        bool on[PIECE];
+#pragma unroll
+        for (int j = 0; j < PIECE; ++j) {
+          if constexpr (BN) av[j] = ET<T>::to_f(ET<T>::from_f(fmaxf(fmaf(v[i][j], sc[j], sh[j]), 0.f)));
+          else av[j] = v[i][j];
+        }
+#pragma unroll
+        for (int co = 0; co < CO; ++co)
+#pragma unroll
+          for (int j = 0; j < PIECE; ++j) dwacc[co][j] = fmaf(ds[co], av[j], dwacc[co][j]);
 #pragma unroll
         for (int j = 0; j < PIECE; ++j) {
           if constexpr (BN) {
-            const float z = fmaf(v[i][j], sc[j], sh[j]);
-            on[j] = z > 0.f;
-            av[j] = ET<T>::to_f(ET<T>::from_f(fmaxf(z, 0.f)));
-          } else {
-            on[j] = true;
-            av[j] = v[i][j];
-          }
-        }
-#pragma unroll
-        for (int co = 0; co < CO; ++co)
-#pragma unroll
-          for (int j = 0; j < PIECE; ++j) {
-            d[j] = fmaf(ds[co], wr[co][j], d[j]);
-            dwacc[co][j] = fmaf(ds[co], av[j], dwacc[co][j]);
-          }
-        if constexpr (BN) {
-#pragma unroll
-          for (int j = 0; j < PIECE; ++j) {
-            d[j] = ET<T>::to_f(ET<T>::from_f(on[j] ? d[j] : 0.f));
+            d[j] = head_dz<T, CO, PIECE>(ds, &wr[0][j], v[i][j], sc[j], sh[j]);
             bs0[j] += d[j];
             bs1[j] = fmaf(d[j], v[i][j] - mu[j], bs1[j]);
+          } else {
+            d[j] = head_dx<CO, PIECE>(ds, &wr[0][j]);
           }
         }
-        if (p < pixels) Vec<T>::store(dx + p * Cin + g * PIECE, d);
+        if constexpr (STORE)
+          if (p < pixels) Vec<T>::store(dx + p * Cin + g * PIECE, d);
       }
     }
   }
@@ -290,7 +301,7 @@
   }
 }
 
-template <typename T, int CO, bool BN>
+template <typename T, int CO, bool BN, bool STORE = true>
 __global__ __launch_bounds__(256) void head_bwd_tile_kernel(const T* __restrict__ x, const float* __restrict__ out,
                                                             const float* __restrict__ dout, long long pixels,
                                                             long long hw, const float* __restrict__ w, int sigm,
@@ -344,8 +355,7 @@
         split_pixel(p, hw, n, q);
 #pragma unroll
         for (int co = 0; co < CO; ++co) {
-          float d = dout[(n * CO + co) * hw + q];
-          if (sigm) { const float o = out[(n * CO + co) * hw + q]; d *= o * (1.f - o); }
+          const float d = head_dlogit(dout, out, (n * CO + co) * hw + q, sigm);
           dl[co] = d;
           dbacc[co] += d;
         }
@@ -376,26 +386,19 @@
 #pragma unroll
       for (int j = 0; j < 2; ++j) {
         float av = v[j];
-        bool on = true;
+        if constexpr (BN) av = ET<T>::to_f(ET<T>::from_f(fmaxf(fmaf(v[j], sc[j], sh[j]), 0.f)));
+#pragma unroll
+        for (int co = 0; co < CO; ++co) dwacc[co][j] = fmaf(ds[co], av, dwacc[co][j]);
         if constexpr (BN) {
-          const float z = fmaf(v[j], sc[j], sh[j]);
-          on = z > 0.f;
-          av = ET<T>::to_f(ET<T>::from_f(fmaxf(z, 0.f)));
-        }
-        float t = 0.f;
-#pragma unroll
-        for (int co = 0; co < CO; ++co) {
-          t = fmaf(ds[co], wr[co][j], t);
-          dwacc[co][j] = fmaf(ds[co], av, dwacc[co][j]);
-        }
-        if constexpr (BN) {
-          t = ET<T>::to_f(ET<T>::from_f(on ? t : 0.f));
-          bs0[j] += t;
-          bs1[j] = fmaf(t, v[j] - mu[j], bs1[j]);
-        }
-        d[j] = t;
-      }
-      if constexpr (sizeof(T) == 2) {
+          d[j] = head_dz<T, CO, 2>(ds, &wr[0][j], v[j], sc[j], sh[j]);
+          bs0[j] += d[j];
+          bs1[j] = fmaf(d[j], v[j] - mu[j], bs1[j]);
+        } else {
+          d[j] = head_dx<CO, 2>(ds, &wr[0][j]);
+        }
+      }
+      if constexpr (!STORE) {
+      } else if constexpr (sizeof(T) == 2) {
         const bf16_t d0 = (bf16_t)d[0], d1 = (bf16_t)d[1];
         const unsigned u = (unsigned)__builtin_bit_cast(unsigned short, d0) | ((unsigned)__builtin_bit_cast(unsigned short, d1) << 16);
         *reinterpret_cast<unsigned*>(tile + p * ROW + c2 * 4) = u;
@@ -406,15 +409,17 @@
     }
     __builtin_amdgcn_wave_barrier();
     asm volatile("s_waitcnt lgkmcnt(0)" ::: "memory");
-#pragma unroll
-    for (int i = 0; i < NLD; ++i) {
-      const int q = i * 64 + lane;
-      const long long p = base + q / (ROW / 16);
-      const u32x4 r = *reinterpret_cast<const u32x4*>(tile + q * 16);
-      if (p < pixels) *reinterpret_cast<u32x4*>(reinterpret_cast<char*>(dx) + base * ROW + (size_t)q * 16) = r;
-    }
-    __builtin_amdgcn_wave_barrier();
-    asm volatile("s_waitcnt lgkmcnt(0)" ::: "memory");
+    if constexpr (STORE) {
+#pragma unroll
+      for (int i = 0; i < NLD; ++i) {
+        const int q = i * 64 + lane;
+        const long long p = base + q / (ROW / 16);
+        const u32x4 r = *reinterpret_cast<const u32x4*>(tile + q * 16);
+        if (p < pixels) *reinterpret_cast<u32x4*>(reinterpret_cast<char*>(dx) + base * ROW + (size_t)q * 16) = r;
+      }
+      __builtin_amdgcn_wave_barrier();
+      asm volatile("s_waitcnt lgkmcnt(0)" ::: "memory");
+    }
   }
 #pragma unroll
   for (int co = 0; co < CO; ++co) {
@@ -452,18 +457,82 @@
   }
 }
 
-template <typename T, int CO, bool BN>
+template <typename T, int CO, bool BN, bool STORE = true>
 int32_t launch_head_bwd_tile(const void* x, const float* out, const float* dout, long long pixels, long long hw,
                              const float* w, int sigm, void* dx, float* part, const float* bn_scale,
                              const float* bn_shift, const float* bn_mean, float* bn_part, int nb, hipStream_t s) {
   constexpr int TILE = 64 * 64 * ET<T>::ES;
   constexpr int LDS = 4 * (TILE + CO * 256);
   static_assert(LDS >= 4 * (CO * 65 + 128) * 4, "reduction scratch fits the tile area");
-  auto kern = head_bwd_tile_kernel<T, CO, BN>;
+  auto kern = head_bwd_tile_kernel<T, CO, BN, STORE>;
   unet_set_max_lds(reinterpret_cast<const void*>(kern), LDS);
   hipLaunchKernelGGL(kern, dim3(nb), dim3(256), LDS, s, (const T*)x, out, dout, pixels, hw, w, sigm, (T*)dx, part,
                      bn_scale, bn_shift, bn_mean, bn_part);
   return unet_check_launch("head_bwd_tile_kernel");
+}
+
+template <typename T, int TPP, int CO>
+__global__ __launch_bounds__(256) void head_bnrelu_bwd_apply_kernel(const T* __restrict__ y, const float* __restrict__ out,
+                                                                    const float* __restrict__ dout, long long pixels,
+                                                                    long long hw, int Cin, const float* __restrict__ w,
+                                                                    int sigm, const float* __restrict__ bn_scale,
+                                                                    const float* __restrict__ bn_shift,
+                                                                    const float* __restrict__ coefs, T* __restrict__ dy) {
+  constexpr int PIECE = ET<T>::PIECE;
+  constexpr int PPW = 64 / TPP, S = TPP;
+  constexpr int SB = S < 8 ? S : 8;
+  const int lane = threadIdx.x & 63, wave = threadIdx.x >> 6;
+  const int g = lane % TPP, sub = lane / TPP;
+  float wr[CO][PIECE], sc[PIECE], sh[PIECE], A[PIECE], B[PIECE], K[PIECE];
+#pragma unroll
+  for (int j = 0; j < PIECE; ++j) {
+    const int ch = g * PIECE + j;
+#pragma unroll
+    for (int co = 0; co < CO; ++co) wr[co][j] = w[co * Cin + ch];
+    sc[j] = bn_scale[ch]; sh[j] = bn_shift[ch];
+    A[j] = coefs[ch]; B[j] = coefs[Cin + ch]; K[j] = coefs[2 * Cin + ch];
+  }
+  const long long nw = (long long)gridDim.x * 4;
+  for (long long c = blockIdx.x * 4LL + wave; c * 64 < pixels; c += nw) {
+    const long long base = c * 64;
+    float dl[CO];
+#pragma unroll
+    for (int co = 0; co < CO; ++co) dl[co] = 0.f;
+    {
+      const long long p = base + lane;
+      if (p < pixels) {
+        long long n, q;
+        split_pixel(p, hw, n, q);
+#pragma unroll
+        for (int co = 0; co < CO; ++co) dl[co] = head_dlogit(dout, out, (n * CO + co) * hw + q, sigm);
+      }
+    }
+#pragma unroll 1
+    for (int s0 = 0; s0 < S; s0 += SB) {
+      u32x4 raw[SB];
+#pragma unroll
+      for (int i = 0; i < SB; ++i) {
+        const long long p = base + (s0 + i) * PPW + sub;
+        raw[i] = u32x4{0u, 0u, 0u, 0u};
+        if (p < pixels) raw[i] = *reinterpret_cast<const u32x4*>(y + p * Cin + g * PIECE);
+      }
+#pragma unroll
+      for (int i = 0; i < SB; ++i) {
+        const int s = s0 + i;
+        const long long p = base + s * PPW + sub;
+        float ds[CO], r[PIECE], v[PIECE];
+        Vec<T>::load(reinterpret_cast<const T*>(&raw[i]), v);
+#pragma unroll
+        for (int co = 0; co < CO; ++co) ds[co] = __shfl(dl[co], s * PPW + sub);
+#pragma unroll
+        for (int j = 0; j < PIECE; ++j) {
+          const float dz = head_dz<T, CO, PIECE>(ds, &wr[0][j], v[j], sc[j], sh[j]);
+          r[j] = fmaf(A[j], dz, fmaf(B[j], v[j], K[j]));
+        }
+        if (p < pixels) Vec<T>::store(dy + p * Cin + g * PIECE, r);
+      }
+    }
+  }
 }
 
 inline int head_blocks(long long pixels, int tpp) {
@@ -599,13 +668,14 @@
 
 extern "C" size_t unet_head_bnrelu_max_parts(void) { return 1024; }
 
-extern "C" int32_t unet_head_bnrelu_bwd(int32_t dtype, const void* y, const float* bn_scale, const float* bn_shift,
-                                        const float* bn_mean, const float* out, const float* dout, int32_t n, int32_t h,
-                                        int32_t w, int32_t c_in, const float* weight, int32_t c_out, int32_t sigmoid,
-                                        void* dz, float* dweight, float* dbias, float* bn_partial, int32_t* n_parts,
-                                        void* workspace, size_t workspace_bytes, void* stream) {
-  UNET_REQUIRE(y && bn_scale && bn_shift && bn_mean && dout && weight && dz && dweight && dbias && bn_partial && n_parts &&
-               workspace && (out || !sigmoid), UNET_ERR_BAD_ARG, "unet_head_bnrelu_bwd: null pointer");
+template <bool STORE>
+static int32_t head_bnrelu_bwd_impl(int32_t dtype, const void* y, const float* bn_scale, const float* bn_shift,
+                                    const float* bn_mean, const float* out, const float* dout, int32_t n, int32_t h,
+                                    int32_t w, int32_t c_in, const float* weight, int32_t c_out, int32_t sigmoid,
+                                    void* dz, float* dweight, float* dbias, float* bn_partial, int32_t* n_parts,
+                                    void* workspace, size_t workspace_bytes, void* stream) {
+  UNET_REQUIRE(y && bn_scale && bn_shift && bn_mean && dout && weight && (dz || !STORE) && dweight && dbias && bn_partial &&
+               n_parts && workspace && (out || !sigmoid), UNET_ERR_BAD_ARG, "unet_head_bnrelu_bwd: null pointer");
   UNET_REQUIRE(n > 0 && h > 0 && w > 0, UNET_ERR_BAD_ARG, "unet_head_bnrelu_bwd: bad dims");
   UNET_REQUIRE(c_out >= 1 && c_out <= MAXCO && (c_in == 32 || c_in == 64 || c_in == 128), UNET_ERR_UNSUPPORTED,
                "unet_head_bnrelu_bwd: %d -> %d channels unsupported", c_in, c_out);
@@ -619,23 +689,23 @@
     nb = head_blocks(pixels, 8);
     int32_t rc = UNET_OK;
     if (dtype == UNET_BF16) {
-      HEAD_CO_SWITCH(rc = (launch_head_bwd_tile<bf16_t, CO, true>(y, out, dout, pixels, hw, weight, sigmoid, dz, (float*)workspace,
+      HEAD_CO_SWITCH(rc = (launch_head_bwd_tile<bf16_t, CO, true, STORE>(y, out, dout, pixels, hw, weight, sigmoid, dz, (float*)workspace,
                                                                 bn_scale, bn_shift, bn_mean, bn_partial, nb, s)));
     } else {
-      HEAD_CO_SWITCH(rc = (launch_head_bwd_tile<float, CO, true>(y, out, dout, pixels, hw, weight, sigmoid, dz, (float*)workspace,
+      HEAD_CO_SWITCH(rc = (launch_head_bwd_tile<float, CO, true, STORE>(y, out, dout, pixels, hw, weight, sigmoid, dz, (float*)workspace,
                                                                bn_scale, bn_shift, bn_mean, bn_partial, nb, s)));
     }
     if (rc) return rc;
   } else if (dtype == UNET_BF16) {
     const int tpp = tpp_of<bf16_t>(c_in);
     nb = head_blocks(pixels, tpp);
-    HEAD_TPP_SWITCH(bf16_t, tpp, hipLaunchKernelGGL((head_bwd_kernel<bf16_t, TPP, CO, true>), dim3(nb), dim3(256), 0, s,
+    HEAD_TPP_SWITCH(bf16_t, tpp, hipLaunchKernelGGL((head_bwd_kernel<bf16_t, TPP, CO, true, STORE>), dim3(nb), dim3(256), 0, s,
                     (const bf16_t*)y, out, dout, pixels, hw, c_in, weight, sigmoid, (bf16_t*)dz, (float*)workspace,
                     bn_scale, bn_shift, bn_mean, bn_partial));
   } else if (dtype == UNET_F32) {
     const int tpp = tpp_of<float>(c_in);
     nb = head_blocks(pixels, tpp);
-    HEAD_TPP_SWITCH(float, tpp, hipLaunchKernelGGL((head_bwd_kernel<float, TPP, CO, true>), dim3(nb), dim3(256), 0, s,
+    HEAD_TPP_SWITCH(float, tpp, hipLaunchKernelGGL((head_bwd_kernel<float, TPP, CO, true, STORE>), dim3(nb), dim3(256), 0, s,
                     (const float*)y, out, dout, pixels, hw, c_in, weight, sigmoid, (float*)dz, (float*)workspace,
                     bn_scale, bn_shift, bn_mean, bn_partial));
   } else {
@@ -649,3 +719,51 @@
                      (const float*)workspace, nb, c_out, c_in, dweight, dbias);
   return unet_check_launch("head_bwd_finalize_kernel");
 }
+
+extern "C" int32_t unet_head_bnrelu_bwd(int32_t dtype, const void* y, const float* bn_scale, const float* bn_shift,
+                                        const float* bn_mean, const float* out, const float* dout, int32_t n, int32_t h,
+                                        int32_t w, int32_t c_in, const float* weight, int32_t c_out, int32_t sigmoid,
+                                        void* dz, float* dweight, float* dbias, float* bn_partial, int32_t* n_parts,
+                                        void* workspace, size_t workspace_bytes, void* stream) {
+  return head_bnrelu_bwd_impl<true>(dtype, y, bn_scale, bn_shift, bn_mean, out, dout, n, h, w, c_in, weight, c_out, sigmoid,
+                                    dz, dweight, dbias, bn_partial, n_parts, workspace, workspace_bytes, stream);
+}
+
+extern "C" int32_t unet_head_bnrelu_bwd_sums(int32_t dtype, const void* y, const float* bn_scale, const float* bn_shift,
+                                             const float* bn_mean, const float* out, const float* dout, int32_t n,
+                                             int32_t h, int32_t w, int32_t c_in, const float* weight, int32_t c_out,
+                                             int32_t sigmoid, float* dweight, float* dbias, float* bn_partial,
+                                             int32_t* n_parts, void* workspace, size_t workspace_bytes, void* stream) {
+  return head_bnrelu_bwd_impl<false>(dtype, y, bn_scale, bn_shift, bn_mean, out, dout, n, h, w, c_in, weight, c_out,
+                                     sigmoid, nullptr, dweight, dbias, bn_partial, n_parts, workspace, workspace_bytes,
+                                     stream);
+}
+
+extern "C" int32_t unet_head_bnrelu_bwd_apply(int32_t dtype, const void* y, const float* bn_scale, const float* bn_shift,
+                                              const float* out, const float* dout, int32_t n, int32_t h, int32_t w,
+                                              int32_t c_in, const float* weight, int32_t c_out, int32_t sigmoid,
+                                              const float* coefs, void* dy, void* stream) {
+  UNET_REQUIRE(y && bn_scale && bn_shift && dout && weight && coefs && dy && (out || !sigmoid), UNET_ERR_BAD_ARG,
+               "unet_head_bnrelu_bwd_apply: null pointer");
+  UNET_REQUIRE(n > 0 && h > 0 && w > 0, UNET_ERR_BAD_ARG, "unet_head_bnrelu_bwd_apply: bad dims");
+  UNET_REQUIRE(c_out >= 1 && c_out <= MAXCO && (c_in == 32 || c_in == 64 || c_in == 128), UNET_ERR_UNSUPPORTED,
+               "unet_head_bnrelu_bwd_apply: %d -> %d channels unsupported", c_in, c_out);
+  hipStream_t s = (hipStream_t)stream;
+  const long long pixels = (long long)n * h * w, hw = (long long)h * w;
+  ProfScope prof(UNET_K_HEAD, 2.0 * pixels * c_in * c_out, s);
+  const long long want = cdiv64(pixels, 256);
+  const int nb = (int)(want < 2048 ? want : 2048);
+  if (dtype == UNET_BF16) {
+    const int tpp = tpp_of<bf16_t>(c_in);
+    HEAD_TPP_SWITCH(bf16_t, tpp, hipLaunchKernelGGL((head_bnrelu_bwd_apply_kernel<bf16_t, TPP, CO>), dim3(nb), dim3(256), 0, s,
+                    (const bf16_t*)y, out, dout, pixels, hw, c_in, weight, sigmoid, bn_scale, bn_shift, coefs, (bf16_t*)dy));
+  } else if (dtype == UNET_F32) {
+    const int tpp = tpp_of<float>(c_in);
+    HEAD_TPP_SWITCH(float, tpp, hipLaunchKernelGGL((head_bnrelu_bwd_apply_kernel<float, TPP, CO>), dim3(nb), dim3(256), 0, s,
+                    (const float*)y, out, dout, pixels, hw, c_in, weight, sigmoid, bn_scale, bn_shift, coefs, (float*)dy));
+  } else {
+    unet_set_error("unet_head_bnrelu_bwd_apply: dtype %d", dtype);
+    return UNET_ERR_BAD_ARG;
+  }
+  return unet_check_launch("head_bnrelu_bwd_apply_kernel");
+}
diff --git a/tiaozhanbei_unet_amd/ops.py b/tiaozhanbei_unet_amd/ops.py
--- a/tiaozhanbei_unet_amd/ops.py
+++ b/tiaozhanbei_unet_amd/ops.py
@@ -599,14 +599,17 @@
             part = torch.empty((lib.unet_head_bnrelu_max_parts(), 2, co), dtype=torch.float32, device=dev)
             nparts = C.c_int32(0)
             ws = _workspace(lib.unet_head_bwd_workspace(n, h, w, co, hc), dev)
-            L.check(lib.unet_head_bnrelu_bwd(dt, _ptr(y), _ptr(coef[2]), _ptr(coef[3]), _ptr(coef[0]), _ptr(out),
-                                             _ptr(dout), n, h, w, co, _ptr(head_w), hc, int(ctx.head), _ptr(dy),
-                                             _ptr(dhw), _ptr(dhb), _ptr(part), C.byref(nparts), _ptr(ws), ws.numel(),
-                                             st), "unet_head_bnrelu_bwd")
-            ws = _workspace(3 * co * 4, dev)
-            L.check(lib.unet_bn_bwd_premasked(dt, _ptr(dy), _ptr(y), pixels, co, _ptr(gamma), _ptr(coef[0]),
-                                              _ptr(coef[1]), _ptr(part), nparts.value, _ptr(dgb[0]), _ptr(dgb[1]),
-                                              _ptr(dy), _ptr(ws), ws.numel(), st), "unet_bn_bwd_premasked")
+            L.check(lib.unet_head_bnrelu_bwd_sums(dt, _ptr(y), _ptr(coef[2]), _ptr(coef[3]), _ptr(coef[0]), _ptr(out),
+                                                  _ptr(dout), n, h, w, co, _ptr(head_w), hc, int(ctx.head), _ptr(dhw),
+                                                  _ptr(dhb), _ptr(part), C.byref(nparts), _ptr(ws), ws.numel(), st),
+                    "unet_head_bnrelu_bwd_sums")
+            cf = _workspace(3 * co * 4, dev)
+            L.check(lib.unet_bn_bwd_premasked(dt, None, None, pixels, co, _ptr(gamma), _ptr(coef[0]), _ptr(coef[1]),
+                                              _ptr(part), nparts.value, _ptr(dgb[0]), _ptr(dgb[1]), None, _ptr(cf),
+                                              cf.numel(), st), "unet_bn_bwd_premasked(coefficients)")
+            L.check(lib.unet_head_bnrelu_bwd_apply(dt, _ptr(y), _ptr(coef[2]), _ptr(coef[3]), _ptr(out), _ptr(dout), n, h,
+                                                   w, co, _ptr(head_w), hc, int(ctx.head), _ptr(cf), _ptr(dy), st),
+                    "unet_head_bnrelu_bwd_apply")
         elif ctx.pool and dpooled is not None:
             own = False
             if da is not None:
@@ -620,14 +623,16 @@
             dy = da if own else _nhwc_empty(n, co, h, w, dtype, dev)
             part = torch.empty((lib.unet_bn_relu_pool_max_parts(), 2, co), dtype=torch.float32, device=dev)
             nparts = C.c_int32(0)
-            L.check(lib.unet_bn_relu_pool_bwd(dt, _ptr(y), _ptr(dpooled), _ptr(da), n, h, w, co, _ptr(coef[2]),
-                                              _ptr(coef[3]), _ptr(coef[0]), _ptr(dy), _ptr(part), C.byref(nparts), st),
-                    "unet_bn_relu_pool_bwd")
+            L.check(lib.unet_bn_relu_pool_bwd_sums(dt, _ptr(y), _ptr(dpooled), _ptr(da), n, h, w, co, _ptr(coef[2]),
+                                                   _ptr(coef[3]), _ptr(coef[0]), _ptr(part), C.byref(nparts), st),
+                    "unet_bn_relu_pool_bwd_sums")
             dgb = (grad_out(gamma.shape, dev, gkey), grad_out(gamma.shape, dev, bkey))
-            ws = _workspace(3 * co * 4, dev)
-            L.check(lib.unet_bn_bwd_premasked(dt, _ptr(dy), _ptr(y), pixels, co, _ptr(gamma), _ptr(coef[0]),
-                                              _ptr(coef[1]), _ptr(part), nparts.value, _ptr(dgb[0]), _ptr(dgb[1]),
-                                              _ptr(dy), _ptr(ws), ws.numel(), st), "unet_bn_bwd_premasked")
+            cf = _workspace(3 * co * 4, dev)
+            L.check(lib.unet_bn_bwd_premasked(dt, None, None, pixels, co, _ptr(gamma), _ptr(coef[0]), _ptr(coef[1]),
+                                              _ptr(part), nparts.value, _ptr(dgb[0]), _ptr(dgb[1]), None, _ptr(cf),
+                                              cf.numel(), st), "unet_bn_bwd_premasked(coefficients)")
+            L.check(lib.unet_bn_relu_pool_bwd_apply(dt, _ptr(y), _ptr(dpooled), _ptr(da), n, h, w, co, _ptr(coef[2]),
+                                                    _ptr(coef[3]), _ptr(cf), _ptr(dy), st), "unet_bn_relu_pool_bwd_apply")
         else:
             if da is None:
                 da = torch.zeros_like(y)
```

Result: faster. 1862 images/sec (median of 6 runs) (+1.4%).
